# inferflow/inferflow

Hardware: AMD Instinct MI355X
Metric: decode tokens/sec, Llama-2-7B Q4 batch=1 greedy (whole job) (higher is better)
Workload: dtype i8 (Q8 activations x Q4_B32T1A weights, i32 dot, f32 scale, f16 I/O); 1 GPU; llama2_7b decode, Q4_B32T1A weights + F16 lm_head, F16 KV cache, batch 1 greedy, 16-token prompt, context 21..1851; parallelism=single, weights_bytes=4309647360

## Files before the change

### include/inferflow_amd.h

```cpp
#ifndef INFERFLOW_AMD_H_
#define INFERFLOW_AMD_H_

#include <stddef.h>
#include <stdint.h>

#ifdef __cplusplus
extern "C" {
#endif

typedef enum {
    IFA_F32 = 0, IFA_F16 = 1,
    IFA_Q8_B32T1 = 7, IFA_Q8_B32T2 = 8, IFA_Q6_B64T1 = 9, IFA_Q5_B64T1 = 10, IFA_Q5_B32T1 = 11,
    IFA_Q4_B16 = 12, IFA_Q4_B32T1A = 13, IFA_Q4_B32T1B = 14, IFA_Q4_B64T1 = 17, IFA_Q3H_B64T1 = 18,
    IFA_Q3_B32T1A = 19, IFA_Q3_B32T1B = 20, IFA_Q2_B32T1A = 21, IFA_Q2_B32T1B = 22
} ifa_dtype;

enum {
    IFA_OK = 0,
    IFA_ERR_ARG = -1,
    IFA_ERR_DTYPE = -2,
    IFA_ERR_HIP = -3,
    IFA_ERR_STATE = -4,
    IFA_ERR_NOMEM = -5
};
// ... 89 lines not shown
typedef struct {
    int strategy_id;
    float temperature, top_p;
    int max_k;
    float min_p;
    int pool_size;
} ifa_sample_params;
int ifa_sample_pool_rows(const int *counts_dev, const int *ids_dev, const void *vals_f16_dev, size_t rows, int k_stride,
                         const ifa_sample_params *params_dev, unsigned long long *rng_state_dev, int *tokens_out_dev, int *index_out_dev,
                         float *weights_out_dev, int *err_dev, ifa_stream stream);
int ifa_sample_pool_host(const int *ids, const unsigned short *vals_f16, int count, const ifa_sample_params *p,
                         unsigned long long *rng_state_inout, int *token_out, int *index_out, int *cut_len_out, float *weights_out,
                         int *order_ids_out);

int ifa_logit_adjust_rows(const void *logits_f16, size_t row_stride, const int *row_idx_dev, const int *state_slot_dev, size_t rows, size_t n,
                          const unsigned *state_dev, const float *bias_dev, const float *params_dev, void *out_f16_dev, ifa_stream stream);
int ifa_logit_state_reset(int slot, const int *prompt_tokens_dev, size_t n_prompt, float rep, float freq, float pres, const int *bias_ids_dev,
                          const float *bias_vals_dev, size_t n_bias, size_t n, unsigned *state_dev, float *bias_dev, float *params_dev, ifa_stream stream);
int ifa_logit_state_add(const int *slots_dev, const int *tokens_dev, size_t n_pairs, size_t n, size_t n_slots, unsigned *state_dev, ifa_stream stream);

typedef struct ifa_model ifa_model;

typedef struct {
    int dim, layers, heads, kv_heads, head_dim, ffn, vocab, max_ctx;
    int norm_kind;
    int act_kind;
    int is_glu;
    int rope_order;
    int use_alibi;
    int parallel_attn;
    int share_input;
    float rope_theta, partial_rotary, kq_scale, eps;
    int kv_dtype;
    int full_quant_gemv;
    int experts, moe_top_k, moe_norm_topk;
    int tp_rank, tp_size;
    int device;
    float attn_norm_base, ffn_norm_base, out_norm_base, attn_out_scale, ffn_out_scale, out_scale;
    float embd_scale;
} ifa_model_config;

enum {
    IFA_T_EMBD = 0, IFA_T_OUT_NORM = 1, IFA_T_OUT_NORM_B = 2, IFA_T_LM_HEAD = 3,
    IFA_T_ATTN_NORM = 10, IFA_T_ATTN_NORM_B = 11, IFA_T_WQ = 12, IFA_T_WK = 13, IFA_T_WV = 14, IFA_T_WO = 15,
    IFA_T_FFN_NORM = 16, IFA_T_FFN_NORM_B = 17, IFA_T_W1 = 18, IFA_T_W2 = 19, IFA_T_W3 = 20, IFA_T_MOE_GATE = 21,
    IFA_T_WQ_B = 22, IFA_T_WK_B = 23, IFA_T_WV_B = 24, IFA_T_WO_B = 25, IFA_T_W1_B = 26, IFA_T_W2_B = 27, IFA_T_W3_B = 28,
    IFA_T_ATTN_POST_NORM = 29, IFA_T_ATTN_POST_NORM_B = 30, IFA_T_FFN_POST_NORM = 31, IFA_T_FFN_POST_NORM_B = 32
};

int ifa_model_create(const ifa_model_config *cfg, ifa_model **out);
int ifa_model_destroy(ifa_model *m);
int ifa_model_set_tensor(ifa_model *m, int layer, int tensor_id, int expert, int dtype,
                         const void *dev_src, size_t rows, size_t cols);
int ifa_model_set_tensor_f16(ifa_model *m, int layer, int tensor_id, int expert, int target_dtype,
                             const void *dev_src_f16, size_t rows, size_t cols);
int ifa_model_finalize(ifa_model *m);
int ifa_model_reset(ifa_model *m);
int ifa_model_kv_slots(ifa_model *m, int n_slots);
int ifa_model_select_kv(ifa_model *m, int slot);
int ifa_model_kv_copy(ifa_model *m, int src_slot, int dst_slot, int n_rows);
int ifa_model_kv_shift(ifa_model *m, int slot, int keep, int discard, int n_rows);
int ifa_kv_shift_rows(int kv_dtype, void *kcache, void *vcache, size_t kv_heads, size_t head_dim, int rope_order, int rope_cols,
                      const float *table_dev, size_t keep, size_t discard, size_t n_rows, ifa_stream stream);
int ifa_model_set_option(ifa_model *m, const char *name, int value);
int ifa_model_set_excluded_tokens(ifa_model *m, const int *ids_host, int n);
int ifa_model_perf_stat(ifa_model *m, int *keys_out, float *ms_out, int cap, int *n_out, int clear);
int ifa_model_fused_supported(ifa_model *m, char *why, size_t why_len);
int ifa_model_forward(ifa_model *m, const int *tokens_host, int n_tokens, int prefix_len,
                      void *logits_out_dev, int *next_token_host);
int ifa_model_decode(ifa_model *m, int first_token, int start_pos, int n_steps,
                     int *out_tokens_host, float *elapsed_ms);
int ifa_model_decode_sampled(ifa_model *m, int first_token, int start_pos, int n_steps, const ifa_sample_params *p,
                             unsigned long long *rng_state_inout, int state_slot, int *out_tokens_host, float *elapsed_ms);
int ifa_model_decode_prepare(ifa_model *m, int start_pos, int n_steps);
int ifa_model_decode_batch(ifa_model *m, int n, const int *tokens_host, const int *positions_host, const int *kv_slots_host,
                           int *next_tokens_host, void *logits_out_dev);
int ifa_model_decode_draft(ifa_model *m, int n, const int *tokens_host, int pos0, int *next_tokens_host, void *logits_out_dev);
int ifa_model_set_pool_excluded(ifa_model *m, const int *ids_host, int n);
int ifa_model_decode_pool(ifa_model *m, int token, int pos, int k, int *next_token_host,
                          int *pool_ids_host, unsigned short *pool_vals_host, int *pool_count_host);
int ifa_model_decode_batch_pool(ifa_model *m, int n, const int *tokens_host, const int *positions_host, const int *kv_slots_host,
                                int *next_tokens_host, int k, const int *rows_sel_host, int n_sel,
                                int *pool_ids_host, unsigned short *pool_vals_host, int *pool_counts_host);
int ifa_model_forward_pool(ifa_model *m, const int *tokens_host, int n_tokens, int prefix_len, void *logits_out_dev, int k,
                           int *next_token_host, int *pool_ids_host, unsigned short *pool_vals_host, int *pool_count_host);
int ifa_model_pool_lse(ifa_model *m, float *lse_host, int cap, int *n_out);
#define IFA_LOGIT_BIAS_MAX 1024
int ifa_model_logit_state_reset(ifa_model *m, int kv_slot, const int *prompt_host, int n_prompt, float rep, float freq, float pres,
                                const int *bias_ids_host, const float *bias_vals_host, int n_bias);
int ifa_model_logit_state_add(ifa_model *m, int n, const int *kv_slots_host, const int *tokens_host);
int ifa_model_pool_adjust(ifa_model *m, int n_sel, const int *state_slots_host);
int ifa_model_forward_score(ifa_model *m, const int *tokens_host, int n_tokens, int prefix_len, const int *targets_host,
                            float *lse_host, float *target_logit_host, int *next_token_host);
int ifa_model_get_buffer(ifa_model *m, const char *name, int layer, void **dptr, size_t *bytes);
void *ifa_model_stream(ifa_model *m);
int ifa_debug_alloc_fail_at(long long nth);
int ifa_debug_live_allocs(long long *count, long long *bytes);
int ifa_model_set_stream(ifa_model *m, ifa_stream stream);

typedef struct ifa_comm ifa_comm;
#define IFA_COMM_ID_BYTES 128
int ifa_comm_unique_id(void *id_out_128);
int ifa_comm_init_rank(const void *id_128, int nranks, int rank, int device, ifa_comm **out);
int ifa_comm_init_all(const int *device_ids, int n, ifa_comm **comms_out);
int ifa_comm_capturable(const ifa_comm *c);
unsigned long long ifa_comm_serial(const ifa_comm *c);
int ifa_comm_oneshot(const ifa_comm *c);
#define IFA_ONESHOT_HANDLE_BYTES 128
int ifa_comm_oneshot_export(ifa_comm *c, void *handle_out_128);
int ifa_comm_oneshot_import(ifa_comm *c, const void *handles_all_ranks);
int ifa_comm_set_oneshot(ifa_comm *c, int on);
int ifa_comm_status(ifa_comm *c);
int ifa_comm_abort(ifa_comm *c);
int ifa_comm_destroy(ifa_comm *c);
int ifa_comm_rank(const ifa_comm *c);
int ifa_comm_size(const ifa_comm *c);
int ifa_comm_group_start(void);
int ifa_comm_group_end(void);
int ifa_allreduce_sum_f16(ifa_comm *c, const void *send_f16, void *recv_f16, size_t count, ifa_stream stream);
int ifa_allgather(ifa_comm *c, const void *send, void *recv, size_t bytes_per_rank, ifa_stream stream);
int ifa_broadcast(ifa_comm *c, void *buf, size_t bytes, int root, ifa_stream stream);
int ifa_send(ifa_comm *c, const void *buf, size_t bytes, int peer, ifa_stream stream);
int ifa_recv(ifa_comm *c, void *buf, size_t bytes, int peer, ifa_stream stream);

int ifa_model_tp_begin(ifa_model *m, int token, int pos);
int ifa_model_tp_begin_hidden(ifa_model *m, const void *x_f16, int pos);
int ifa_model_tp_hidden(ifa_model *m, void *x_out_f16);
int ifa_model_tp_attn(ifa_model *m, int layer, void *partial_out_f16);
int ifa_model_tp_post_attn(ifa_model *m, int layer, const void *reduced_f16);
int ifa_model_tp_ffn(ifa_model *m, int layer, void *partial_out_f16);
int ifa_model_tp_post_ffn(ifa_model *m, int layer, const void *reduced_f16);
int ifa_model_tp_logits(ifa_model *m, void *logits_shard_out_f16);
int ifa_model_tp_set_token(ifa_model *m, const int *token_dev);
typedef struct {
    ifa_comm *tp;
    ifa_comm *world;
    int stage, n_stages;
    int prev_rank, next_rank, token_src;
    int vocab_offset;
    int force_collectives;
} ifa_tp_topology;
int ifa_model_tp_decode(ifa_model *m, const ifa_tp_topology *topo, int first_token, int start_pos, int n_steps,
                        int *out_tokens_host, float *elapsed_ms);
int ifa_model_tp_prefill(ifa_model *m, const ifa_tp_topology *topo, const int *tokens_host, int n_tokens, int start_pos,
                         void *logits_shard_out_dev, int *next_token_host);
int ifa_model_tp_decode_batch(ifa_model *m, const ifa_tp_topology *topo, int n, const int *tokens_host, const int *positions_host,
                              const int *kv_slots_host, int *next_tokens_host, void *logits_shard_out_dev);
int ifa_model_get_tensor(ifa_model *m, int layer, int tensor_id, int *dtype, void **dptr, size_t *rows, size_t *cols);
int ifa_model_get_expert_tensor(ifa_model *m, int layer, int expert, int tensor_id, int *dtype, void **dptr, size_t *rows, size_t *cols);
int ifa_model_time_kernel(ifa_model *m, int which, int iters, float *avg_us);

int ifa_decode_route_plan(const int *facts, int n_facts, int *out, int n_out);
int ifa_model_decode_route(ifa_model *m, int *out, int n_out);

int ifa_prompt_route_plan(const int *facts, int n_facts, int *out, int n_out);
int ifa_batch_route_plan(const int *facts, int n_facts, int *out, int n_out);
int ifa_model_prompt_route(ifa_model *m, int *out, int n_out);

#ifdef __cplusplus
}
#endif
#endif
```

### inferflow_amd/_capi.py

```python
import ctypes as C
import os

_HERE = os.path.dirname(os.path.abspath(__file__))
_LIB_PATH = os.environ.get("IFA_LIB") or os.path.join(_HERE, "lib", "libinferflow_amd.so")
_lib = None


class IfaError(RuntimeError):
    def __init__(self, code, msg):
        super().__init__("inferflow_amd error %d: %s" % (code, msg))
        self.code = code


def library_path():
    return _LIB_PATH


def lib():
    global _lib
    if _lib is None:
        if not os.path.exists(_LIB_PATH):
            raise ImportError(
                "inferflow_amd: %s is missing -- run `python __graft_entry__.py build` "
                "(hipcc --offload-arch=gfx950); there is no CPU fallback" % _LIB_PATH)
        L = C.CDLL(_LIB_PATH, mode=C.RTLD_GLOBAL)
        _declare(L)
        _lib = L
    return _lib


def check(rc):
    if rc != 0:
        raise IfaError(rc, lib().ifa_last_error().decode(errors="replace"))
    return rc


_vp, _sz, _i, _f = C.c_void_p, C.c_size_t, C.c_int, C.c_float

SIGNATURES = {
    "ifa_version": (C.c_char_p, []),
    "ifa_last_error": (C.c_char_p, []),
    "ifa_device_count": (_i, []),
    "ifa_set_device": (_i, [_i]),
    "ifa_malloc": (_i, [C.POINTER(_vp), _sz]),
    "ifa_free": (_i, [_vp]),
    "ifa_memcpy_h2d": (_i, [_vp, _vp, _sz, _vp]),
    "ifa_memcpy_d2h": (_i, [_vp, _vp, _sz, _vp]),
    "ifa_memcpy_d2d": (_i, [_vp, _vp, _sz, _vp]),
    "ifa_memset": (_i, [_vp, _i, _sz, _vp]),
    "ifa_stream_create": (_i, [C.POINTER(_vp)]),
    "ifa_stream_destroy": (_i, [_vp]),
    "ifa_stream_sync": (_i, [_vp]),
    "ifa_block_capacity": (_i, [_i]),
    "ifa_block_bytes": (_i, [_i]),
    "ifa_row_bytes": (_sz, [_i, _sz]),
    "ifa_dtype_from_name": (_i, [C.c_char_p]),
    "ifa_quantize": (_i, [_i, _vp, _sz, _sz, _vp, _vp]),
    "ifa_quantize_f32": (_i, [_i, _vp, _sz, _sz, _vp, _vp]),
    "ifa_dequantize": (_i, [_i, _vp, _sz, _sz, _vp, _vp]),
    "ifa_quantize_act_q8": (_i, [_vp, _sz, _sz, _vp, _vp]),
    "ifa_gemv": (_i, [_i, _vp, _sz, _sz, _i, _vp, _vp, _vp, _vp]),
    "ifa_gemm": (_i, [_i, _vp, _sz, _sz, _vp, _sz, _vp, _vp, _vp]),
    "ifa_attention_two_pass_min": (_i, [_i]),
    "ifa_attention_two_pass_min_keys": (_i, [_i]),
    "ifa_gemm_big_tiles": (_i, [_i]),
    "ifa_wait_grid_decision": (_i, [_i, _i, C.c_longlong]),
    "ifa_visible_cus_from_mask": (_i, [C.c_char_p, _i, _i]),
    "ifa_inlaunch_waits_enabled": (_i, []),
    "ifa_gemm_release_stream": (_i, [_vp]),
    "ifa_tiled_row_bytes": (_sz, [_i, _sz]),
    "ifa_repack_weights": (_i, [_i, _vp, _sz, _sz, _vp, _vp]),
    "ifa_gemv_tiled": (_i, [_i, _vp, _sz, _sz, _vp, _vp, _vp, _vp]),
    "ifa_layernorm": (_i, [_i, _vp, _sz, _sz, _vp, _vp, _f, _f, _vp, _vp]),
    "ifa_exact_rmsnorm": (_i, [_vp, _sz, _sz, _vp, _vp, _f, _f, _vp, _vp]),
    "ifa_exact_gemv": (_i, [_i, _vp, _sz, _sz, _i, _vp, _vp, _vp, _vp]),
    "ifa_exact_attention": (_i, [_vp, _vp, _vp, _i, _i, _i, _i, _i, _f, _vp, _vp]),
    "ifa_exact_activation_mul": (_i, [_i, _vp, _vp, _sz, _vp, _vp]),
    "ifa_rope": (_i, [_vp, _i, _i, _i, _i, _f, _i, _f, _vp]),
    "ifa_alibi": (_i, [_vp, _i, _i, _i, _i, _i, _vp]),
    "ifa_softmax": (_i, [_vp, _i, _i, _i, _i, _f, _vp]),
    "ifa_activation": (_i, [_i, _i, _vp, _sz, _sz, _vp, _vp]),
    "ifa_mul": (_i, [_vp, _vp, _sz, _vp, _vp]),
    "ifa_add": (_i, [_vp, _vp, _sz, _sz, _vp, _vp]),
    "ifa_scale": (_i, [_vp, _f, _sz, _vp, _vp]),
    "ifa_attention": (_i, [_vp, _vp, _vp, _i, _i, _i, _i, _i, _i, _i, _f, _i, _i, _i, _vp, _vp]),
    "ifa_moe_route_topk": (_i, [_vp, _sz, _i, _i, _i, _vp, _vp, _vp]),
    "ifa_kv_store": (_i, [_i, _vp, _sz, _sz, _vp, _sz, _vp]),
    "ifa_argmax": (_i, [_vp, _sz, _vp, _vp]),
    "ifa_argmax_masked": (_i, [_vp, _sz, _vp, _vp, _vp]),
    "ifa_topk_pool": (_i, [_vp, _sz, _sz, _i, _vp, _vp, _vp, _vp, _vp]),
    "ifa_sample_pool_rows": (_i, [_vp, _vp, _vp, _sz, _i, _vp, _vp, _vp, _vp, _vp, _vp, _vp]),
    "ifa_sample_pool_host": (_i, [_vp, _vp, _i, _vp, _vp, _vp, _vp, _vp, _vp, _vp]),
    "ifa_logsumexp_workspace": (_sz, [_sz, _sz]),
    "ifa_logsumexp_rows": (_i, [_vp, _sz, _vp, _sz, _sz, _vp, _vp, _vp, _vp, _vp]),
    "ifa_logit_adjust_rows": (_i, [_vp, _sz, _vp, _vp, _sz, _sz, _vp, _vp, _vp, _vp, _vp]),
    "ifa_logit_state_reset": (_i, [_i, _vp, _sz, _f, _f, _f, _vp, _vp, _sz, _sz, _vp, _vp, _vp, _vp]),
    "ifa_logit_state_add": (_i, [_vp, _vp, _sz, _sz, _sz, _vp, _vp]),
    "ifa_model_create": (_i, [_vp, C.POINTER(_vp)]),
    "ifa_model_destroy": (_i, [_vp]),
    "ifa_debug_alloc_fail_at": (_i, [C.c_longlong]),
    "ifa_debug_live_allocs": (_i, [C.POINTER(C.c_longlong), C.POINTER(C.c_longlong)]),
    "ifa_model_set_tensor": (_i, [_vp, _i, _i, _i, _i, _vp, _sz, _sz]),
    "ifa_model_set_tensor_f16": (_i, [_vp, _i, _i, _i, _i, _vp, _sz, _sz]),
    "ifa_model_finalize": (_i, [_vp]),
    "ifa_model_reset": (_i, [_vp]),
    "ifa_model_set_option": (_i, [_vp, C.c_char_p, _i]),
    "ifa_model_set_excluded_tokens": (_i, [_vp, _vp, _i]),
    "ifa_model_perf_stat": (_i, [_vp, _vp, _vp, _i, _vp, _i]),
    "ifa_model_fused_supported": (_i, [_vp, C.c_char_p, _sz]),
    "ifa_model_forward": (_i, [_vp, _vp, _i, _i, _vp, _vp]),
    "ifa_model_decode": (_i, [_vp, _i, _i, _i, _vp, _vp]),
    "ifa_model_decode_sampled": (_i, [_vp, _i, _i, _i, _vp, _vp, _i, _vp, _vp]),
    "ifa_model_decode_prepare": (_i, [_vp, _i, _i]),
    "ifa_add_by_row_index": (_i, [_vp, _vp, _sz, _sz, _vp, _vp, _vp]),
    "ifa_model_kv_slots": (_i, [_vp, _i]),
    "ifa_model_select_kv": (_i, [_vp, _i]),
    "ifa_model_kv_copy": (_i, [_vp, _i, _i, _i]),
    "ifa_model_kv_shift": (_i, [_vp, _i, _i, _i, _i]),
    "ifa_kv_shift_rows": (_i, [_i, _vp, _vp, _sz, _sz, _i, _i, _vp, _sz, _sz, _sz, _vp]),
    "ifa_model_decode_batch": (_i, [_vp, _i, _vp, _vp, _vp, _vp, _vp]),
    "ifa_model_decode_draft": (_i, [_vp, _i, _vp, _i, _vp, _vp]),
    "ifa_model_set_pool_excluded": (_i, [_vp, _vp, _i]),
    "ifa_model_decode_pool": (_i, [_vp, _i, _i, _i, _vp, _vp, _vp, _vp]),
    "ifa_model_decode_batch_pool": (_i, [_vp, _i, _vp, _vp, _vp, _vp, _i, _vp, _i, _vp, _vp, _vp]),
    "ifa_model_forward_pool": (_i, [_vp, _vp, _i, _i, _vp, _i, _vp, _vp, _vp, _vp]),
    "ifa_model_pool_lse": (_i, [_vp, _vp, _i, _vp]),
    "ifa_model_logit_state_reset": (_i, [_vp, _i, _vp, _i, _f, _f, _f, _vp, _vp, _i]),
    "ifa_model_logit_state_add": (_i, [_vp, _i, _vp, _vp]),
    "ifa_model_pool_adjust": (_i, [_vp, _i, _vp]),
    "ifa_model_forward_score": (_i, [_vp, _vp, _i, _i, _vp, _vp, _vp, _vp]),
    "ifa_model_get_buffer": (_i, [_vp, C.c_char_p, _i, C.POINTER(_vp), C.POINTER(_sz)]),
    "ifa_model_stream": (_vp, [_vp]),
    "ifa_model_time_kernel": (_i, [_vp, _i, _i, _vp]),
    "ifa_decode_route_plan": (_i, [_vp, _i, _vp, _i]),
    "ifa_model_decode_route": (_i, [_vp, _vp, _i]),
    "ifa_prompt_route_plan": (_i, [_vp, _i, _vp, _i]),
    "ifa_batch_route_plan": (_i, [_vp, _i, _vp, _i]),
    "ifa_model_prompt_route": (_i, [_vp, _vp, _i]),
    "ifa_model_set_stream": (_i, [_vp, _vp]),
    "ifa_model_tp_begin": (_i, [_vp, _i, _i]),
    "ifa_model_tp_begin_hidden": (_i, [_vp, _vp, _i]),
    "ifa_model_tp_hidden": (_i, [_vp, _vp]),
    "ifa_model_tp_attn": (_i, [_vp, _i, _vp]),
    "ifa_model_tp_post_attn": (_i, [_vp, _i, _vp]),
    "ifa_model_tp_ffn": (_i, [_vp, _i, _vp]),
    "ifa_model_tp_post_ffn": (_i, [_vp, _i, _vp]),
    "ifa_model_tp_logits": (_i, [_vp, _vp]),
    "ifa_model_tp_set_token": (_i, [_vp, _vp]),
    "ifa_comm_unique_id": (_i, [_vp]),
    "ifa_comm_init_rank": (_i, [_vp, _i, _i, _i, C.POINTER(_vp)]),
    "ifa_comm_init_all": (_i, [_vp, _i, C.POINTER(_vp)]),
    "ifa_comm_destroy": (_i, [_vp]),
    "ifa_comm_capturable": (_i, [_vp]),
    "ifa_comm_serial": (C.c_ulonglong, [_vp]),
    "ifa_comm_abort": (_i, [_vp]),
    "ifa_comm_oneshot": (_i, [_vp]),
    "ifa_comm_oneshot_export": (_i, [_vp, _vp]),
    "ifa_comm_oneshot_import": (_i, [_vp, _vp]),
    "ifa_comm_set_oneshot": (_i, [_vp, _i]),
    "ifa_comm_status": (_i, [_vp]),
    "ifa_comm_rank": (_i, [_vp]),
    "ifa_comm_size": (_i, [_vp]),
    "ifa_comm_group_start": (_i, []),
    "ifa_comm_group_end": (_i, []),
    "ifa_allreduce_sum_f16": (_i, [_vp, _vp, _vp, _sz, _vp]),
    "ifa_allgather": (_i, [_vp, _vp, _vp, _sz, _vp]),
    "ifa_broadcast": (_i, [_vp, _vp, _sz, _i, _vp]),
    "ifa_send": (_i, [_vp, _vp, _sz, _i, _vp]),
    "ifa_recv": (_i, [_vp, _vp, _sz, _i, _vp]),
    "ifa_model_tp_decode": (_i, [_vp, _vp, _i, _i, _i, _vp, _vp]),
    "ifa_model_tp_prefill": (_i, [_vp, _vp, _vp, _i, _i, _vp, _vp]),
    "ifa_model_tp_decode_batch": (_i, [_vp, _vp, _i, _vp, _vp, _vp, _vp, _vp]),
    "ifa_model_get_tensor": (_i, [_vp, _i, _i, _vp, C.POINTER(_vp), C.POINTER(_sz), C.POINTER(_sz)]),
    "ifa_model_get_expert_tensor": (_i, [_vp, _i, _i, _i, _vp, C.POINTER(_vp), C.POINTER(_sz), C.POINTER(_sz)]),
}


_ip = C.POINTER(C.c_int)
ENGINE_SIGNATURES = {
    "ifa_engine_create": (_vp, [C.c_char_p, C.c_char_p, C.c_char_p]),
    "ifa_engine_destroy": (None, [_vp]),
    "ifa_engine_last_error": (C.c_char_p, []),
    "ifa_engine_add_query": (_i, [_vp, _ip, _i]),
    "ifa_engine_add_query_ex": (_i, [_vp, _ip, _i, _i, _i, _f]),
    "ifa_engine_add_query_lp": (_i, [_vp, _ip, _i, _i, _i, _f, _i]),
    "ifa_engine_add_query_opt": (_i, [_vp, _ip, _i, _vp]),
    "ifa_engine_last_logprobs": (_i, [_vp, _i, C.POINTER(_f), _ip, C.POINTER(_f), _i, _ip]),
    "ifa_engine_score": (_i, [_vp, _ip, _i, C.POINTER(_f)]),
    "ifa_engine_strategy_id": (_i, [_vp, C.c_char_p]),
    "ifa_sampling_choose": (_i, [_vp, _i, _i, _i, _f, _i, _f, C.c_longlong, _i, _ip, C.POINTER(_f), _ip, C.POINTER(_f), _i]),
    "ifa_sampling_choose_ex": (_i, [_vp, _i, _i, C.POINTER(_f), _f, C.c_longlong, _i, _ip, C.POINTER(_f), _ip, C.POINTER(_f), _i, C.POINTER(_f), _ip, _i]),
    "ifa_sampling_choose_from_pool": (_i, [_ip, _vp, _i, _i, C.POINTER(_f), _f, C.c_longlong, _i, _ip, C.POINTER(_f), _ip, C.POINTER(_f), _i, C.POINTER(_f), _ip, _i]),
    "ifa_sampling_random_doubles": (_i, [C.c_longlong, _i, C.POINTER(C.c_double)]),
    "ifa_engine_query_count": (_i, [_vp]),
    "ifa_engine_remove_query": (_i, [_vp, _i]),
    "ifa_engine_infer": (_i, [_vp, _ip, _ip, _i]),
    "ifa_engine_commit": (_i, [_vp, _ip, _ip, _ip, _i]),
    "ifa_engine_last_logits": (_i, [_vp, _i, _vp, _sz, _ip, _ip]),
    "ifa_engine_perf_stat": (_i, [_vp, _vp, _vp, _i]),
    "ifa_engine_generate": (_i, [_vp, _i, _i, _ip, C.POINTER(_f)]),
    "ifa_engine_generate_lookup": (_i, [_vp, _i, _i, _ip, _i, _ip, C.POINTER(_f)]),
    "ifa_lookup_draft": (_i, [_ip, _i, _ip, _i, _i, _i, _i, _ip]),
    "ifa_engine_perplexity": (_i, [_vp, _ip, _i, _i, _i, C.POINTER(C.c_double), C.POINTER(C.c_double), C.POINTER(C.c_longlong)]),
    "ifa_engine_perplexity_device": (_i, [_vp, _ip, _i, _i, _i, C.POINTER(C.c_double), C.POINTER(C.c_double), C.POINTER(C.c_longlong)]),
    "ifa_perplexity_token_nll": (C.c_double, [_vp, _i, _i]),
    "ifa_engine_model_info": (_i, [_vp, C.c_char_p]),
    "ifa_engine_query_cached_tokens": (_i, [_vp, _i]),
    "ifa_context_shift_plan": (_i, [_i, _i, _i, _i, _ip]),
    "ifa_engine_shift_query": (_i, [_vp, _i, _i, _i]),
    "ifa_engine_query_shifted_tokens": (_i, [_vp, _i]),
    "ifa_prefix_cache_plan": (_i, [_ip, _ip, _ip, C.POINTER(C.c_longlong), _i, _ip, _i, _i, _ip]),
    "ifa_step_plan_query": (_i, [_i, _i, _i, _i, _i, _ip]),
    "ifa_step_plan_batch": (_i, [_i, _ip, _i, _ip, _ip]),
    "ifa_engine_worker": (_vp, [_vp, _i]),
    "ifa_engine_worker_plan": (_i, [_vp, _i, _ip]),
    "ifa_service_parse_request": (_i, [C.c_char_p, _i, C.c_char_p, _sz]),
    "ifa_service_format_response": (_i, [_ip, _i, _i, _i, _i, _i, C.c_char_p, _sz]),
    "ifa_service_selftest_loop": (_i, [_i, _i, _i, _ip, _i, _i, _i, _i, _i, C.c_char_p, _sz]),
    "ifa_service_selftest_request": (_i, [C.c_char_p, _i, _i, C.c_char_p, _sz]),
    "ifa_partition_slice": (_i, [_i, _i, _i, _i, _i, _i, _i, _i, _sz, _sz, C.POINTER(_sz)]),
    "ifa_partition_split_layers": (_i, [_i, _i, _ip, _i]),
}


class QueryOptions(C.Structure):
    _fields_ = [("struct_size", C.c_size_t), ("strategy_id", C.c_int), ("random_seed", C.c_int), ("temperature", C.c_float),
                ("logprobs", C.c_int), ("repetition_penalty", C.c_float), ("presence_penalty", C.c_float),
                ("frequency_penalty", C.c_float), ("n_logit_bias", C.c_int), ("logit_bias_ids", C.POINTER(C.c_int)),
                ("logit_bias_values", C.POINTER(C.c_float))]


class QueryOptionsShift(C.Structure):
    _fields_ = QueryOptions._fields_ + [("context_shift", C.c_int), ("context_keep", C.c_int)]


class SampleParams(C.Structure):
    _fields_ = [("strategy_id", C.c_int), ("temperature", C.c_float), ("top_p", C.c_float), ("max_k", C.c_int), ("min_p", C.c_float), ("pool_size", C.c_int)]


class ModelConfig(C.Structure):
    _fields_ = [(n, C.c_int) for n in (
        "dim", "layers", "heads", "kv_heads", "head_dim", "ffn", "vocab", "max_ctx",
        "norm_kind", "act_kind", "is_glu", "rope_order", "use_alibi", "parallel_attn",
        "share_input")] + [(n, C.c_float) for n in (
            "rope_theta", "partial_rotary", "kq_scale", "eps")] + [(n, C.c_int) for n in (
                "kv_dtype", "full_quant_gemv", "experts", "moe_top_k", "moe_norm_topk",
                "tp_rank", "tp_size", "device")] + [(n, C.c_float) for n in (
                    "attn_norm_base", "ffn_norm_base", "out_norm_base", "attn_out_scale", "ffn_out_scale", "out_scale", "embd_scale")]


def _declare(L):
    missing = []
    for name, (res, args) in list(SIGNATURES.items()) + list(ENGINE_SIGNATURES.items()):
        try:
            fn = getattr(L, name)
        except AttributeError:
            missing.append(name)
            continue
        fn.restype = res
        fn.argtypes = args
    if missing and os.environ.get("IFA_LIB"):
        return
    if missing:
        raise ImportError("libinferflow_amd.so lacks symbols declared in include/*.h: %s" % missing)
```

### inferflow_amd/csrc/ifa_decode_route.h

```cpp
#pragma once
#include <algorithm>
#include <cstddef>
#include <cstring>

static constexpr size_t IFA_LDS_LIMIT = 160 * 1024;

namespace ifa {
constexpr int DEC_ATTN_MAX_SPLITS = 32;
constexpr int DEC_PV_STAGE = 4096;

constexpr size_t dec_attn_scores_smem(int head_dim, bool q8) { return q8 ? 16 : (size_t)256 * (head_dim * 2 + 16); }
constexpr size_t dec_attn_pv_smem(int head_dim, int max_ctx, int nsplits = 8)
{
    const size_t nsplit = 256 / (head_dim / 8);
    const size_t chunk = (((size_t)max_ctx + nsplits - 1) / nsplits + 63) / 64 * 64;
    return 8 * 4 + nsplit * head_dim * 4 + (size_t)(DEC_PV_STAGE + 8) * 2 + chunk * 2 + 16;
}
constexpr size_t dec_attn_smem(int head_dim, int max_ctx, int ktile_rows = 0)
{
    const size_t nsplit = 256 / (head_dim / 8);
    return (size_t)head_dim * 3 * 2 + 16 * 4 + nsplit * head_dim * 4 + (size_t)ktile_rows * head_dim * 2 + (((size_t)max_ctx * 2 + 15) & ~(size_t)15) + 16;
}

inline bool dec_qkv_attn_ul_shape(int rw, int gk) { return (rw == 6 && gk == 8) || (rw == 3 && gk == 32); }

struct DecRouteFacts {
    int head_dim = 0, heads = 0, kv_heads = 0, max_ctx = 0, kv_q8 = 0;
    int reach = 0;
    int attn_split_ctx = -1, attn_nsplits = 0, attn_kt = 1, attn_unload = 1, fuse_attn = 1, fuse_ffn = 0, attn_q8 = 1;
    int tail_layers_ok = 0, gk = 0, rw = 0;
    int chain_level = 0;
    int have_attq = 0;
    int waits = 1;
    int num_cus = 0, visible_cus = 0;
    int own_launches = 0;
};
enum DecRouteKind { DEC_ROUTE_ONE_WORKGROUP = 0, DEC_ROUTE_SPLIT = 1, DEC_ROUTE_FUSED_TAIL = 2 };

struct DecRoute {
    int kind = DEC_ROUTE_ONE_WORKGROUP;
    int nsplits = 0;
    int pb = 256, kt = 0, ul = 0;
    int gk = 0, rw = 0;
    int chain = 0;
    int split_threshold = 0, split = 0;
    int lds_attn = 0;
    int lds_scores = 0, lds_pv = 0;
    int error = 0;
    bool operator==(const DecRoute &o) const { return std::memcmp(this, &o, sizeof(o)) == 0; }
};
constexpr int DEC_ROUTE_N_FACTS = sizeof(DecRouteFacts) / sizeof(int), DEC_ROUTE_N_OUT = sizeof(DecRoute) / sizeof(int);

inline DecRoute plan_decode_route(const DecRouteFacts &f)
{
    DecRoute r;
    const bool tail_possible = f.fuse_attn && f.waits && dec_attn_smem(f.head_dim, f.max_ctx, 256) <= IFA_LDS_LIMIT && f.tail_layers_ok && (long long)f.kv_heads * f.gk <= (long long)f.visible_cus;
    r.split_threshold = f.attn_split_ctx >= 0 ? f.attn_split_ctx : (tail_possible && f.attn_unload) ? (f.heads > f.kv_heads ? 640 : 512) : 320;
    r.split = (r.split_threshold > 0 && f.reach > r.split_threshold) ? (f.reach > 8192 ? 16 : 8) : 0;
    const int bucket = f.reach <= 64 ? 64 : (f.reach <= 128 ? 128 : 256);
    const bool lds_split = dec_attn_smem(f.head_dim, f.max_ctx, 0) > IFA_LDS_LIMIT;
    r.kind = (r.split || lds_split) ? DEC_ROUTE_SPLIT : (tail_possible && !f.own_launches) ? DEC_ROUTE_FUSED_TAIL : DEC_ROUTE_ONE_WORKGROUP;
    const bool kt_fits = f.attn_kt && !f.kv_q8 && dec_attn_smem(f.head_dim, f.max_ctx, bucket) <= IFA_LDS_LIMIT;
    if (r.kind == DEC_ROUTE_SPLIT) {
        r.pb = 0; r.nsplits = r.split > 1 ? r.split : 8;
        while (r.nsplits < DEC_ATTN_MAX_SPLITS && dec_attn_pv_smem(f.head_dim, f.max_ctx, r.nsplits) > IFA_LDS_LIMIT) r.nsplits *= 2;
        if (f.attn_nsplits > 0) r.nsplits = std::min(f.attn_nsplits, DEC_ATTN_MAX_SPLITS);
        r.lds_scores = (int)dec_attn_scores_smem(f.head_dim, f.kv_q8 != 0); r.lds_pv = (int)dec_attn_pv_smem(f.head_dim, f.max_ctx, r.nsplits);
        r.error = (size_t)r.lds_pv > IFA_LDS_LIMIT;
    } else if (r.kind == DEC_ROUTE_ONE_WORKGROUP) {
        const bool pow2 = f.head_dim == 32 || f.head_dim == 64 || f.head_dim == 128;
        r.pb = pow2 ? bucket : 256; r.kt = kt_fits && pow2;
    } else {
        r.kt = kt_fits;
        const bool unload = (f.attn_unload >= 1 && bucket == 256) || (f.attn_unload >= 2 && bucket == 128 && (r.kt || f.kv_q8));
        r.ul = unload && dec_qkv_attn_ul_shape(f.rw, f.gk);
        r.pb = (r.ul && bucket == 64) || (!f.kv_q8 && !r.kt) ? 256 : bucket;
        r.gk = f.gk; r.rw = f.rw;
    }
    if (r.kind != DEC_ROUTE_SPLIT) r.lds_attn = (int)dec_attn_smem(f.head_dim, f.max_ctx, r.kt ? r.pb : 0);
    if (!f.own_launches) {
        r.chain = (f.fuse_ffn && f.waits && f.num_cus <= f.visible_cus) ? std::min(f.fuse_ffn, 2) : 0;
        if (r.chain == 2 && (!f.have_attq || !f.attn_q8 || f.head_dim % 32 != 0)) r.chain = 1;
        r.chain = std::min(r.chain, f.chain_level);
    }
    return r;
}

}
```

### inferflow_amd/csrc/ifa_engine.hip

```cpp
#include <mutex>
#include <unordered_map>
#include "ifa_engine_state.h"

namespace ifa {

namespace {
struct SpaceBook {
    std::mutex mu;
    std::unordered_map<void *, size_t> live;
    long long live_bytes = 0, fail_at = 0;
};
SpaceBook &book() { static SpaceBook *b = new SpaceBook(); return *b; }

template <class Alloc> int space_alloc(const char *call, void **p, size_t bytes, Alloc alloc)
{
    SpaceBook &b = book();
    *p = nullptr;
    {
        std::lock_guard<std::mutex> g(b.mu);
        if (b.fail_at > 0 && --b.fail_at == 0)
            return ifa_fail(IFA_ERR_HIP, "%s(%zu bytes) failed: out of memory (simulated: ifa_debug_alloc_fail_at)", call, bytes);
    }
    const hipError_t e = alloc(p, bytes);
    if (e != hipSuccess) {
        (void)hipGetLastError();
        *p = nullptr;
        return ifa_fail(IFA_ERR_HIP, "%s(%zu bytes) failed: %s", call, bytes, hipGetErrorString(e));
    }
    if (*p) { std::lock_guard<std::mutex> g(b.mu); b.live[*p] = bytes; b.live_bytes += (long long)bytes; }
    return IFA_OK;
}

void space_forget(void *p)
{
    SpaceBook &b = book();
    std::lock_guard<std::mutex> g(b.mu);
    auto it = b.live.find(p);
    if (it != b.live.end()) { b.live_bytes -= (long long)it->second; b.live.erase(it); }
}
}

int DevSpace::alloc(void **p, size_t bytes) { return space_alloc("hipMalloc", p, bytes, [](void **q, size_t n) { return hipMalloc(q, n); }); }
void DevSpace::free(void *p) { space_forget(p); (void)hipFree(p); }
int PinSpace::alloc(void **p, size_t bytes) { return space_alloc("hipHostMalloc", p, bytes, [](void **q, size_t n) { return hipHostMalloc(q, n, hipHostMallocDefault); }); }
void PinSpace::free(void *p) { space_forget(p); (void)hipHostFree(p); }

}

extern "C" int ifa_debug_alloc_fail_at(long long nth)
{
    IFA_REQUIRE(nth >= 0, "ifa_debug_alloc_fail_at: nth %lld", nth);
    std::lock_guard<std::mutex> g(book().mu);
    book().fail_at = nth;
    return IFA_OK;
}

extern "C" int ifa_debug_live_allocs(long long *count, long long *bytes)
{
    std::lock_guard<std::mutex> g(book().mu);
    if (count) *count = (long long)book().live.size();
    if (bytes) *bytes = book().live_bytes;
    return IFA_OK;
}

namespace ifae {

int perf_begin(ifa_model *m, int key)
{
    if (!m->opt_perf_stat) return -1;
    hipStreamCaptureStatus cs = hipStreamCaptureStatusNone;
    if (hipStreamIsCapturing(m->stream, &cs) != hipSuccess || cs != hipStreamCaptureStatusNone) { (void)hipGetLastError(); return -1; }
    auto take = [&]() -> hipEvent_t {
        if (!m->perf_pool.empty()) { hipEvent_t e = m->perf_pool.back(); m->perf_pool.pop_back(); return e; }
        hipEvent_t e = nullptr;
        if (hipEventCreate(&e) != hipSuccess) { (void)hipGetLastError(); return nullptr; }
        return e;
    };
    ifa_model::PerfSpanRec r; r.key = key; r.e0 = take(); r.e1 = take();
    if (!r.e0 || !r.e1) { if (r.e0) m->perf_pool.push_back(r.e0); if (r.e1) m->perf_pool.push_back(r.e1); return -1; }
    if (hipEventRecord(r.e0, m->stream) != hipSuccess) { (void)hipGetLastError(); m->perf_pool.push_back(r.e0); m->perf_pool.push_back(r.e1); return -1; }
    m->perf_spans.push_back(r);
    return (int)m->perf_spans.size() - 1;
}

void perf_end(ifa_model *m, int idx)
{
    if (idx < 0 || idx >= (int)m->perf_spans.size()) return;
    if (hipEventRecord(m->perf_spans[(size_t)idx].e1, m->stream) != hipSuccess) (void)hipGetLastError();
}

int perf_collect(ifa_model *m)
{
    if (m->perf_spans.empty()) return IFA_OK;
    IFA_HIP_CHECK(hipStreamSynchronize(m->stream));
    for (auto &r : m->perf_spans) {
        float ms = 0.0f;
        if (hipEventElapsedTime(&ms, r.e0, r.e1) == hipSuccess) m->perf_map[r.key] += ms;
        else (void)hipGetLastError();
        m->perf_pool.push_back(r.e0); m->perf_pool.push_back(r.e1);
    }
    m->perf_spans.clear();
    return IFA_OK;
}

void drop_graphs(ifa_model *m)
{
    if (m->tp_graph_exec) { (void)hipGraphExecDestroy(m->tp_graph_exec); m->tp_graph_exec = nullptr; }
    if (m->tp_graph) { (void)hipGraphDestroy(m->tp_graph); m->tp_graph = nullptr; }
    if (m->graph_exec) { (void)hipGraphExecDestroy(m->graph_exec); m->graph_exec = nullptr; }
    if (m->graph) { (void)hipGraphDestroy(m->graph); m->graph = nullptr; }
    if (m->graph_exec_n) { (void)hipGraphExecDestroy(m->graph_exec_n); m->graph_exec_n = nullptr; }
    if (m->graph_n) { (void)hipGraphDestroy(m->graph_n); m->graph_n = nullptr; }
    for (auto &sl : m->slots) {
        if (sl.exec) { (void)hipGraphExecDestroy(sl.exec); sl.exec = nullptr; }
        if (sl.graph) { (void)hipGraphDestroy(sl.graph); sl.graph = nullptr; }
    }
    for (auto &kv : m->batch_graphs) if (kv.second) (void)hipGraphExecDestroy(kv.second);
    m->batch_graphs.clear();
    for (auto &kv : m->draft_graphs) if (kv.second) (void)hipGraphExecDestroy(kv.second);
    m->draft_graphs.clear();
    sampled_drop_graphs(m);
}

int ensure_scratch(ifa_model *m, int T)
{
    if (T <= m->scratch_tokens) return IFA_OK;
    const ifa_model_config &c = m->cfg;
    const size_t D = c.dim, QD = (size_t)c.heads * c.head_dim, KVD = (size_t)c.kv_heads * c.head_dim, F = c.ffn;
    size_t maxcols = std::max(std::max(D, QD), F);
    Scratch n;
    int rc;
    if ((rc = n.x.alloc(T * D)) || (rc = n.x2.alloc(T * D)) || (rc = n.xn.alloc(T * D)) || (rc = n.hn.alloc(T * D)) || (rc = n.pn.alloc(T * D))
        || (rc = n.q.alloc(T * QD)) || (rc = n.k.alloc(T * KVD)) || (rc = n.v.alloc(T * KVD)) || (rc = n.att.alloc(T * QD))
        || (rc = n.a.alloc(T * D)) || (rc = n.f.alloc(T * D)) || (rc = n.t1.alloc(std::max<size_t>(T, 3) * F)) || (rc = n.t2.alloc(T * F))
        || (rc = n.logits.alloc((size_t)T * c.vocab)))
        return rc;
    if (!m->dqkv && (rc = n.dqkv.alloc(QD + 2 * KVD))) return rc;
    if (T <= 32 && !m->bqkv && ((rc = n.bqkv.alloc(32 * (QD + 2 * KVD))) || (rc = n.brope.alloc(32 * (size_t)c.head_dim)))) return rc;
    if (c.experts > 0) {
        const size_t cap = (size_t)T * (size_t)std::max(1, c.moe_top_k);
        if ((rc = n.moe_gate.alloc((size_t)T * c.experts)) || (rc = n.moe_out.alloc((size_t)T * D)) || (rc = n.moe_in.alloc((size_t)T * D))
            || (rc = n.moe_wdev.alloc(cap)) || (rc = n.moe_idx.alloc(cap)) || (rc = n.moe_pin.alloc(cap * (sizeof(int) + 2) + 16)))
            return rc;
        if (!m->moe_route) {
            if ((rc = n.moe_route.alloc(64 / sizeof(int)))) return rc;
            IFA_HIP_CHECK(hipMemsetAsync(n.moe_route, 0, 64, m->stream));
        }
        if ((rc = n.moe_sel.alloc(cap)) || (rc = n.moe_epos.alloc(cap)) || (rc = n.moe_counts.alloc(16))
            || (rc = n.moe_xq_in.alloc(cap * (D / 32 + 1) * 34)) || (rc = n.moe_xq_mid.alloc(cap * (F / 32 + 1) * 34))
            || (rc = n.moe_tiles.alloc((cap / 64 + (size_t)c.experts + 1) * sizeof(MoeTile)))
            || (rc = n.moe_singles.alloc(((size_t)c.experts + 1) * sizeof(MoeSingle))) || (rc = n.moe_smalls.alloc(((size_t)c.experts + 1) * sizeof(MoeTile)))
            || (rc = n.moe_selw.alloc(cap)) || (rc = n.moe_g1.alloc(cap * F)) || (rc = n.moe_g3.alloc(cap * F)) || (rc = n.moe_gin.alloc(cap * D))
            || (rc = n.moe_gout.alloc(cap * D)))
            return rc;
    }
    if ((rc = n.xq.alloc((maxcols / 32 + 1) * 34))) return rc;
    if (!m->attq && (rc = n.attq.alloc(xq_image_bytes(c.heads * c.head_dim)))) return rc;
    if ((rc = n.tokens_dev.alloc((size_t)T))) return rc;
    if (!n.dqkv) n.dqkv = std::move(m->dqkv);
    if (!n.bqkv) { n.bqkv = std::move(m->bqkv); n.brope = std::move(m->brope); }
    if (!n.moe_route) n.moe_route = std::move(m->moe_route);
    if (!n.attq) n.attq = std::move(m->attq);
    static_cast<Scratch &>(*m) = std::move(n);
    m->scratch_tokens = T;
    drop_graphs(m);
    return IFA_OK;
}

void *kv_ptr(ifa_model *m, size_t layer, int slot, bool is_v)
{
    if (slot == m->cur_slot || m->slots.empty()) return is_v ? m->layers[layer].vcache : m->layers[layer].kcache;
    const ifa_model::KvSlot &sl = m->slots[(size_t)slot];
    return is_v ? sl.v[layer] : sl.k[layer];
}

int ensure_mo(ifa_model *m)
{
    if (!m->opt_rows_mo) return IFA_OK;
    const int rc = ensure_mo_build(m);
    if (rc == IFA_OK) return IFA_OK;
    (void)hipGetLastError();
    for (Layer &L : m->layers) {
        for (Tensor &t : L.t) t.mo.reset();
        for (Tensor &t : L.experts) t.mo.reset();
        L.moe_table_mo.reset();
    }
    m->opt_rows_mo = 0;
    drop_graphs(m);
    fprintf(stderr, "inferflow_amd: the rows GEMM's operand-order weight copies could not be built (%s); batched steps use the tiled kernels\n", ifa_last_error());
    return IFA_OK;
}

int ensure_mo_build(ifa_model *m)
{
    const ifa_model_config &c = m->cfg;
    bool built = false;
    for (Layer &L : m->layers) {
        const bool moe = c.experts > 0 && L.t[T_MOE_GATE].present();
        const int ids[] = {T_WQ, T_WK, T_WV, T_WO, T_W1, T_W3, T_W2};
        for (int id : ids) {
            Tensor &t = L.t[id];
            if (moe && (id == T_W1 || id == T_W3 || id == T_W2)) continue;
            if (t.mo || !t.present() || !t.tiled || !rows_mo_fmt(t.dtype) || t.cols % 128 != 0) continue;
            if (m->opt_debug_mo_alloc_fail && built) return ifa_fail(IFA_ERR_HIP, "hipMalloc: out of memory (simulated: debug_mo_alloc_fail)");
            int rc = t.mo.alloc(gemm_rows_mo_bytes(t.rows, t.cols));
            if (rc) return rc;
            rc = gemm_rows_mo_build(t.dtype, t.tiled, t.rows, t.cols, t.mo, m->stream);
            if (rc) return rc;
            built = true;
        }
    }
    for (Layer &L : m->layers) {
        if (!(c.experts > 0 && L.t[T_MOE_GATE].present()) || L.moe_table_mo || (int)L.experts.size() != c.experts * 3) continue;
        bool ok = true;
        for (Tensor &t : L.experts) ok = ok && t.present() && t.tiled && is_q4(t.dtype) && t.cols % 128 == 0;
        if (!ok) continue;
        std::vector<void *> tab((size_t)c.experts * 4, nullptr);
        for (int e = 0; e < c.experts; e++) {
            const int order[3] = {0, 2, 1};
            for (int k = 0; k < 3; k++) {
                Tensor &t = L.experts[(size_t)e * 3 + order[k]];
                if (!t.mo) {
                    int rc = t.mo.alloc(gemm_rows_mo_bytes(t.rows, t.cols));
                    if (rc) return rc;
                    rc = gemm_rows_mo_build(t.dtype, t.tiled, t.rows, t.cols, t.mo, m->stream);
                    if (rc) return rc;
                    built = true;
                }
                tab[(size_t)e * 4 + k] = t.mo;
            }
        }
        { int rc = L.moe_table_mo.alloc(tab.size()); if (rc) return rc; }
        IFA_HIP_CHECK(hipMemcpy(L.moe_table_mo, tab.data(), tab.size() * sizeof(void *), hipMemcpyHostToDevice));
    }
    if (built) IFA_HIP_CHECK(hipStreamSynchronize(m->stream));
    return IFA_OK;
}

int ensure_x32(ifa_model *m)
{
    bool built = false;
    for (Layer &L : m->layers) {
        const int ids[] = {T_WQ, T_WK, T_WV, T_WO, T_W1, T_W3, T_W2};
        for (int id : ids) {
            Tensor &t = L.t[id];
            if (t.x32 || !t.present() || !t.tiled || (t.dtype != Q4_B64T1 && t.dtype != Q3H_B64T1) || t.cols % 64 != 0) continue;
            int rc = t.x32.alloc(t.rows * (t.cols / 32) * 20);
            if (rc) return rc;
            rc = expand_b64_to_q4b32(t.dtype, t.tiled, t.rows, t.cols, t.x32, m->stream);
            if (rc) return rc;
            built = true;
        }
    }
    if (built) IFA_HIP_CHECK(hipStreamSynchronize(m->stream));
    return IFA_OK;
}

int ensure_q3hn(ifa_model *m)
{
    bool built = false;
    for (Layer &L : m->layers) {
        const int ids[] = {T_WO, T_W1, T_W3, T_W2};
        for (int id : ids) {
            Tensor &t = L.t[id];
            if (t.q3hn || !t.present() || t.dtype != Q3H_B64T1 || t.cols % 64 != 0) continue;
            int rc = t.q3hn.alloc(t.rows * (t.cols / 64) * 32);
            if (rc) return rc;
            rc = q3h_native_rows(t.data, t.rows, t.cols, t.q3hn, m->stream);
            if (rc) return rc;
// ... 83 lines not shown
        if (vec) IFA_REQUIRE(rows * cols == ec, "ifa_model_set_tensor: tensor %d holds %zu x %zu values, the model needs %zu", tensor_id, rows, cols, ec);
        else {
            IFA_REQUIRE(ec == 0 || cols == ec, "ifa_model_set_tensor: tensor %d has %zu columns, the model needs %zu", tensor_id, cols, ec);
            IFA_REQUIRE(er == 0 || rows == er, "ifa_model_set_tensor: tensor %d has %zu rows, the model needs %zu", tensor_id, rows, er);
        }
        if (tensor_id == T_LM_HEAD && layer < 0) IFA_REQUIRE(rows <= (size_t)c.vocab, "ifa_model_set_tensor: lm_head has %zu rows, vocab is %d", rows, c.vocab);
        if (tensor_id == T_EMBD) IFA_REQUIRE(rows <= (size_t)c.vocab, "ifa_model_set_tensor: %zu embedding rows, vocab is %d", rows, c.vocab);
    }
    IFA_HIP_CHECK(hipSetDevice(m->cfg.device));
    Tensor *t;
    if (tensor_id < 10) t = &m->g[tensor_id];
    else {
        IFA_REQUIRE(layer >= 0 && layer < m->cfg.layers, "ifa_model_set_tensor: layer %d", layer);
        Layer &L = m->layers[(size_t)layer];
        if (expert >= 0) {
            if (L.experts.empty()) L.experts.resize((size_t)m->cfg.experts * 3);
            t = &L.experts[(size_t)expert * 3 + (tensor_id == T_W1 ? 0 : (tensor_id == T_W2 ? 1 : 2))];
        } else t = &L.t[tensor_id];
    }
    *t = Tensor();
    if (expert >= 0) m->layers[(size_t)layer].moe_table_mo.reset();
    IFA_HIP_CHECK(hipDeviceSynchronize());
    const size_t bytes = rows * ifa_row_bytes(dtype, cols);
    int rc = t->data.alloc(bytes);
    if (rc) return rc;
    IFA_HIP_CHECK(hipMemcpyAsync(t->data, dev_src, bytes, hipMemcpyDeviceToDevice, m->stream));
    t->dtype = dtype; t->rows = rows; t->cols = cols;
    const bool is_matrix = (layer < 0 && tensor_id == T_LM_HEAD) || tensor_id == T_WQ || tensor_id == T_WK || tensor_id == T_WV || tensor_id == T_WO
        || tensor_id == T_W1 || tensor_id == T_W2 || tensor_id == T_W3;
    if (is_matrix && ax8_eligible(dtype)) {
        if ((rc = t->tiled.alloc(rows * ifa_tiled_row_bytes(dtype, cols)))) return rc;
        rc = ifa_repack_weights(dtype, t->data, rows, cols, t->tiled, m->stream);
        if (rc) return rc;
    }
    IFA_HIP_CHECK(hipStreamSynchronize(m->stream));
    drop_graphs(m);
    return IFA_OK;
}

int ifa_model_set_tensor_f16(ifa_model *m, int layer, int tensor_id, int expert, int target_dtype,
                             const void *dev_src_f16, size_t rows, size_t cols)
{
    IFA_REQUIRE(m && dev_src_f16, "ifa_model_set_tensor_f16: null pointer");
    if (target_dtype == F16) return ifa_model_set_tensor(m, layer, tensor_id, expert, F16, dev_src_f16, rows, cols);
    IFA_HIP_CHECK(hipSetDevice(m->cfg.device));
    DevBuf<void> tmp;
    const size_t bytes = rows * ifa_row_bytes(target_dtype, cols);
    IFA_REQUIRE(bytes > 0, "ifa_model_set_tensor_f16: dtype %d", target_dtype);
    int rc = tmp.alloc(bytes);
    if (rc) return rc;
    IFA_HIP_CHECK(hipDeviceSynchronize());
    rc = ifa_quantize(target_dtype, dev_src_f16, rows, cols, tmp, m->stream);
    if (rc == IFA_OK) rc = ifa_model_set_tensor(m, layer, tensor_id, expert, target_dtype, tmp, rows, cols);
    (void)hipStreamSynchronize(m->stream);
    return rc;
}

int ifa_model_finalize(ifa_model *m)
{
    IFA_REQUIRE(m, "ifa_model_finalize: null model");
    IFA_HIP_CHECK(hipSetDevice(m->cfg.device));
    (void)wait_err_word();
    const ifa_model_config &c = m->cfg;
    const size_t KVD = (size_t)c.kv_heads * c.head_dim;
    IFA_REQUIRE(c.kv_dtype != Q8_B32T2 || KVD % 32 == 0, "Q8 KV cache needs kv_dim %% 32 == 0");
    m->kv_row_bytes = ifa_row_bytes(c.kv_dtype, KVD);
    int rc;
    for (Layer &L : m->layers) {
        if (!L.kcache) {
            const size_t kv_alloc = m->kv_row_bytes * (size_t)std::max(c.max_ctx, DEC_ATTN_MIN_ROWS);
            if ((rc = L.kcache.alloc(kv_alloc)) || (rc = L.vcache.alloc(kv_alloc))) return rc;
            IFA_HIP_CHECK(hipMemsetAsync(L.kcache, 0, kv_alloc, m->stream));
            IFA_HIP_CHECK(hipMemsetAsync(L.vcache, 0, kv_alloc, m->stream));
        }
        if (c.experts > 0 && (int)L.experts.size() == c.experts * 3) {
            std::vector<void *> tab((size_t)c.experts * 4, nullptr);
            for (int e = 0; e < c.experts; e++) {
                tab[(size_t)e * 4 + 0] = L.experts[(size_t)e * 3 + 0].tiled;
                tab[(size_t)e * 4 + 1] = L.experts[(size_t)e * 3 + 2].tiled;
                tab[(size_t)e * 4 + 2] = L.experts[(size_t)e * 3 + 1].tiled;
            }
            if (!L.moe_table && (rc = L.moe_table.alloc(tab.size()))) return rc;
            IFA_HIP_CHECK(hipMemcpy(L.moe_table, tab.data(), tab.size() * sizeof(void *), hipMemcpyHostToDevice));
            std::vector<void *> aos((size_t)c.experts * 3, nullptr);
            for (int e = 0; e < c.experts; e++) for (int k3 = 0; k3 < 3; k3++) aos[(size_t)e * 3 + k3] = L.experts[(size_t)e * 3 + k3].data;
            if (!L.moe_table_aos && (rc = L.moe_table_aos.alloc(aos.size()))) return rc;
            IFA_HIP_CHECK(hipMemcpy(L.moe_table_aos, aos.data(), aos.size() * sizeof(void *), hipMemcpyHostToDevice));
        }
    }
    if (!m->attn_ws.S) {
        if ((rc = m->attn_ws_S.alloc((size_t)c.heads * c.max_ctx + 32))
            || (rc = m->attn_ws_lmax.alloc((size_t)c.heads * DEC_ATTN_MAX_SPLITS))
            || (rc = m->attn_ws_opart.alloc((size_t)c.heads * DEC_ATTN_MAX_SPLITS * c.head_dim))) return rc;
        m->attn_ws.S = m->attn_ws_S; m->attn_ws.lmax = m->attn_ws_lmax; m->attn_ws.opart = m->attn_ws_opart;
    }
    if (!m->state) {
        if ((rc = m->state.alloc(8 + ifa_model::RING))) return rc;
        IFA_HIP_CHECK(hipMemsetAsync(m->state, 0, sizeof(int) * (8 + ifa_model::RING), m->stream));
        if ((rc = m->rope_tab.alloc((size_t)c.head_dim)) || (rc = m->host_pinned.alloc(16 + ifa_model::RING))) return rc;
    }
    if ((rc = ensure_scratch(m, 1))) return rc;
    IFA_HIP_CHECK(hipStreamSynchronize(m->stream));
    m->finalized = true;
    return IFA_OK;
}

int ifa_model_reset(ifa_model *m)
{
    IFA_REQUIRE(m && m->finalized, "ifa_model_reset: model not finalized");
    IFA_HIP_CHECK(hipSetDevice(m->cfg.device));
    for (Layer &L : m->layers) {
        IFA_HIP_CHECK(hipMemsetAsync(L.kcache, 0, m->kv_row_bytes * (size_t)m->cfg.max_ctx, m->stream));
        IFA_HIP_CHECK(hipMemsetAsync(L.vcache, 0, m->kv_row_bytes * (size_t)m->cfg.max_ctx, m->stream));
    }
    IFA_HIP_CHECK(hipStreamSynchronize(m->stream));
    return IFA_OK;
}

int ifa_model_kv_slots(ifa_model *m, int n_slots)
{
    IFA_REQUIRE(m && m->finalized, "ifa_model_kv_slots: model not finalized");
    IFA_REQUIRE(n_slots >= 1 && n_slots <= 4096, "ifa_model_kv_slots: n_slots %d", n_slots);
    IFA_HIP_CHECK(hipSetDevice(m->cfg.device));
    if (m->slots.empty()) m->slots.resize(1);
    IFA_REQUIRE((int)m->slots.size() <= n_slots, "ifa_model_kv_slots: cannot shrink below %zu slots", m->slots.size());
    const size_t bytes = m->kv_row_bytes * (size_t)std::max(m->cfg.max_ctx, DEC_ATTN_MIN_ROWS);
    while ((int)m->slots.size() < n_slots) {
        ifa_model::KvSlot sl;
        for (size_t l = 0; l < m->layers.size(); l++) {
            DevBuf<void> k, v;
            int rc;
            if ((rc = k.alloc(bytes)) || (rc = v.alloc(bytes))) return rc;
            IFA_HIP_CHECK(hipMemsetAsync(k, 0, bytes, m->stream));
            IFA_HIP_CHECK(hipMemsetAsync(v, 0, bytes, m->stream));
            sl.k.push_back(std::move(k)); sl.v.push_back(std::move(v));
        }
        m->slots.push_back(std::move(sl));
    }
    IFA_HIP_CHECK(hipStreamSynchronize(m->stream));
    return IFA_OK;
}

int ifa_model_select_kv(ifa_model *m, int slot)
{
    IFA_REQUIRE(m && m->finalized, "ifa_model_select_kv: model not finalized");
    if (m->slots.empty()) m->slots.resize(1);
    IFA_REQUIRE(slot >= 0 && slot < (int)m->slots.size(), "ifa_model_select_kv: slot %d of %zu", slot, m->slots.size());
    if (slot == m->cur_slot) return IFA_OK;
    if (m->tp_graph_exec) { (void)hipGraphExecDestroy(m->tp_graph_exec); m->tp_graph_exec = nullptr; }
    if (m->tp_graph) { (void)hipGraphDestroy(m->tp_graph); m->tp_graph = nullptr; }
    ifa_model::KvSlot &out = m->slots[(size_t)m->cur_slot], &in = m->slots[(size_t)slot];
    out.k.clear(); out.v.clear();
    for (Layer &L : m->layers) { out.k.push_back(std::move(L.kcache)); out.v.push_back(std::move(L.vcache)); }
    out.graph = m->graph; out.exec = m->graph_exec;
    if (m->graph_exec_n) { (void)hipGraphExecDestroy(m->graph_exec_n); m->graph_exec_n = nullptr; }
    if (m->graph_n) { (void)hipGraphDestroy(m->graph_n); m->graph_n = nullptr; }
    for (size_t l = 0; l < m->layers.size(); l++) { m->layers[l].kcache = std::move(in.k[l]); m->layers[l].vcache = std::move(in.v[l]); }
    m->graph = in.graph; m->graph_exec = in.exec;
    in.k.clear(); in.v.clear(); in.graph = nullptr; in.exec = nullptr;
    m->cur_slot = slot;
    return IFA_OK;
}

int ifa_model_set_option(ifa_model *m, const char *name, int value)
{
    IFA_REQUIRE(m && name, "ifa_model_set_option: null pointer");
    if (strcmp(name, "pool_lse") == 0) { m->opt_pool_lse = value != 0; return IFA_OK; }
    struct { const char *n; int *p; } opts[] = {
        {"fused", &m->opt_fused}, {"graph", &m->opt_graph}, {"rpw_qkv", &m->opt_rpw_qkv}, {"rpw_wo", &m->opt_rpw_wo},
        {"rpw_ffn", &m->opt_rpw_ffn}, {"rpw_w2", &m->opt_rpw_w2}, {"rpw_lm", &m->opt_rpw_lm}, {"trace", &m->opt_trace},
        {"bench_mode", &m->opt_bench_mode}, {"touch_stride", &m->opt_touch_stride}, {"attn_split_ctx", &m->opt_attn_split_ctx}, {"batch_graph", &m->opt_batch_graph}, {"gemm_rows", &m->opt_gemm_rows}, {"batch_fused", &m->opt_batch_fused}, {"rows_mo", &m->opt_rows_mo}, {"debug_mo_alloc_fail", &m->opt_debug_mo_alloc_fail}, {"rows_kparts", &m->opt_rows_kparts}, {"prefill_chunk", &m->opt_prefill_chunk}, {"prefill_big_min", &m->opt_prefill_big_min}, {"prefill_mid", &m->opt_prefill_mid}, {"prefill_mid_max", &m->opt_prefill_mid_max}, {"prefill_res_mid", &m->opt_prefill_res_mid}, {"gemm_splitk", &m->opt_gemm_splitk}, {"moe_singles", &m->opt_moe_singles}, {"moe_overlap", &m->opt_moe_overlap}, {"prefill_big", &m->opt_prefill_big}, {"moe_router_fused", &m->opt_moe_router_fused}, {"tp_fuse_add", &m->opt_tp_fuse_add}, {"attn_q8", &m->opt_attn_q8}, {"attn_kt", &m->opt_attn_kt}, {"fuse_attn", &m->opt_fuse_attn}, {"fuse_ffn", &m->opt_fuse_ffn}, {"attn_post_as_residual", &m->opt_attn_post_as_residual}, {"chain_late_w2", &m->opt_chain_late_w2}, {"exact_order", &m->opt_exact_order}, {"perf_stat", &m->opt_perf_stat}, {"attn_nsplits", &m->opt_attn_nsplits}, {"attn_unload", &m->opt_attn_unload}, {"q3h_native", &m->opt_q3h_native}, {"fuse_attn_timeout_us", &m->opt_fuse_attn_timeout_us}, {"step_tail", &m->opt_step_tail}, {"graph_steps", &m->opt_graph_steps}, {"moe_device", &m->opt_moe_device}, 
        
        {"debug_layers", &m->opt_debug_layers}, {"debug_layer0", &m->opt_debug_layer0}, {"debug_hidden_in", &m->opt_debug_hidden_in}};
    for (auto &o : opts)
        if (strcmp(o.n, name) == 0) {
            *o.p = value;
            drop_graphs(m);
            return IFA_OK;
        }
    return ifa_fail(IFA_ERR_ARG, "ifa_model_set_option: unknown option '%s'", name);
}

int ifa_model_perf_stat(ifa_model *m, int *keys_out, float *ms_out, int cap, int *n_out, int clear)
{
    IFA_REQUIRE(m && n_out && cap >= 0 && (cap == 0 || (keys_out && ms_out)), "ifa_model_perf_stat: null pointer");
    IFA_HIP_CHECK(hipSetDevice(m->cfg.device));
    int rc = perf_collect(m);
    if (rc) return rc;
    int n = 0;
    for (auto &kv : m->perf_map) {
        if (n < cap) { keys_out[n] = kv.first; ms_out[n] = kv.second; }
        n++;
    }
    *n_out = n;
    if (clear) m->perf_map.clear();
    return IFA_OK;
}

int ifa_model_set_excluded_tokens(ifa_model *m, const int *ids_host, int n)
{
    IFA_REQUIRE(m && m->finalized, "ifa_model_set_excluded_tokens: model not finalized");
    IFA_REQUIRE(n >= 0 && n <= 3 && (n == 0 || ids_host), "ifa_model_set_excluded_tokens: n %d (0..3)", n);
    int v[4] = {n, -1, -1, -1};
    for (int i = 0; i < n; i++) v[1 + i] = ids_host[i];
    IFA_HIP_CHECK(hipStreamSynchronize(m->stream));
    IFA_HIP_CHECK(hipMemcpy(m->state + 3, v, sizeof(v), hipMemcpyHostToDevice));
    return IFA_OK;
}

int ifa_model_fused_supported(ifa_model *m, char *why, size_t why_len)
{
    IFA_REQUIRE(m, "ifa_model_fused_supported: null model");
    std::string w;
    bool ok = fused_supported(m, &w);
    if (why && why_len) { strncpy(why, w.c_str(), why_len - 1); why[why_len - 1] = 0; }
    return ok ? 1 : 0;
}

int ifa_decode_route_plan(const int *facts, int n_facts, int *out, int n_out)
{
    IFA_REQUIRE(facts && out && n_facts == DEC_ROUTE_N_FACTS && n_out >= DEC_ROUTE_N_OUT, "ifa_decode_route_plan: %d facts, %d outputs expected", DEC_ROUTE_N_FACTS, DEC_ROUTE_N_OUT);
    DecRouteFacts f;
    memcpy(&f, facts, sizeof(f));
    IFA_REQUIRE(f.head_dim >= 8 && f.max_ctx >= 1, "ifa_decode_route_plan: head_dim %d, max_ctx %d", f.head_dim, f.max_ctx);
    const DecRoute r = plan_decode_route(f);
    memcpy(out, &r, sizeof(r));
    return IFA_OK;
}

int ifa_model_decode_route(ifa_model *m, int *out, int n_out)
{
    IFA_REQUIRE(m && out && n_out >= DEC_ROUTE_N_OUT + 3, "ifa_model_decode_route: %d outputs expected", DEC_ROUTE_N_OUT + 3);
    memcpy(out, &m->route, sizeof(m->route));
    out[DEC_ROUTE_N_OUT] = num_cus(); out[DEC_ROUTE_N_OUT + 1] = visible_cus(); out[DEC_ROUTE_N_OUT + 2] = waits_enabled() ? 1 : 0;
    return IFA_OK;
}

int ifa_prompt_route_plan(const int *facts, int n_facts, int *out, int n_out)
{
    IFA_REQUIRE(facts && out && n_facts == PROMPT_ROUTE_N_FACTS && n_out >= PROMPT_ROUTE_N_OUT, "ifa_prompt_route_plan: %d facts, %d outputs expected", PROMPT_ROUTE_N_FACTS, PROMPT_ROUTE_N_OUT);
    PromptRouteFacts f;
    memcpy(&f, facts, sizeof(f));
    const PromptRoute r = plan_prompt_route(f);
    memcpy(out, &r, sizeof(r));
    return IFA_OK;
}

int ifa_batch_route_plan(const int *facts, int n_facts, int *out, int n_out)
{
    IFA_REQUIRE(facts && out && n_facts == BATCH_ROUTE_N_FACTS && n_out >= BATCH_ROUTE_N_OUT, "ifa_batch_route_plan: %d facts, %d outputs expected", BATCH_ROUTE_N_FACTS, BATCH_ROUTE_N_OUT);
    BatchRouteFacts f;
    memcpy(&f, facts, sizeof(f));
    const BatchRoute r = plan_batch_route(f);
    memcpy(out, &r, sizeof(r));
    return IFA_OK;
}

int ifa_model_prompt_route(ifa_model *m, int *out, int n_out)
{
    IFA_REQUIRE(m && out && n_out >= PROMPT_ROUTE_N_OUT, "ifa_model_prompt_route: %d outputs expected", PROMPT_ROUTE_N_OUT);
    memcpy(out, &m->prompt_route, sizeof(m->prompt_route));
    return IFA_OK;
}

int ifa_model_get_buffer(ifa_model *m, const char *name, int layer, void **dptr, size_t *bytes)
{
    IFA_REQUIRE(m && name && dptr, "ifa_model_get_buffer: null pointer");
    const ifa_model_config &c = m->cfg;
    size_t b = 0; void *p = nullptr;
    if (!strcmp(name, "logits")) { p = m->logits; b = (size_t)c.vocab * 2; }
    else if (!strcmp(name, "logits_adj")) { p = m->la_adj; b = m->la_adj ? m->la_adj.cap() / m->g[T_LM_HEAD].rows * (size_t)c.vocab * 2 : 0; }
    else if (!strcmp(name, "logit_state")) { p = m->la_state; b = m->la_slots * m->g[T_LM_HEAD].rows * sizeof(unsigned); }
    else if (!strcmp(name, "tp_logits")) { p = m->tp_logits; b = m->tp_logits ? m->g[T_LM_HEAD].rows * 2 : 0; }
    else if (!strcmp(name, "trace")) { p = m->trace; b = m->trace ? sizeof(long long) * 2048 * 8 : 0; }
    else if (!strcmp(name, "hidden")) { p = m->xn; b = (size_t)c.dim * 2; }
    else if (!strcmp(name, "x")) { p = m->x; b = (size_t)c.dim * 2; }
    else if (!strcmp(name, "x2")) { p = m->x2; b = (size_t)c.dim * 2; }
    else if (!strcmp(name, "dqkv")) { p = m->dqkv; b = ((size_t)c.heads + 2 * (size_t)c.kv_heads) * c.head_dim * 2; }
    else if (!strcmp(name, "att")) { p = m->att; b = (size_t)c.heads * c.head_dim * 2; }
    else if (!strcmp(name, "attq")) { p = m->attq; b = m->attq ? xq_image_bytes(c.heads * c.head_dim) : 0; }
    else if (!strcmp(name, "a")) { p = m->a; b = (size_t)c.dim * 2; }
    else if (!strcmp(name, "t1")) { p = m->t1; b = (size_t)c.ffn * 2; }
    else if (!strcmp(name, "kcache") || !strcmp(name, "vcache")) {
        IFA_REQUIRE(layer >= 0 && layer < c.layers && m->finalized, "ifa_model_get_buffer: layer %d", layer);
        p = name[0] == 'k' ? m->layers[(size_t)layer].kcache : m->layers[(size_t)layer].vcache;
        b = m->kv_row_bytes * (size_t)c.max_ctx;
    } else return ifa_fail(IFA_ERR_ARG, "ifa_model_get_buffer: unknown buffer '%s'", name);
    *dptr = p;
    if (bytes) *bytes = b;
    return IFA_OK;
}

void *ifa_model_stream(ifa_model *m) { return m ? (void *)m->stream : nullptr; }

int ifa_model_set_stream(ifa_model *m, ifa_stream stream)
{
    IFA_REQUIRE(m, "ifa_model_set_stream: null model");
    IFA_HIP_CHECK(hipSetDevice(m->cfg.device));
    if (m->stream) IFA_HIP_CHECK(hipStreamSynchronize(m->stream));
    if (m->stream) (void)ifa_gemm_release_stream((ifa_stream)m->stream);
    if (m->stream && m->own_stream) IFA_HIP_CHECK(hipStreamDestroy(m->stream));
    m->stream = ifa_s(stream);
    m->own_stream = false;
    drop_graphs(m);
    return IFA_OK;
}

int ifa_model_get_tensor(ifa_model *m, int layer, int tensor_id, int *dtype, void **dptr, size_t *rows, size_t *cols)
{
    IFA_REQUIRE(m && tensor_id >= 0 && tensor_id < T_MAX, "ifa_model_get_tensor: bad arguments");
    const Tensor *t;
    if (tensor_id < 10) t = &m->g[tensor_id];
    else {
        IFA_REQUIRE(layer >= 0 && layer < m->cfg.layers, "ifa_model_get_tensor: layer %d", layer);
        t = &m->layers[(size_t)layer].t[tensor_id];
    }
    if (dtype) *dtype = t->dtype;
    if (dptr) *dptr = t->data;
    if (rows) *rows = t->rows;
    if (cols) *cols = t->cols;
    return t->present() ? IFA_OK : 1;
}

int ifa_model_get_expert_tensor(ifa_model *m, int layer, int expert, int tensor_id, int *dtype, void **dptr, size_t *rows, size_t *cols)
{
    IFA_REQUIRE(m && layer >= 0 && layer < m->cfg.layers, "ifa_model_get_expert_tensor: layer %d", layer);
    IFA_REQUIRE(tensor_id == T_W1 || tensor_id == T_W2 || tensor_id == T_W3, "ifa_model_get_expert_tensor: tensor id %d (w1 / w2 / w3 only)", tensor_id);
    const Layer &L = m->layers[(size_t)layer];
    IFA_REQUIRE(expert >= 0 && (size_t)expert * 3 + 2 < L.experts.size(), "ifa_model_get_expert_tensor: expert %d of layer %d", expert, layer);
    const Tensor &t = L.experts[(size_t)expert * 3 + (tensor_id == T_W1 ? 0 : (tensor_id == T_W2 ? 1 : 2))];
    if (dtype) *dtype = t.dtype;
    if (dptr) *dptr = t.data;
    if (rows) *rows = t.rows;
    if (cols) *cols = t.cols;
    return t.present() ? IFA_OK : 1;
}

}
```

### inferflow_amd/csrc/ifa_engine_decode.hip

```cpp
#include "ifa_engine_state.h"

namespace ifae {


__global__ void __launch_bounds__(256) k_touch(const uint8_t *__restrict__ p, size_t bytes, size_t stride, int *sink)
{
    size_t i = ((size_t)blockIdx.x * blockDim.x + threadIdx.x) * stride;
    int acc = 0;
    for (; i < bytes; i += (size_t)gridDim.x * blockDim.x * stride) acc += *reinterpret_cast<const int *>(p + i);
    if (acc == 0x7FFFFFFF) *sink = acc;
}

static long long *g_trace_ptr = nullptr;

bool fused_ok(const Tensor &t, bool long_rows)
{
    if (!t.present()) return false;
    if (fused_int8(t.dtype)) return t.tiled && (long_rows ? dec_gemv_supported_long(t.dtype, t.cols) : dec_gemv_supported(t.dtype, t.cols));
    return dec_gemv_h_supported(t.dtype, t.cols) && (long_rows || t.cols <= 8192);
}

template <int EPI, int NORM>
static int launch_dec_gemv(int w_dtype, const DecGemvParams &P, int wgs_per_cu_opt, hipStream_t s)
{
    if (!fused_int8(w_dtype) && w_dtype != Q3H_NATIVE) {
        if constexpr (NORM == 2 || epi_is_moe(EPI)) return ifa_fail(IFA_ERR_STATE, "fused GEMV: dtype %d has no kernel for this launch", w_dtype);
        else return dec_gemv_h_launch(w_dtype, EPI, NORM, P, s);
    }
    return dec_gemv_launch(w_dtype, EPI, NORM, P, wgs_per_cu_opt, s, g_trace_ptr);
}

int lmhead_grid(const DecLmHeadParams &P, int wgs_per_cu_opt)
{
    const int nj = (P.cols / 8 + 63) / 64;
    const int R = nj <= 4 ? 2 : 1;
    const int nbatch = (P.rows + R - 1) / R;
    const int per_cu = wgs_per_cu_opt > 0 ? wgs_per_cu_opt : 2;
    return std::max(1, std::min(num_cus() * per_cu, (nbatch + DEC_WAVES - 1) / DEC_WAVES));
}

template <int NJ>
static void lmhead_go(int nj, int norm, dim3 grid, size_t smem, hipStream_t s, const DecLmHeadParams &P, const DecStepTail *Z)
{
    if constexpr (NJ <= 16) {
        constexpr int R = NJ <= 4 ? 2 : 1;
        if (nj != NJ) return lmhead_go<NJ + 1>(nj, norm, grid, smem, s, P, Z);
        if (Z) { if (norm) k_dec_lmhead_tail<NJ, R, 1><<<grid, dim3(DEC_THREADS), smem, s>>>(P, *Z); else k_dec_lmhead_tail<NJ, R, 0><<<grid, dim3(DEC_THREADS), smem, s>>>(P, *Z); }
        else if (norm) k_dec_lmhead_f16<NJ, R, 1><<<grid, dim3(DEC_THREADS), smem, s>>>(P);
        else k_dec_lmhead_f16<NJ, R, 0><<<grid, dim3(DEC_THREADS), smem, s>>>(P);
    }
}

int launch_lmhead(const DecLmHeadParams &P, int norm, int wgs_per_cu_opt, hipStream_t s, const DecStepTail *Z)
{
    const int nj = (P.cols / 8 + 63) / 64;
    if (P.cols % 8 != 0 || nj < 1 || nj > 16) return ifa_fail(IFA_ERR_ARG, "fused lm_head supports cols %% 8 == 0 and <= 8192 (got %d)", P.cols);
    dim3 grid((unsigned)lmhead_grid(P, wgs_per_cu_opt));
    const size_t smem = (((size_t)P.cols * 2 + 15) & ~(size_t)15) + 132 * 4 + 16;
    lmhead_go<1>(nj, norm, grid, smem, s, P, Z);
    IFA_LAUNCH_CHECK();
    return IFA_OK;
}

bool has_post_norms(const ifa_model *m)
{
    for (const Layer &L : m->layers) if (L.t[T_ATTN_POST_NORM].present() || L.t[T_FFN_POST_NORM].present()) return true;
    return false;
}

bool fused_supported(const ifa_model *m, std::string *why)
{
    const ifa_model_config &c = m->cfg;
    auto fail = [&](const char *s) { if (why) *why = s; return false; };
    if (has_post_norms(m)) return fail("post norms (self_attn.post_norm / feed_forward.post_norm) use the op-by-op path");
    if (c.experts > 64 || (c.experts > 0 && (c.moe_top_k < 1 || c.moe_top_k > 8))) return fail("MoE: experts / top_k out of range");
    if ((scale_on(c.attn_out_scale) || scale_on(c.ffn_out_scale) || scale_on(c.out_scale)) && c.tp_size > 1)
        return fail("output scales (attn_out_scale / ffn_out_scale / out_scale) on a partitioned model use the op-by-op path");
    if (c.experts > 0 && (c.norm_kind != 0 || c.parallel_attn || c.share_input)) return fail("MoE layers need the sequential RMS-norm wiring");
    if (!c.full_quant_gemv) return fail("full_quant_gemv disabled");
    if (c.head_dim != 32 && c.head_dim != 48 && c.head_dim != 64 && c.head_dim != 80 && c.head_dim != 96 && c.head_dim != 128)
        return fail("fused attention supports head_dim 32/48/64/80/96/128");
    if (c.kv_dtype == Q8_B32T2 && c.head_dim % 32 != 0) return fail("Q8 KV needs head_dim % 32 == 0");
    if (dec_attn_pv_smem(c.head_dim, c.max_ctx, DEC_ATTN_MAX_SPLITS) > IFA_LDS_LIMIT) return fail("max_context_len too large for the fused attention kernels' LDS (decode falls back to the op-by-op path)");
    if (c.dim % 32 != 0 || c.ffn % 32 != 0) return fail("dim/ffn must be multiples of 32");
    if (c.dim > 8192) return fail("fused norm prologue supports dim <= 8192");
    for (const Layer &L : m->layers) {
        const bool moe = c.experts > 0 && L.t[T_MOE_GATE].present();
        if (moe) {
            if ((int)L.experts.size() != c.experts * 3 || !L.moe_table) return fail("MoE: expert tensors missing");
            for (int e = 0; e < c.experts; e++)
                for (int k = 0; k < 3; k++) {
                    const Tensor &t = L.experts[(size_t)e * 3 + k];
                    if (!t.present() || !t.tiled || !(k == 1 ? dec_gemv_supported_long(t.dtype, t.cols) : dec_gemv_supported(t.dtype, t.cols)))
                        return fail("MoE: expert weights must be in an int8-GEMV format");
                    if (!same_fmt(t.dtype, L.experts[(size_t)(k == 1 ? 1 : 0)].dtype) || t.rows != L.experts[(size_t)k].rows) return fail("MoE: experts differ in dtype / shape");
                }
        }
        const int ids_dense[] = {T_WQ, T_WK, T_WV, T_WO, T_W1, T_W2};
        const int ids_moe[] = {T_WQ, T_WK, T_WV, T_WO};
        const int *ids = moe ? ids_moe : ids_dense;
        const int n_ids = moe ? 4 : 6;
        for (int ii = 0; ii < n_ids; ii++) {
            const int id = ids[ii];
            const Tensor &t = L.t[id];
            if (!t.present()) return fail("fused path: a layer's weight matrix is missing");
            const bool plain_input = id == T_WO || id == T_W2;
            if (!fused_ok(t, plain_input)) return fail("fused GEMV: columns out of range for this weight format (or cols % 8 != 0 for fp16 activations)");
        }
        if (L.t[T_W3].present() && (!fused_ok(L.t[T_W3], false) || !same_fmt(L.t[T_W3].dtype, L.t[T_W1].dtype))) return fail("w1/w3 dtype mismatch");
        if (!L.t[T_ATTN_NORM].present()) return fail("pre-norm weights required");
        if (!L.t[T_FFN_NORM].present() && !c.parallel_attn) return fail("ffn pre-norm weights required");
    }
    const Tensor &lm = m->g[T_LM_HEAD];
    if (!lm.present()) {  }
    else if (lm.dtype == F16) {
        if (lm.cols > 8192 || lm.cols % 8 != 0) return fail("fused F16 lm_head needs cols <= 8192");
    } else if (!fused_ok(lm, false) || !m->g[T_OUT_NORM].present()) {
        return fail("fused lm_head: columns out of range for its weight format (or no output norm)");
    }
    if (m->g[T_EMBD].present() && m->g[T_EMBD].dtype != F16) return fail("F16 embeddings required");
    return true;
}

int sep_norm(ifa_model *m, const half_t *x, const Tensor &w, const Tensor &b, half_t *dst)
{
    return ifa_layernorm(m->cfg.norm_kind, x, 1, (size_t)m->cfg.dim, w.data, b.data, 0.0f, m->cfg.eps, dst, (ifa_stream)m->stream);
}

static bool qkv_attn_layer_ok(const ifa_model *m, int l, int *gk_out, int *rw_out)
{
    const ifa_model_config &c = m->cfg;
    const Layer &L = m->layers[(size_t)l];
    if (c.norm_kind != 0 || c.tp_size > 1) return false;
    const Tensor &wq = L.t[T_WQ], &wk = L.t[T_WK], &wv = L.t[T_WV];
    if (!wq.present() || !wk.present() || !wv.present() || !wq.tiled || !wk.tiled || !wv.tiled) return false;
    if (!fused_int8(wq.dtype) || !same_fmt(wq.dtype, wk.dtype) || !same_fmt(wq.dtype, wv.dtype)) return false;
    if ((int)wq.rows != c.heads * c.head_dim || (int)wk.rows != c.kv_heads * c.head_dim || (int)wv.rows != c.kv_heads * c.head_dim) return false;
    return dec_qkv_attn_supported(wq.dtype, (int)wq.cols, c.heads, c.kv_heads, c.head_dim, num_cus(), gk_out, rw_out);
}

static int chain_level(const ifa_model *m)
{
    const ifa_model_config &c = m->cfg;
    if (c.norm_kind != 0 || c.tp_size > 1 || c.experts != 0 || c.parallel_attn || c.share_input) return 0;
    int level = 2;
    for (int l = 0; level && l < c.layers; l++) {
        const Layer &L = m->layers[(size_t)l];
        const Tensor &wo = L.t[T_WO], &w1 = L.t[T_W1], &w3 = L.t[T_W3], &w2 = L.t[T_W2];
        if (!w1.present() || !w1.tiled || !w3.present() || !w3.tiled || !w2.present() || !w2.tiled || !L.t[T_FFN_NORM].present()
            || (int)w1.cols != c.dim || (int)w2.rows != c.dim || w2.cols != w1.rows || w3.rows != w1.rows || !same_fmt(w1.dtype, w3.dtype)
            || !dec_chain_supported(w1.dtype, w2.dtype, w1.dtype, c.dim, (int)w1.rows, false, c.dim, num_cus()))
            level = 0;
        else if (level == 2 && (!wo.present() || !wo.tiled || (int)wo.rows != c.dim
                                || !dec_chain_supported(w1.dtype, w2.dtype, wo.dtype, c.dim, (int)w1.rows, true, (int)wo.cols, num_cus())))
            level = 1;
    }
    return level;
}

static DecRouteFacts route_facts(const ifa_model *m, int reach, bool own_launches)
{
    const ifa_model_config &c = m->cfg;
    DecRouteFacts f;
    f.head_dim = c.head_dim; f.heads = c.heads; f.kv_heads = c.kv_heads; f.max_ctx = c.max_ctx; f.kv_q8 = c.kv_dtype == Q8_B32T2;
    f.reach = reach;
    f.attn_split_ctx = m->opt_attn_split_ctx; f.attn_nsplits = m->opt_attn_nsplits; f.attn_kt = m->opt_attn_kt; f.attn_unload = m->opt_attn_unload;
    f.fuse_attn = m->opt_fuse_attn; f.fuse_ffn = m->opt_fuse_ffn; f.attn_q8 = m->opt_attn_q8;
    f.waits = waits_enabled(); f.num_cus = num_cus(); f.visible_cus = visible_cus();
    f.have_attq = m->attq ? 1 : 0; f.own_launches = own_launches;
    f.tail_layers_ok = f.fuse_attn && f.waits;
    for (int l = 0; f.tail_layers_ok && l < c.layers; l++) if (!qkv_attn_layer_ok(m, l, &f.gk, &f.rw)) f.tail_layers_ok = 0;
    f.chain_level = (f.fuse_ffn && f.waits && !own_launches) ? chain_level(m) : 0;
    return f;
}

int decode_route_ready(ifa_model *m, int reach, bool own_launches)
{
    const ifa_model_config &c = m->cfg;
    const DecRoute route = plan_decode_route(route_facts(m, reach, own_launches));
    m->route_reach = reach;
    if (!(route == m->route)) { m->route = route; drop_graphs(m); }
    if (route.kind == DEC_ROUTE_FUSED_TAIL && !m->qa_gran) {
        const size_t n = (size_t)c.layers * (size_t)(c.heads + 2 * c.kv_heads) * c.head_dim;
        DevBuf<unsigned long long> gran; DevBuf<unsigned> call, err;
        int rc;
        if ((rc = gran.alloc(n)) || (rc = call.alloc(4)) || (rc = err.alloc(4))) return rc;
        IFA_HIP_CHECK(hipMemsetAsync(gran, 0, n * 8, m->stream));
        IFA_HIP_CHECK(hipMemsetAsync(call, 0, 16, m->stream));
        IFA_HIP_CHECK(hipMemsetAsync(err, 0, 16, m->stream));
        m->qa_gran = std::move(gran); m->qa_call = std::move(call); m->qa_err = std::move(err);
        IFA_HIP_CHECK(hipStreamSynchronize(m->stream));
    }
    if (route.chain && !m->ch_gran) {
        const size_t n = (size_t)c.layers * (size_t)(c.dim + (int)m->layers[0].t[T_W1].rows);
        DevBuf<uint32_t> gran, flags; DevBuf<unsigned> call, err;
        int rc;
        if ((rc = gran.alloc(n)) || (rc = flags.alloc((size_t)c.layers * 2 * 1024))) return rc;
        IFA_HIP_CHECK(hipMemsetAsync(gran, 0, n * 4, m->stream));
        IFA_HIP_CHECK(hipMemsetAsync(flags, 0, (size_t)c.layers * 2 * 1024 * 4, m->stream));
        if (!m->qa_call) { if ((rc = call.alloc(4))) return rc; IFA_HIP_CHECK(hipMemsetAsync(call, 0, 16, m->stream)); }
        if (!m->qa_err) { if ((rc = err.alloc(4))) return rc; IFA_HIP_CHECK(hipMemsetAsync(err, 0, 16, m->stream)); }
        m->ch_gran = std::move(gran); m->ch_flags = std::move(flags);
        if (call) m->qa_call = std::move(call);
        if (err) m->qa_err = std::move(err);
        IFA_HIP_CHECK(hipStreamSynchronize(m->stream));
    }
    return IFA_OK;
}

void qkv_params(ifa_model *m, int l, const half_t *x, DecGemvParams &P)
{
    const ifa_model_config &c = m->cfg;
    Layer &L = m->layers[(size_t)l];
    memset(&P, 0, sizeof(P));
    P.x = x; P.norm_w = (const half_t *)L.t[T_ATTN_NORM].data; P.norm_b = (const half_t *)L.t[T_ATTN_NORM_B].data;
    P.multi_base = c.attn_norm_base; P.eps = c.eps; P.cols = c.dim; P.nblk = c.dim / 32;
    if (c.parallel_attn) P.xn_out = m->xn;
    const int ids[3] = {T_WQ, T_WK, T_WV}; const int bids[3] = {T_WQ_B, T_WK_B, T_WV_B};
    const size_t QDd = (size_t)c.heads * c.head_dim, KVDd = (size_t)c.kv_heads * c.head_dim;
    half_t *outs[3] = {m->dqkv, m->dqkv + QDd, m->dqkv + QDd + KVDd};
    for (int i = 0; i < 3; i++) {
        P.W0[i] = wbytes(L.t[ids[i]]); P.b0[i] = (const half_t *)L.t[bids[i]].data;
        P.y[i] = outs[i]; P.rows[i] = (int)L.t[ids[i]].rows;
    }
    P.nsets = 3;
}

int launch_qkv_attn(ifa_model *m, int l, const half_t *x, unsigned tag_add)
{
    const ifa_model_config &c = m->cfg;
    Layer &L = m->layers[(size_t)l];
    DecGemvParams P; qkv_params(m, l, x, P);
    DecAttnParams A; attn_params(m, l, A);
    DecQkvAttnExtra E; memset(&E, 0, sizeof(E));
    E.gran = m->qa_gran + (size_t)l * (size_t)(c.heads + 2 * c.kv_heads) * c.head_dim;
    const DecRoute &R = m->route;
    E.epoch = m->qa_call; E.epoch_add = tag_add; E.err = m->qa_err; E.timeout_us = m->opt_fuse_attn_timeout_us; E.gk = R.gk; E.unload = R.ul;
    return dec_qkv_attn_launch(L.t[T_WQ].dtype, 1, A.kv_q8 != 0, R.pb, R.kt != 0, R.ul != 0, P, A, E, c.max_ctx, m->stream);
}

int launch_qkv(ifa_model *m, int l, const half_t *x)
{
    const ifa_model_config &c = m->cfg;
    Layer &L = m->layers[(size_t)l];
    DecGemvParams P; qkv_params(m, l, x, P);
    const bool std_norm = c.norm_kind != 0;
    if (std_norm) {
        int rc = sep_norm(m, x, L.t[T_ATTN_NORM], L.t[T_ATTN_NORM_B], m->xn);
        if (rc) return rc;
        P.x = m->xn; P.norm_w = nullptr; P.norm_b = nullptr; P.xn_out = nullptr;
    }
    if (m->pend.on && !std_norm) {
        P.x = m->pend.x; P.x_add = m->pend.add; P.x_add_bias = m->pend.bias; P.xsum_out = m->pend.out;
        m->pend.on = false;
    }
    auto go = [&](int dtype, const DecGemvParams &Q) {
        if (std_norm) return launch_dec_gemv<EPI_PLAIN, 0>(dtype, Q, m->opt_rpw_qkv, m->stream);
        return launch_dec_gemv<EPI_PLAIN, 1>(dtype, Q, m->opt_rpw_qkv, m->stream);
    };
    if (same_fmt(L.t[T_WQ].dtype, L.t[T_WK].dtype) && same_fmt(L.t[T_WQ].dtype, L.t[T_WV].dtype)) return go(L.t[T_WQ].dtype, P);
    const int ids[3] = {T_WQ, T_WK, T_WV};
    for (int i = 0; i < 3; i++) {
        DecGemvParams Q = P;
        Q.nsets = 1; Q.W0[0] = P.W0[i]; Q.b0[0] = P.b0[i]; Q.y[0] = P.y[i]; Q.rows[0] = P.rows[i];
        if (i > 0) {
            Q.xn_out = nullptr;
            if (P.x_add) { Q.x = P.xsum_out; Q.x_add = nullptr; Q.x_add_bias = nullptr; Q.xsum_out = nullptr; }
        }
        int rc = go(L.t[ids[i]].dtype, Q);
        if (rc) return rc;
    }
    return IFA_OK;
}

void attn_params(ifa_model *m, int l, DecAttnParams &A)
{
    const ifa_model_config &c = m->cfg;
    Layer &L = m->layers[(size_t)l];
    const int rope_dims = (int)(c.head_dim * c.partial_rotary + 0.5f);
    memset(&A, 0, sizeof(A));
    A.q = m->dqkv; A.k_new = m->dqkv + (size_t)c.heads * c.head_dim; A.v_new = A.k_new + (size_t)c.kv_heads * c.head_dim; A.kcache = (uint8_t *)L.kcache; A.vcache = (uint8_t *)L.vcache;
    A.state = m->state; A.rope_tab = m->rope_tab; A.heads = c.heads; A.kv_heads = c.kv_heads;
    A.kv_q8 = c.kv_dtype == Q8_B32T2; A.kq_scale = c.use_alibi ? 1.0f : c.kq_scale;
    A.rope_order = c.rope_order; A.rope_cols = rope_dims;
    A.alibi = c.use_alibi; A.alibi_base = c.tp_rank * c.heads; A.alibi_total = c.heads * std::max(1, c.tp_size);
    A.out = m->att; A.max_ctx = c.max_ctx; A.xq = (c.head_dim % 32 == 0) ? m->attq : nullptr; A.trace = g_trace_ptr;
}

int launch_attn(ifa_model *m, int l)
{
    const ifa_model_config &c = m->cfg;
    const bool unplanned = m->route.kind == DEC_ROUTE_FUSED_TAIL || (m->route.lds_attn | m->route.lds_pv) == 0;
    const DecRoute R = unplanned ? plan_decode_route(route_facts(m, m->route_reach, true)) : m->route;
    hipStream_t s = m->stream;
    DecAttnParams A; attn_params(m, l, A);
    if (R.kind == DEC_ROUTE_SPLIT) {
        if (R.error) return ifa_fail(IFA_ERR_ARG, "fused attention: max_context_len %d needs %d bytes of LDS per workgroup", c.max_ctx, R.lds_pv);
        DecAttnSplitWs ws = m->attn_ws; ws.nsplits = R.nsplits;
        const dim3 g2((unsigned)c.heads, (unsigned)R.nsplits);
        return attn_dispatch(c.head_dim, A.kv_q8 != 0, [&](auto hd, auto q8) {
            constexpr int HD = decltype(hd)::value; constexpr bool Q8 = decltype(q8)::value;
            int rc;
            if ((rc = launch_lds(k_dec_attn_scores<HD, Q8>, g2, dim3(256), (size_t)R.lds_scores, s, A, ws))) return rc;
            if ((rc = launch_lds(k_dec_attn_pv<HD, Q8>, g2, dim3(256), (size_t)R.lds_pv, s, A, ws))) return rc;
            return launch_lds(k_dec_attn_combine<HD>, dim3((unsigned)c.heads), dim3(HD), 0, s, ws, m->att.get(), A.xq, c.heads);
        });
    }
    return attn_dispatch(c.head_dim, A.kv_q8 != 0, [&](auto hd, auto q8) {
        constexpr int HD = decltype(hd)::value; constexpr bool Q8 = decltype(q8)::value;
        constexpr bool pow2 = HD == 32 || HD == 64 || HD == 128;
        auto go = [&](auto pb, auto kt) -> int {
            constexpr int PB = decltype(pb)::value; constexpr bool KT = decltype(kt)::value;
            if constexpr ((PB != 256 && !pow2) || (KT && (Q8 || !pow2)))
                return ifa_fail(IFA_ERR_ARG, "fused attention: no instance for head_dim %d, Q8 cache %d, %d-row bucket, K tile %d", HD, (int)Q8, PB, (int)KT);
            else
                return launch_lds(k_dec_attn<HD, Q8, false, PB, KT>, dim3((unsigned)c.heads), dim3(256), (size_t)R.lds_attn, s, A.q, A.kcache, A.vcache, A.heads, A.kv_heads, A);
        };
        auto by_kt = [&](auto pb) { return R.kt ? go(pb, std::true_type{}) : go(pb, std::false_type{}); };
        using std::integral_constant;
        return R.pb == 64 ? by_kt(integral_constant<int, 64>{}) : R.pb == 128 ? by_kt(integral_constant<int, 128>{}) : by_kt(integral_constant<int, 256>{});
    });
}

static int native_fmt(const ifa_model *m, const Tensor &t, const uint8_t *&w)
{
    if (m->opt_q3h_native && t.q3hn && t.dtype == Q3H_B64T1) { w = (const uint8_t *)t.q3hn; return Q3H_NATIVE; }
    return t.dtype;
}

void wo_params(ifa_model *m, int l, const half_t *x, half_t *partial, DecGemvParams &P)
{
    Layer &L = m->layers[(size_t)l];
    memset(&P, 0, sizeof(P));
    P.x = m->att; P.cols = (int)L.t[T_WO].cols; P.nblk = P.cols / 32; P.eps = m->cfg.eps;
    P.W0[0] = wbytes(L.t[T_WO]); P.rows[0] = (int)L.t[T_WO].rows; P.nsets = 1;
    if (partial) { P.y[0] = partial; return; }
    P.b0[0] = (const half_t *)L.t[T_WO_B].data;
    P.y[0] = m->a; P.residual = x;
    if (scale_on(m->cfg.attn_out_scale)) P.pre_scale = m->cfg.attn_out_scale;
}

int launch_wo(ifa_model *m, int l, const half_t *x, half_t *partial)
{
    Layer &L = m->layers[(size_t)l];
    DecGemvParams P; wo_params(m, l, x, partial, P);
    const bool preq = m->attq && m->opt_attn_q8 && m->cfg.head_dim % 32 == 0 && P.cols == m->cfg.heads * m->cfg.head_dim && fused_int8(L.t[T_WO].dtype)
        && dec_gemv_supported(L.t[T_WO].dtype, (size_t)P.cols);
    if (preq) P.x = reinterpret_cast<const half_t *>(m->attq.get());
    const int dto = native_fmt(m, L.t[T_WO], P.W0[0]);
    const bool plain = partial || m->cfg.parallel_attn || m->cfg.share_input;
    if (preq) return plain ? launch_dec_gemv<EPI_PLAIN, 2>(dto, P, m->opt_rpw_wo, m->stream) : launch_dec_gemv<EPI_RESIDUAL, 2>(dto, P, m->opt_rpw_wo, m->stream);
    return plain ? launch_dec_gemv<EPI_PLAIN, 0>(dto, P, m->opt_rpw_wo, m->stream) : launch_dec_gemv<EPI_RESIDUAL, 0>(dto, P, m->opt_rpw_wo, m->stream);
}

void moe_params(ifa_model *m, Layer &L, DecGemvParams &P, int slot, int tab_off)
{
    P.w_table = (const uint8_t *const *)L.moe_table;
    P.moe_sel = m->moe_route;
    P.moe_w = reinterpret_cast<const half_t *>(reinterpret_cast<const char *>(m->moe_route.get()) + 32);
    P.moe_acc = m->f;
// ... 134 lines not shown
int step_tail_ready(ifa_model *m)
{
    const int want = step_tail_ok(m) ? 1 : 0;
    if (want != m->st_on) { m->st_on = want; drop_graphs(m); }
    if (!want) return IFA_OK;
    const int grid = lmhead_grid(lm_params(m, m->x, nullptr), m->opt_rpw_lm);
    int rc;
    if ((size_t)grid > m->st_keys.cap()) {
        IFA_HIP_CHECK(hipStreamSynchronize(m->stream));
        if ((rc = m->st_keys.alloc((size_t)grid))) return rc;
    }
    if (!m->st_counter) {
        if ((rc = m->st_counter.alloc(4))) return rc;
        IFA_HIP_CHECK(hipMemsetAsync(m->st_counter, 0, 16, m->stream));
    }
    return IFA_OK;
}

int launch_lm_tail(ifa_model *m, const half_t *x)
{
    const ifa_model_config &c = m->cfg;
    const DecLmHeadParams H = lm_params(m, x, nullptr);
    DecStepTail Z; memset(&Z, 0, sizeof(Z));
    Z.state = m->state; Z.ring = ifa_model::RING; Z.keys = m->st_keys; Z.counter = m->st_counter;
    Z.embd = (const half_t *)m->g[T_EMBD].data; Z.vocab = (int)m->g[T_EMBD].rows; Z.x_out = m->x;
    Z.rope_tab = c.rope_order ? m->rope_tab : nullptr; Z.head_dim = c.head_dim; Z.theta = c.rope_theta;
    Z.rope_dims = (int)(c.head_dim * c.partial_rotary + 0.5f); Z.embd_scale = c.embd_scale;
    return launch_lmhead(H, m->g[T_OUT_NORM].present() ? 1 : 0, m->opt_rpw_lm, m->stream, &Z);
}

int launch_gather(ifa_model *m)
{
    const ifa_model_config &c = m->cfg;
    k_dec_gather<<<dim3(2), dim3(256), 0, m->stream>>>(m->opt_debug_hidden_in ? nullptr : (const half_t *)m->g[T_EMBD].data, m->state, c.dim, (int)m->g[T_EMBD].rows, m->x,
                                                       c.rope_order ? m->rope_tab : nullptr, c.head_dim, c.rope_theta,
                                                       (int)(c.head_dim * c.partial_rotary + 0.5f), c.embd_scale);
    IFA_LAUNCH_CHECK();
    return IFA_OK;
}

int launch_lm(ifa_model *m, const half_t *x, half_t *logits_out)
{
    const ifa_model_config &c = m->cfg;
    const Tensor &lmt = m->g[T_LM_HEAD];
    if (lmt.dtype != F16) {
        DecGemvParams P; memset(&P, 0, sizeof(P));
        P.x = x; P.norm_w = (const half_t *)m->g[T_OUT_NORM].data; P.norm_b = (const half_t *)m->g[T_OUT_NORM_B].data;
        P.eps = c.eps; P.cols = c.dim; P.xn_out = m->xn; P.multi_base = c.out_norm_base;
        P.W0[0] = wbytes(lmt); P.rows[0] = (int)lmt.rows; P.nsets = 1;
        P.y[0] = logits_out ? logits_out : m->logits;
        return launch_dec_gemv<EPI_PLAIN, 1>(lmt.dtype, P, m->opt_rpw_lm, m->stream);
    }
    if (c.norm_kind != 0 && m->g[T_OUT_NORM].present()) {
        int rc = sep_norm(m, x, m->g[T_OUT_NORM], m->g[T_OUT_NORM_B], m->xn);
        if (rc) return rc;
        DecLmHeadParams H2; memset(&H2, 0, sizeof(H2));
        H2.x = m->xn; H2.eps = c.eps; H2.cols = c.dim; H2.W = (const half_t *)lmt.data; H2.logits = logits_out ? logits_out : m->logits;
        H2.rows = (int)lmt.rows;
        return launch_lmhead(H2, 0, m->opt_rpw_lm, m->stream);
    }
    return launch_lmhead(lm_params(m, x, logits_out), m->g[T_OUT_NORM].present() ? 1 : 0, m->opt_rpw_lm, m->stream);
}

int enqueue_fused_step(ifa_model *m, int tail)
{
    const ifa_model_config &c = m->cfg;
    hipStream_t s = m->stream;
    int rc;
    if ((!m->st_on || tail == STEP_TAIL_SAMPLED) && (rc = launch_gather(m))) return rc;
    half_t *x = m->x, *xnext = m->x2;
    const int l_first = std::min(std::max(m->opt_debug_layer0, 0), c.layers - 1);
    const int n_layers = (m->opt_debug_layers > 0 && l_first + m->opt_debug_layers < c.layers) ? l_first + m->opt_debug_layers : c.layers;
    for (int l = l_first; l < n_layers; l++) {
        if (m->route.kind == DEC_ROUTE_FUSED_TAIL) {
            if ((rc = launch_qkv_attn(m, l, x))) return rc;
        } else {
            if ((rc = launch_qkv(m, l, x))) return rc;
            if ((rc = launch_attn(m, l))) return rc;
        }
        if (m->route.chain) {
            if (m->route.chain == 1 && (rc = launch_wo(m, l, x))) return rc;
            if ((rc = launch_chain(m, l, x, xnext))) return rc;
            std::swap(x, xnext);
            continue;
        }
        if ((rc = launch_wo(m, l, x))) return rc;
        Layer &L = m->layers[(size_t)l];
        if (c.experts > 0 && L.t[T_MOE_GATE].present()) {
            if ((rc = launch_moe_router(m, l))) return rc;
            for (int k0 = 0; k0 < c.moe_top_k; k0 += 3) {
                const int ns = std::min(3, c.moe_top_k - k0);
                if ((rc = launch_ffn13(m, l, k0, nullptr, ns))) return rc;
                for (int k = k0; k < k0 + ns; k++)
                    if ((rc = launch_w2(m, l, xnext, nullptr, k, k + 1 == c.moe_top_k, nullptr, k - k0))) return rc;
            }
        } else {
            const bool extra = c.parallel_attn || c.share_input;
            if ((rc = launch_ffn13(m, l, -1, x))) return rc;
            if ((rc = launch_w2(m, l, xnext, nullptr, -1, false, extra ? x : nullptr))) return rc;
        }
        std::swap(x, xnext);
    }
    if (tail == STEP_TAIL_SAMPLED) return sampled_tail_enqueue(m, x);
    if (m->st_on) return launch_lm_tail(m, x);
    if ((rc = launch_lm(m, x))) return rc;
    k_dec_argmax_advance<<<dim3(1), dim3(1024), 0, s>>>(m->logits, (int)m->g[T_LM_HEAD].rows, m->state, ifa_model::RING);
    IFA_LAUNCH_CHECK();
    return IFA_OK;
}

}

extern "C" {

int ifa_model_decode(ifa_model *m, int first_token, int start_pos, int n_steps, int *out_tokens_host, float *elapsed_ms)
{
    return decode_impl(m, first_token, start_pos, n_steps, out_tokens_host, elapsed_ms, false);
}

int ifa_model_decode_prepare(ifa_model *m, int start_pos, int n_steps)
{
    return decode_impl(m, 0, start_pos, n_steps, nullptr, nullptr, true);
}

}

namespace ifae {

static int qa_err_check(ifa_model *m, int qerr)
{
    if (qerr == 0) return IFA_OK;
    (void)hipMemsetAsync(m->qa_err, 0, 16, m->stream);
    (void)hipStreamSynchronize(m->stream);
    m->opt_fuse_attn = 0; m->opt_fuse_ffn = 0;
    drop_graphs(m);
    waits_disable("the fused QKV + attention launch timed out waiting for sibling workgroups");
    return ifa_fail(IFA_ERR_STATE, "fused decode launch: a wait for another workgroup's rows timed out (code 0x%x: 0x5_ q | k | v / attention output, 0x6_ Wo output, 0x9_ chained FFN launch); "
                    "the results of this call are not valid -- repeat it: options fuse_attn / fuse_ffn are off now (five-launch step)", (unsigned)qerr);
}

static int capture_steps(ifa_model *m, int n, hipGraph_t *graph, hipGraphExec_t *exec)
{
    int rc = IFA_OK;
    IFA_HIP_CHECK(hipStreamSynchronize(m->stream));
    IFA_HIP_CHECK(hipStreamBeginCapture(m->stream, hipStreamCaptureModeThreadLocal));
    for (int i = 0; i < n && !rc; i++) rc = enqueue_fused_step(m);
    hipGraph_t gph = nullptr;
    hipError_t e = hipStreamEndCapture(m->stream, &gph);
    if (rc) { if (gph) (void)hipGraphDestroy(gph); return rc; }
    if (e != hipSuccess) return ifa_fail(IFA_ERR_HIP, "hipStreamEndCapture: %s", hipGetErrorString(e));
    if (*graph) (void)hipGraphDestroy(*graph);
    *graph = gph;
    IFA_HIP_CHECK(hipGraphInstantiate(exec, gph, nullptr, nullptr, 0));
    return IFA_OK;
}

int decode_impl(ifa_model *m, int first_token, int start_pos, int n_steps, int *out_tokens_host, float *elapsed_ms, bool prepare_only,
                const SampledCall *sc)
{
    IFA_REQUIRE(m && m->finalized, "ifa_model_decode: model not finalized");
    IFA_REQUIRE(n_steps > 0 && n_steps <= ifa_model::RING, "ifa_model_decode: n_steps %d (max %d per call)", n_steps, ifa_model::RING);
    IFA_REQUIRE(start_pos >= 0 && start_pos + n_steps <= m->cfg.max_ctx, "ifa_model_decode: positions [%d,%d) exceed max_ctx %d",
                start_pos, start_pos + n_steps, m->cfg.max_ctx);
    IFA_REQUIRE(m->g[T_EMBD].present() && m->g[T_LM_HEAD].present(), "ifa_model_decode: embeddings / lm_head missing (pipeline stage worker)");
    IFA_HIP_CHECK(hipSetDevice(m->cfg.device));
    std::string why;
    const bool exact = m->opt_exact_order != 0;
    if (exact || !m->opt_fused || m->opt_perf_stat || !fused_supported(m, &why)) {
        if (prepare_only) return IFA_OK;
        int tok = first_token;
        for (int i = 0; i < n_steps; i++) {
            int nt = 0;
            int rc = exact ? forward_exact(m, tok, start_pos + i, nullptr, &nt) : forward_ops(m, &tok, 1, start_pos + i, nullptr, &nt);
            if (rc) return rc;
            if (out_tokens_host) out_tokens_host[i] = nt;
            tok = nt;
        }
        if (elapsed_ms) *elapsed_ms = -1.0f;
        return IFA_OK;
    }
    static const bool trace_host = getenv("IFA_TRACE_DECODE") != nullptr;
    const auto th0 = std::chrono::steady_clock::now();
    auto th = [&](const char *what) {
        if (trace_host) fprintf(stderr, "decode-host %-28s %8.1f us\n", what, std::chrono::duration<double, std::micro>(std::chrono::steady_clock::now() - th0).count());
    };
    int rc = ensure_scratch(m, 1);
    if (rc) return rc;
    if (m->opt_q3h_native && (rc = ensure_q3hn(m))) return rc;
    hipStream_t s = m->stream;
    if ((rc = decode_route_ready(m, start_pos + n_steps))) return rc;
    const bool waits_on = m->route.kind == DEC_ROUTE_FUSED_TAIL || m->route.chain;
    if ((rc = step_tail_ready(m))) return rc;
    m->host_pinned[0] = first_token; m->host_pinned[1] = start_pos; m->host_pinned[2] = 0;
    IFA_HIP_CHECK(hipMemcpyAsync(m->state, m->host_pinned, 3 * sizeof(int), hipMemcpyHostToDevice, s));
    if (waits_on) {
        m->qa_calls = (m->qa_calls % 4000u) + 1u;
        m->host_pinned[6] = (int)m->qa_calls;
        IFA_HIP_CHECK(hipMemcpyAsync(m->qa_call, m->host_pinned + 6, sizeof(int), hipMemcpyHostToDevice, s));
    }
    hipGraphExec_t samp_exec = nullptr;
    if (sc) {
        if ((rc = sampled_prepare(m, *sc))) return rc;
        if (m->opt_graph && (rc = sampled_graph(m, &samp_exec))) return rc;
        if ((rc = sampled_begin(m, *sc))) return rc;
    }
    if (!sc && m->opt_graph && !m->graph_exec && (rc = capture_steps(m, 1, &m->graph, &m->graph_exec))) return rc;
    const int S = m->opt_graph_steps;
    if (!sc && m->opt_graph && S > 1 && n_steps >= S && (!m->graph_exec_n || m->graph_n_steps != S)) {
        if (m->graph_exec_n) { (void)hipGraphExecDestroy(m->graph_exec_n); m->graph_exec_n = nullptr; }
        if (m->graph_n) { (void)hipGraphDestroy(m->graph_n); m->graph_n = nullptr; }
        if ((rc = capture_steps(m, S, &m->graph_n, &m->graph_exec_n))) return rc;
        m->graph_n_steps = S;
    }
    if (prepare_only) return IFA_OK;
    th("state copies enqueued");
    hipEvent_t e0 = nullptr, e1 = nullptr;
    if (elapsed_ms) { IFA_HIP_CHECK(hipEventCreate(&e0)); IFA_HIP_CHECK(hipEventCreate(&e1)); IFA_HIP_CHECK(hipEventRecord(e0, s)); }
    th("events created, first recorded");
    if (!sc && m->st_on && (rc = launch_gather(m))) return rc;
    for (int i = 0; i < n_steps;) {
        if (sc) {
            if (samp_exec) IFA_HIP_CHECK(hipGraphLaunch(samp_exec, s));
            else if ((rc = enqueue_fused_step(m, STEP_TAIL_SAMPLED))) return rc;
            i++;
            continue;
        }
        if (m->opt_graph && m->graph_exec_n && m->graph_n_steps == S && S > 1 && n_steps - i >= S) { IFA_HIP_CHECK(hipGraphLaunch(m->graph_exec_n, s)); i += S; continue; }
        if (m->opt_graph) IFA_HIP_CHECK(hipGraphLaunch(m->graph_exec, s));
        else if ((rc = enqueue_fused_step(m))) return rc;
        i++;
    }
    th("steps enqueued");
    if (elapsed_ms) IFA_HIP_CHECK(hipEventRecord(e1, s));
    if (!sc && (rc = pool_enqueue(m, m->logits, 1))) return rc;
    if (sc && (rc = sampled_copy_back(m))) return rc;
    IFA_HIP_CHECK(hipMemcpyAsync(m->host_pinned + 8, m->state + 8, sizeof(int) * (size_t)n_steps, hipMemcpyDeviceToHost, s));
    int *qerr = m->host_pinned + 8 + ifa_model::RING;
    qerr[0] = 0;
    if (waits_on) IFA_HIP_CHECK(hipMemcpyAsync(qerr, m->qa_err, 4, hipMemcpyDeviceToHost, s));
    th("copies back enqueued");
    IFA_HIP_CHECK(hipStreamSynchronize(s));
    th("stream synchronised");
    if ((rc = qa_err_check(m, qerr[0])) || (sc && (rc = sampled_finish(m, *sc)))) {
        if (elapsed_ms) { (void)hipEventDestroy(e0); (void)hipEventDestroy(e1); }
        return rc;
    }
    if (elapsed_ms) { IFA_HIP_CHECK(hipEventElapsedTime(elapsed_ms, e0, e1)); (void)hipEventDestroy(e0); (void)hipEventDestroy(e1); }
    if (out_tokens_host) memcpy(out_tokens_host, m->host_pinned + 8, sizeof(int) * (size_t)n_steps);
    th("done");
    return IFA_OK;
}

}

extern "C" {

int ifa_model_time_kernel(ifa_model *m, int which, int iters, float *avg_us)
{
    IFA_REQUIRE(m && m->finalized && avg_us, "ifa_model_time_kernel: bad arguments");
    IFA_REQUIRE(iters > 0 && which >= 0 && which <= 9, "ifa_model_time_kernel: which %d iters %d", which, iters);
    IFA_HIP_CHECK(hipSetDevice(m->cfg.device));
    std::string why;
    if (!fused_supported(m, &why)) return ifa_fail(IFA_ERR_STATE, "fused path unavailable: %s", why.c_str());
    int rc = ensure_scratch(m, 1);
    if (rc) return rc;
    if (m->opt_q3h_native && (rc = ensure_q3hn(m))) return rc;
    hipStream_t s = m->stream;
    m->host_pinned[0] = 1; m->host_pinned[1] = std::min(m->cfg.max_ctx - 1, 64); m->host_pinned[2] = 0;
    IFA_HIP_CHECK(hipMemcpyAsync(m->state, m->host_pinned, 3 * sizeof(int), hipMemcpyHostToDevice, s));
    auto touch_layer = [&](int l) {
        const int ids[] = {T_WQ, T_WK, T_WV, T_WO, T_W1, T_W3, T_W2};
        for (int id : ids) {
            const Tensor &t = m->layers[(size_t)l].t[id];
            if (!t.tiled) continue;
            const size_t bytes = t.rows * ifa_tiled_row_bytes(t.dtype, t.cols);
            k_touch<<<dim3(8), dim3(256), 0, s>>>((const uint8_t *)t.tiled, bytes, (size_t)m->opt_touch_stride, m->state + 7);
        }
    };
    if ((rc = decode_route_ready(m, m->route_reach))) return rc;
    if (which == 9 && !m->route.chain) return ifa_fail(IFA_ERR_STATE, "chained FFN launch unavailable for this model / option set");
    if (which == 7 && m->route.kind != DEC_ROUTE_FUSED_TAIL) return ifa_fail(IFA_ERR_STATE, "fused QKV + attention launch unavailable for this model / option set");
    auto one = [&](int i) -> int {
        if (which == 7) return launch_qkv_attn(m, i % m->cfg.layers, m->x, (unsigned)(i + 1));
        if (which == 9) return launch_chain(m, i % m->cfg.layers, m->x, m->x2, (unsigned)(i + 1));
        const int l = m->opt_bench_mode == 1 ? 0 : i % m->cfg.layers;
        if (m->opt_bench_mode == 2) touch_layer(l);
        switch (which) {
        case 0: return launch_qkv(m, l, m->x);
        case 1: return launch_attn(m, l);
        case 2: return launch_wo(m, l, m->x);
        case 3: return launch_ffn13(m, l, -1, m->x);
        case 4: return launch_w2(m, l, m->x2);
        default: return launch_lm(m, m->x);
        }
    };
    if ((rc = launch_gather(m))) return rc;
    for (int i = 0; i < 3; i++) if ((rc = one(i))) return rc;
    if (m->opt_trace) {
        if (!m->trace && (rc = m->trace.alloc(2048 * 8))) return rc;
        IFA_HIP_CHECK(hipMemsetAsync(m->trace, 0, sizeof(long long) * 2048 * 8, s));
        g_trace_ptr = m->trace;
    }
    hipEvent_t e0, e1;
    IFA_HIP_CHECK(hipEventCreate(&e0)); IFA_HIP_CHECK(hipEventCreate(&e1));
    IFA_HIP_CHECK(hipEventRecord(e0, s));
    for (int i = 0; i < iters; i++) if ((rc = one(i))) return rc;
    IFA_HIP_CHECK(hipEventRecord(e1, s));
    IFA_HIP_CHECK(hipStreamSynchronize(s));
    g_trace_ptr = nullptr;
    float ms = 0;
    IFA_HIP_CHECK(hipEventElapsedTime(&ms, e0, e1));
    (void)hipEventDestroy(e0); (void)hipEventDestroy(e1);
    *avg_us = ms * 1000.0f / (float)iters;
    return IFA_OK;
}

}
```

### inferflow_amd/csrc/ifa_engine_sampled.hip

```cpp
#include <algorithm>
#include "ifa_engine_state.h"
#include "ifa_sample_rule.h"

namespace ifa {
int topk_pool_rows(const void *logits, size_t row_stride, const int *row_idx_dev, size_t rows, size_t n, int k, const unsigned *excl,
                   int *ids_out, void *vals_out, int *count_out, hipStream_t s);
int logit_adjust_rows(const void *logits, size_t row_stride, const int *row_idx_dev, const int *state_slot_dev, size_t rows, size_t n,
                      const unsigned *state_dev, const float *bias_dev, const float *params_dev, void *out, hipStream_t s);
int sample_pool_launch(const int *counts, const int *ids, const void *vals, size_t rows, int k_stride, const ifa_sample_params *params,
                       unsigned long long *rng, int *tokens_out, int *index_out, float *weights_out, int *err, int *state, int ring, hipStream_t s);
}

namespace ifae {

enum { SB_PARAMS = 0, SB_RNG = 6, SB_SLOT = 8, SB_ERR = 9, SB_TOKEN = 10, SB_INDEX = 11, SB_WORDS = 16 };
static_assert(sizeof(ifa_sample_params) <= SB_RNG * sizeof(int), "ifa_sample_params outgrew its words of the block");

int sampled_prepare(ifa_model *m, const SampledCall &sc)
{
    const size_t V = m->g[T_LM_HEAD].rows;
    int rc;
    if (!m->samp_blk.cap()) {
        IFA_HIP_CHECK(hipStreamSynchronize(m->stream));
        if ((rc = m->samp_blk.reserve(SB_WORDS))) return rc;
    }
    if ((rc = pool_reserve(m, 1, sc.p->pool_size))) return rc;
    if (sc.state_slot >= 0 && V > m->la_adj.cap()) {
        IFA_HIP_CHECK(hipStreamSynchronize(m->stream));
        if (m->la_adj.alloc(8 * V)) return ifa_fail(IFA_ERR_NOMEM, "ifa_model_decode_sampled: no memory for the adjusted logits row");
    }
    m->samp_k = sc.p->pool_size; m->samp_armed = sc.state_slot >= 0;
    return IFA_OK;
}

int sampled_tail_enqueue(ifa_model *m, const half_t *x)
{
    const size_t V = m->g[T_LM_HEAD].rows;
    const int k = m->samp_k;
    hipStream_t s = m->stream;
    int *blk = m->samp_blk.dev;
    int rc;
    if ((rc = launch_lm(m, x))) return rc;
    const half_t *src = m->logits;
    if (m->samp_armed) {
        if ((rc = ifa::logit_adjust_rows(m->logits, V, nullptr, blk + SB_SLOT, 1, V, m->la_state, m->la_bias, m->la_params, m->la_adj, s))) return rc;
        src = m->la_adj;
    }
    int *counts = (int *)m->pool_blk.dev.get(), *ids = counts + 1;
    uint16_t *vals = (uint16_t *)(ids + k);
    if ((rc = ifa::topk_pool_rows(src, V, nullptr, 1, V, k, m->pool_excl, ids, vals, counts, s))) return rc;
    if ((rc = ifa::sample_pool_launch(counts, ids, vals, 1, k, (const ifa_sample_params *)(blk + SB_PARAMS), (unsigned long long *)(blk + SB_RNG),
                                      blk + SB_TOKEN, blk + SB_INDEX, nullptr, blk + SB_ERR, m->state, ifa_model::RING, s))) return rc;
    if (m->samp_armed && (rc = ifa_logit_state_add(blk + SB_SLOT, m->state, 1, V, m->la_slots, m->la_state, (ifa_stream)s))) return rc;
    return IFA_OK;
}

int sampled_graph(ifa_model *m, hipGraphExec_t *exec_out)
{
    const int key = (m->cur_slot << 10) | (m->samp_k << 1) | (m->samp_armed ? 1 : 0);
    ifa_model::SampGraph &G = m->samp_graphs[key];
    const void *now[8] = {m->samp_blk.dev.get(), m->pool_blk.dev.get(), m->pool_excl.get(), m->la_state.get(), m->la_bias.get(), m->la_params.get(),
                          m->la_adj.get(), m->logits};
    if (G.exec && !std::equal(now, now + 8, G.ptrs)) { (void)hipGraphExecDestroy(G.exec); G.exec = nullptr; }
    if (!G.exec) {
        hipStream_t s = m->stream;
        IFA_HIP_CHECK(hipStreamSynchronize(s));
        IFA_HIP_CHECK(hipStreamBeginCapture(s, hipStreamCaptureModeThreadLocal));
        const int rc = enqueue_fused_step(m, STEP_TAIL_SAMPLED);
        hipGraph_t gph = nullptr;
        const hipError_t e = hipStreamEndCapture(s, &gph);
        if (rc) { if (gph) (void)hipGraphDestroy(gph); return rc; }
        if (e != hipSuccess) return ifa_fail(IFA_ERR_HIP, "hipStreamEndCapture: %s", hipGetErrorString(e));
        const hipError_t ei = hipGraphInstantiate(&G.exec, gph, nullptr, nullptr, 0);
        (void)hipGraphDestroy(gph);
        if (ei != hipSuccess) { G.exec = nullptr; return ifa_fail(IFA_ERR_HIP, "hipGraphInstantiate: %s", hipGetErrorString(ei)); }
        std::copy(now, now + 8, G.ptrs);
    }
    *exec_out = G.exec;
    return IFA_OK;
}

void sampled_drop_graphs(ifa_model *m)
{
    for (auto &kv : m->samp_graphs) if (kv.second.exec) (void)hipGraphExecDestroy(kv.second.exec);
    m->samp_graphs.clear();
}

int sampled_begin(ifa_model *m, const SampledCall &sc)
{
    int *pin = m->samp_blk.pin;
    memset(pin, 0, sizeof(int) * SB_WORDS);
    memcpy(pin + SB_PARAMS, sc.p, sizeof(ifa_sample_params));
    memcpy(pin + SB_RNG, sc.rng, sizeof(unsigned long long));
    pin[SB_SLOT] = std::max(sc.state_slot, 0);
    IFA_HIP_CHECK(hipMemcpyAsync(m->samp_blk.dev, pin, sizeof(int) * SB_WORDS, hipMemcpyHostToDevice, m->stream));
    return IFA_OK;
}

int sampled_copy_back(ifa_model *m)
{
    IFA_HIP_CHECK(hipMemcpyAsync(m->samp_blk.pin + SB_RNG, m->samp_blk.dev + SB_RNG, sizeof(int) * (SB_WORDS - SB_RNG), hipMemcpyDeviceToHost, m->stream));
    return IFA_OK;
}

int sampled_finish(ifa_model *m, const SampledCall &sc)
{
    const int *pin = m->samp_blk.pin;
    if (pin[SB_ERR] != 0)
        return ifa_fail(IFA_ERR_STATE, "ifa_model_decode_sampled: step %d had no token to draw (an empty candidate pool); the results of this call are not valid", pin[SB_ERR] - 1);
    memcpy(sc.rng, pin + SB_RNG, sizeof(unsigned long long));
    return IFA_OK;
}

}

extern "C" {

int ifa_model_decode_sampled(ifa_model *m, int first_token, int start_pos, int n_steps, const ifa_sample_params *p,
                             unsigned long long *rng_state_inout, int state_slot, int *out_tokens_host, float *elapsed_ms)
{
    using namespace ifae;
    const char *who = "ifa_model_decode_sampled";
    IFA_REQUIRE(m && m->finalized, "%s: model not finalized", who);
    IFA_REQUIRE(p && rng_state_inout, "%s: null pointer", who);
    IFA_REQUIRE(ifa_sr::sr_strategy_ok(p->strategy_id), "%s: strategy %d is not one of 1 sample.std, 2 greedy, 3 top_k, 4 sample.top_p, 7 min_p", who, p->strategy_id);
    IFA_REQUIRE(p->pool_size >= 1 && p->pool_size <= IFA_POOL_MAX, "%s: pool_size %d outside 1..%d", who, p->pool_size, IFA_POOL_MAX);
    if (m->cfg.tp_size > 1 || m->topo) return ifa_fail(IFA_ERR_STATE, "%s: the vocabulary of a partitioned worker is sharded; the draw runs on a single-device worker", who);
    if (!m->g[T_LM_HEAD].present() || !m->g[T_EMBD].present()) return ifa_fail(IFA_ERR_STATE, "%s: embeddings / lm_head missing (pipeline stage worker)", who);
    if (m->opt_exact_order) return ifa_fail(IFA_ERR_STATE, "%s: option exact_order steps on the host; the sampled step is the fused, captured one", who);
    if (m->opt_perf_stat) return ifa_fail(IFA_ERR_STATE, "%s: option perf_stat times the op-by-op step; the sampled step is the fused, captured one", who);
    std::string why;
    if (!m->opt_fused || !fused_supported(m, &why)) return ifa_fail(IFA_ERR_STATE, "%s: the fused decode step does not cover this model (%s)", who, m->opt_fused ? why.c_str() : "option fused = 0");
    IFA_REQUIRE(state_slot >= -1 && (state_slot < 0 || (size_t)state_slot < m->la_slots), "%s: state slot %d has no logit state (ifa_model_logit_state_reset first)", who, state_slot);
    SampledCall sc;
    sc.p = p; sc.rng = rng_state_inout; sc.state_slot = state_slot;
    return decode_impl(m, first_token, start_pos, n_steps, out_tokens_host, elapsed_ms, false, &sc);
}

}
```

### inferflow_amd/csrc/ifa_engine_state.h

```cpp
#pragma once
#include <chrono>
#include <cstdlib>
#include <cstring>
#include <map>
#include <string>
#include <type_traits>
#include <vector>
#include "ifa_host.h"
#include "ifa_buf_hip.h"
#include "ifa_decode_kernels.h"
#include "ifa_decode_attn.h"
#include "ifa_decode_gemv.h"
#include "ifa_moe.h"
#include "ifa_gemm_rows_mfma.h"
#include "ifa_gemm_big.h"
#include "ifa_decode_lmhead_tail.h"
#include "ifa_decode_singles.h"
#include "ifa_decode_qkv_attn.h"
#include "ifa_decode_chain.h"
#include "ifa_prompt_route.h"

using namespace ifa;

namespace ifae {


enum { T_EMBD = 0, T_OUT_NORM = 1, T_OUT_NORM_B = 2, T_LM_HEAD = 3,
       T_ATTN_NORM = 10, T_ATTN_NORM_B = 11, T_WQ = 12, T_WK = 13, T_WV = 14, T_WO = 15,
       T_FFN_NORM = 16, T_FFN_NORM_B = 17, T_W1 = 18, T_W2 = 19, T_W3 = 20, T_MOE_GATE = 21,
       T_WQ_B = 22, T_WK_B = 23, T_WV_B = 24, T_WO_B = 25, T_W1_B = 26, T_W2_B = 27, T_W3_B = 28,
       T_ATTN_POST_NORM = 29, T_ATTN_POST_NORM_B = 30, T_FFN_POST_NORM = 31, T_FFN_POST_NORM_B = 32,
       T_MAX = 36 };

struct Tensor {
    int dtype = -1;
    DevBuf<void> data;
    DevBuf<void> tiled;
    DevBuf<void> mo;
    DevBuf<void> q3hn;
    DevBuf<void> x32;
    size_t rows = 0, cols = 0;
    bool present() const { return data != nullptr; }
};

struct Layer {
    Tensor t[T_MAX];
    std::vector<Tensor> experts;
    DevBuf<void *> moe_table;
    DevBuf<void *> moe_table_aos;
    DevBuf<void *> moe_table_mo;
    DevBuf<void> kcache, vcache;
};

struct Scratch {
    DevBuf<half_t> x, x2, xn, hn, q, k, v;
    DevBuf<half_t> dqkv;
    DevBuf<half_t> bqkv;
    DevBuf<float> brope;
    DevBuf<half_t> att, a, f, t1, t2, logits;
    DevBuf<uint8_t> xq;
    DevBuf<int8_t> attq;
    DevBuf<half_t> moe_gate, moe_out;
    DevBuf<half_t> moe_in, moe_wdev;
    DevBuf<int> moe_route;
    DevBuf<int> moe_idx; PinBuf<void> moe_pin;
    DevBuf<int> moe_sel, moe_epos, moe_counts;
    DevBuf<half_t> moe_selw, moe_g1, moe_g3, moe_gin, moe_gout;
    DevBuf<uint8_t> moe_xq_in, moe_xq_mid;
    DevBuf<void> moe_tiles, moe_singles, moe_smalls;
    DevBuf<int> tokens_dev;
    DevBuf<half_t> pn;
};


}
using namespace ifae;

struct ifa_model : Scratch {
    ifa_model_config cfg;
    std::vector<Layer> layers;
    Tensor g[10];
    hipStream_t stream = nullptr;
    hipStream_t side_stream = nullptr; Event ev_fork, ev_join; int opt_moe_overlap = 1;
    bool own_stream = true;
    bool finalized = false;
    int opt_moe_device = 1;
    DevBuf<int> state;
    DevBuf<float> rope_tab;
    DevBuf<long long> trace;
    int opt_trace = 0, opt_bench_mode = 0, opt_touch_stride = 65536;
    PinBuf<int> host_pinned;
    int scratch_tokens = 0;
    size_t kv_row_bytes = 0;
    hipGraph_t graph = nullptr;
    hipGraphExec_t graph_exec = nullptr;
    hipGraph_t graph_n = nullptr; hipGraphExec_t graph_exec_n = nullptr; int graph_n_steps = 0, opt_graph_steps = 1;
    struct PendingAdd { const half_t *x = nullptr, *add = nullptr, *bias = nullptr; half_t *out = nullptr; bool on = false; } pend;
    int opt_tp_fuse_add = 1;
    DevPin<void> batch_tab;
    std::map<int, hipGraphExec_t> batch_graphs;
    std::map<int, hipGraphExec_t> draft_graphs;
    DecAttnSplitWs attn_ws = {nullptr, nullptr, nullptr, 8};
    DevBuf<half_t> attn_ws_S; DevBuf<float> attn_ws_lmax, attn_ws_opart;
    int opt_attn_unload = 1;
    int opt_attn_nsplits = 0;
    DecRoute route; int route_reach = 256;
    PromptRoute prompt_route;
    int opt_fuse_attn = 1, opt_fuse_attn_timeout_us = 20000;
    DevBuf<unsigned long long> qa_gran;
    DevBuf<unsigned> qa_call, qa_err; unsigned qa_calls = 0;
    int opt_fuse_ffn = 0, opt_chain_late_w2 = 0;
    int opt_q3h_native = 0;
    int opt_perf_stat = 0;
    struct PerfSpanRec { int key; hipEvent_t e0, e1; };
    std::vector<PerfSpanRec> perf_spans;
    std::vector<hipEvent_t> perf_pool;
    std::map<int, float> perf_map;
    int opt_exact_order = 0;
    DevBuf<float> exact_rope_tab;
    DevBuf<uint32_t> ch_gran, ch_flags;
    int opt_step_tail = 1, st_on = 0;
    DevBuf<unsigned long long> st_keys; DevBuf<unsigned> st_counter;
    int opt_attn_kt = 1;
    int opt_attn_split_ctx = -1, opt_batch_graph = 0, opt_gemm_rows = 1, opt_batch_fused = 1, opt_moe_router_fused = 1, opt_prefill_big = 1, opt_rows_mo = 1, opt_moe_singles = 1;
    struct KvSlot { std::vector<DevBuf<void>> k, v; hipGraph_t graph = nullptr; hipGraphExec_t exec = nullptr; };
    std::vector<KvSlot> slots;
    int cur_slot = 0;
    int opt_attn_q8 = 1;
    DevBuf<half_t> tp_a, tp_f, tp_hid, tp_logits;
    DevBuf<float> tp_best, tp_gather;
    DevBuf<int> tp_tok;
    hipGraph_t tp_graph = nullptr;
    hipGraphExec_t tp_graph_exec = nullptr;
    struct TpKey {
        unsigned long long tp = 0, world = 0; int tp_size = 0, stage = 0, n_stages = 0, prev = 0, next = 0, src = 0, voff = 0, force = 0, fuse = 0, slot = 0, oneshot = 0;
        bool operator==(const TpKey &o) const { return tp == o.tp && world == o.world && tp_size == o.tp_size && stage == o.stage && n_stages == o.n_stages
                && prev == o.prev && next == o.next && src == o.src && voff == o.voff && force == o.force && fuse == o.fuse && slot == o.slot
                && oneshot == o.oneshot; }
    } tp_key;
    const ifa_tp_topology *topo = nullptr;
    int opt_attn_post_as_residual = 1;
    int opt_fused = 1, opt_graph = 1, opt_rpw_qkv = 0, opt_rpw_wo = 0, opt_rpw_ffn = 0, opt_rpw_w2 = 0, opt_rpw_lm = 0;
    int opt_debug_layers = 0;
    int opt_debug_layer0 = 0, opt_debug_hidden_in = 0;
    int opt_prefill_big_min = 47;
    int opt_prefill_chunk = 1;
    int opt_prefill_mid = 1, opt_prefill_mid_max = 768;
    int opt_prefill_res_mid = 2048;
    int opt_rows_kparts = 1, opt_gemm_splitk = 1;
    int opt_debug_mo_alloc_fail = 0;
    struct PoolReq {
        int k = 0;
        int n_sel = 0;
        const int *rows_sel = nullptr;
        int chunk0 = 0; bool last_chunk = true;
        int done = 0;
        bool lse = false;
        std::vector<int> adj;
    } pool;
    DevBuf<unsigned> pool_excl;
    DevPin<void> pool_blk;
    DevPin<int> pool_idx;
    static constexpr int LA_RING = 8;
    DevBuf<unsigned> la_state; DevBuf<float> la_bias, la_params; size_t la_slots = 0;
    DevBuf<half_t> la_adj;
    std::vector<int> pool_adj_next;
    DevPin<int> la_ring; Event la_ev[LA_RING]; bool la_ev_used[LA_RING] = {}; unsigned la_calls = 0;
    DevPin<int> la_reset;
    int opt_pool_lse = 0;
    std::vector<float> pool_lse_last;
    DevBuf<float> lse_part;
    struct ScoreReq {
        int n = 0;
        int done = 0;
    } score;
    DevPin<int> score_tgt;
    DevPin<float> score_out;
    DevPin<void *> kvc_tab;
    std::vector<void *> kvc_tab_host;
    std::vector<DevPin<void *>> kvc_retired;
    DevBuf<float> kvs_rot;
    struct SampGraph { hipGraphExec_t exec = nullptr; const void *ptrs[8] = {}; };
    std::map<int, SampGraph> samp_graphs;
    DevPin<int> samp_blk;
    int samp_k = 0; bool samp_armed = false;
    static constexpr int RING = 1024;
};


static inline bool is_q4(int dt) { return dt == Q4_B32T1A || dt == Q4_B32T1B; }

static inline bool rows_mo_fmt(int dt) { return is_q4(dt) || dt == Q4_B64T1 || dt == Q3H_B64T1; }

static inline bool scale_on(float s) { return s < 0.9999f || s > 1.0001f; }

static inline bool same_fmt(int a, int b) { return a == b || (is_q4(a) && is_q4(b)); }


static inline int num_cus() { return dec_num_cus(); }


static inline bool fused_int8(int w_dtype) { return ax8_eligible(w_dtype); }

static inline const uint8_t *wbytes(const Tensor &t) { return (const uint8_t *)(fused_int8(t.dtype) ? t.tiled.get() : t.data.get()); }


extern "C" int ifa_add_layernorm(int kind, const void *a, const void *addend, size_t rows, size_t cols, const void *w, const void *b,
                                 float multi_base, float eps, void *sum_out, void *y, ifa_stream stream);

extern "C" int ifa_rope_qk_store(void *q, void *k, const void *v, int head_dim, int heads, int kv_heads, int tokens, int pos0, float theta,
                                 int order, float partial_rotary_factor, void *kcache_rows, void *vcache_rows, size_t cache_row_elems,
                                 ifa_stream stream);

extern "C" int ifa_activation_mul(int kind, const void *a, const void *b, size_t n, void *c, ifa_stream stream);

extern "C" int ifa_argmax_rows(const void *logits, size_t n, size_t row_stride, size_t rows, int *out_dev, const int *excluded_dev, ifa_stream stream);

extern "C" int ifa_gemm_rows_q4(const void *Wt_tiled, size_t rows, size_t cols, const void *x_f16, size_t tokens,
                                const void *bias_f16, void *y_f16, ifa_stream stream);

namespace ifa {
int moe_build_lists(const int *sel, const void *wsel, int T, int top_k, int E, int tile_rows, int small_max, int *idx, void *wdev, int *epos,
                    MoeTile *tiles, MoeSingle *singles, MoeTile *smalls, int *counts, hipStream_t s);
int gemm_rows_q4_grouped_cap(size_t cols);
bool gemm_rows_use_mfma();
bool gemm_rows_mfma_ok(size_t rows, size_t cols, size_t tokens);
int gemm_rows_mfma_grouped(const MoeSmallGroup &grp, size_t rows, size_t cols, const void *X, void *Y, int max_groups, int max_rows, hipStream_t s);
int gemm_rows_mo_grouped(const MoeSmallGroup &grp, size_t rows, size_t cols, const void *X, void *Y, int max_groups, int glu, int act_kind, hipStream_t s);
int gemm_rows_q4_grouped(const MoeSmallGroup &grp, size_t rows, size_t cols, const void *X, void *Y, int max_groups, hipStream_t s);
int moe_gather(const void *src, const int *idx, const int *counts, int max_entries, int dim, void *dst, hipStream_t s);
int moe_combine(const void *y, const int *epos, const void *wsel, int T, int top_k, int dim, void *out, hipStream_t s, const void *residual = nullptr);
int gemm_q_grouped(int w_dtype, const MoeGroup &grp, size_t N, size_t K, const void *X, void *Y, int max_tiles, int tile_rows, hipStream_t s);
int gemv_ax8_grouped(int w_dtype, const MoeGroup &grp, size_t rows, size_t cols, const void *xq8_rows, void *y_rows, int max_singles,
                     hipStream_t s);
}


struct AttnRowH { const void *kc, *vc; int n_ctx, pad; };

extern "C" int ifa_attention_rows(const void *q, const void *rows_dev, int kv_dtype, int n_rows, int max_ctx, int heads, int kv_heads,
                                  int head_dim, float kq_scale, int alibi, int alibi_base_head, int alibi_total_heads, void *out,
                                  ifa_stream stream);

extern "C" int ifa_rope_rows(void *x, int head_dim, int heads, int tokens, const int *positions_dev, float theta, int order,
                             float partial_rotary_factor, ifa_stream stream);

namespace ifae {

template <class K, class... Args>
static int launch_lds(K kern, dim3 grid, dim3 block, size_t smem, hipStream_t s, Args... args)
{
    if (smem > 48 * 1024) IFA_HIP_CHECK(hipFuncSetAttribute((const void *)kern, hipFuncAttributeMaxDynamicSharedMemorySize, (int)smem));
    kern<<<grid, block, smem, s>>>(args...);
    IFA_LAUNCH_CHECK();
    return IFA_OK;
}

template <class F>
static int attn_dispatch(int head_dim, bool q8, F &&f)
{
    using std::integral_constant;
    switch (head_dim) {
    case 32: return q8 ? f(integral_constant<int, 32>{}, std::true_type{}) : f(integral_constant<int, 32>{}, std::false_type{});
    case 64: return q8 ? f(integral_constant<int, 64>{}, std::true_type{}) : f(integral_constant<int, 64>{}, std::false_type{});
    case 96: return q8 ? f(integral_constant<int, 96>{}, std::true_type{}) : f(integral_constant<int, 96>{}, std::false_type{});
    case 128: return q8 ? f(integral_constant<int, 128>{}, std::true_type{}) : f(integral_constant<int, 128>{}, std::false_type{});
    case 48: if (!q8) return f(integral_constant<int, 48>{}, std::false_type{}); break;
    case 80: if (!q8) return f(integral_constant<int, 80>{}, std::false_type{}); break;
    }
    return ifa_fail(IFA_ERR_ARG, "fused attention: head_dim %d with %s cache", head_dim, q8 ? "a Q8" : "an F16");
}

void drop_graphs(ifa_model *m);
int perf_begin(ifa_model *m, int key);
void perf_end(ifa_model *m, int idx);
int perf_collect(ifa_model *m);
struct PerfSpan {
    ifa_model *m; int idx;
    PerfSpan(ifa_model *mm, int key, bool on = true) : m(mm), idx(on ? perf_begin(mm, key) : -1) {}
    ~PerfSpan() { done(); }
    void done() { if (idx >= 0) { perf_end(m, idx); idx = -1; } }
};
void *kv_ptr(ifa_model *m, size_t layer, int slot, bool is_v);
int kv_copy_table(ifa_model *m, int a, int b);
int ensure_mo(ifa_model *m);
int ensure_mo_build(ifa_model *m);
int ensure_x32(ifa_model *m);
int ensure_q3hn(ifa_model *m);
int ensure_scratch(ifa_model *m, int T);
bool fused_ok(const Tensor &t, bool long_rows);
int lmhead_grid(const DecLmHeadParams &P, int wgs_per_cu_opt);
int launch_lmhead(const DecLmHeadParams &P, int norm, int wgs_per_cu_opt, hipStream_t s, const DecStepTail *Z = nullptr);
bool has_post_norms(const ifa_model *m);
bool fused_supported(const ifa_model *m, std::string *why);
int sep_norm(ifa_model *m, const half_t *x, const Tensor &w, const Tensor &b, half_t *dst);
void attn_params(ifa_model *m, int l, DecAttnParams &A);
int decode_route_ready(ifa_model *m, int reach, bool own_launches = false);
void qkv_params(ifa_model *m, int l, const half_t *x, DecGemvParams &P);
int launch_qkv_attn(ifa_model *m, int l, const half_t *x, unsigned tag_add = 0);
int launch_qkv(ifa_model *m, int l, const half_t *x);
int launch_attn(ifa_model *m, int l);
int launch_wo(ifa_model *m, int l, const half_t *x, half_t *partial = nullptr);
void moe_params(ifa_model *m, Layer &L, DecGemvParams &P, int slot, int tab_off);
int launch_ffn13(ifa_model *m, int l, int moe_slot = -1, const half_t *x_layer = nullptr, int moe_nslots = 1);
int launch_w2(ifa_model *m, int l, half_t *xnext, half_t *partial = nullptr, int moe_slot = -1, bool moe_last = false,
                     const half_t *residual2 = nullptr, int moe_t1_slot = 0);
int launch_chain(ifa_model *m, int l, const half_t *x, half_t *xnext, unsigned tag_add = 0);
bool step_tail_ok(const ifa_model *m);
DecLmHeadParams lm_params(ifa_model *m, const half_t *x, half_t *logits_out);
int step_tail_ready(ifa_model *m);
int launch_lm_tail(ifa_model *m, const half_t *x);
int launch_gather(ifa_model *m);
int launch_lm(ifa_model *m, const half_t *x, half_t *logits_out = nullptr);
enum { STEP_TAIL_GREEDY = 0, STEP_TAIL_SAMPLED = 1 };
struct SampledCall { const ifa_sample_params *p = nullptr; unsigned long long *rng = nullptr; int state_slot = -1; };
int enqueue_fused_step(ifa_model *m, int tail = STEP_TAIL_GREEDY);
int decode_impl(ifa_model *m, int first_token, int start_pos, int n_steps, int *out_tokens_host, float *elapsed_ms, bool prepare_only,
                const SampledCall *sc = nullptr);
int sampled_prepare(ifa_model *m, const SampledCall &sc);
int sampled_tail_enqueue(ifa_model *m, const half_t *x);
int sampled_graph(ifa_model *m, hipGraphExec_t *exec_out);
void sampled_drop_graphs(ifa_model *m);
int sampled_begin(ifa_model *m, const SampledCall &sc);
int sampled_copy_back(ifa_model *m);
int sampled_finish(ifa_model *m, const SampledCall &sc);
int gather_rows(ifa_model *m, const half_t *src, const int *idx_dev, int T, int dim, int n_src, half_t *dst, float scale);
int matmul(ifa_model *m, const half_t *A, int T, const Tensor &W, const Tensor &bias, half_t *C);
int norm_rows(ifa_model *m, const half_t *x, int T, const Tensor &w, const Tensor &b, half_t *y, float base = 0.0f);
int ffn_dense(ifa_model *m, const half_t *x, int T, const Tensor &w1, const Tensor &b1, const Tensor &w3, const Tensor &b3,
                     const Tensor &w2, const Tensor &b2, half_t *out, int perf_base = 0);
int layer_tail_ops(ifa_model *m, int l, int T, half_t *&x, const half_t *attn_in, bool &xn_ready);
int prompt_route_ready(ifa_model *m, int T, int prefix_len, bool entry, PromptRoute &R);
int forward_ops(ifa_model *m, const int *tokens_host, int T, int prefix_len, void *logits_out, int *next_token, bool no_head = false,
                const PromptRoute *planned = nullptr);
int draft_kv_store_launch(ifa_model *m, int n, const half_t *k, const half_t *v, int stride, const void *rows_l);
int forward_batch(ifa_model *m, int n, const int *tokens_host, const int *pos_host, const int *slot_host, int *next_tokens,
                         void *logits_out, bool draft = false);
int pool_enqueue(ifa_model *m, const half_t *logits, int n_rows);
int pool_reserve(ifa_model *m, int n_sel, int k);
static constexpr size_t LSE_PART_FLOATS = 256;
int lse_part_reserve(ifa_model *m);
int score_enqueue(ifa_model *m, const half_t *logits, int n_rows);
int launch_moe_router(ifa_model *m, int l);
bool moe_device_ok(const ifa_model *m, const Layer &L);
int moe_ffn_device(ifa_model *m, Layer &L, const half_t *ff_n, int T, const half_t *pre_norm = nullptr, const half_t *residual = nullptr, half_t *out = nullptr);
int moe_ffn(ifa_model *m, Layer &L, const half_t *ff_n, int T);
int max_smalls_possible(bool rows_kernel, int E, int cap);
int ensure_side_stream(ifa_model *m);
bool moe_router_rows_ok(const ifa_model *m, const Layer &L, int T);
bool exact_supported(const ifa_model *m, std::string *why);
int forward_exact(ifa_model *m, int token, int pos, void *logits_out, int *next_token);
int tp_argmax_scratch(ifa_model *m, size_t n_rows);
int tp_pick_rows(ifa_model *m, const ifa_tp_topology &t, const half_t *shard, size_t row_stride, int shard_rows, int n_rows);
bool tp_merging(const ifa_model *m);
int tp_merge_rows(ifa_model *m, half_t *buf, int T, const Tensor &bias);
int tp_ready(ifa_model *m);
int tp_flush_pending(ifa_model *m);
int tp_buffers(ifa_model *m);
int tp_step(ifa_model *m, const ifa_tp_topology &t, int token, int pos, bool want_token = true, void *logits_copy = nullptr);
int tp_check(ifa_model *m, const ifa_tp_topology *topo, const char *who);
int tp_oneshot_status(ifa_model *m, const ifa_tp_topology &t, const char *who);

}
```

### inferflow_amd/worker.py

```python
import ctypes as C

import numpy as np

from . import _capi, dtypes as dt
from ._capi import ModelConfig, check, lib

T_EMBD, T_OUT_NORM, T_OUT_NORM_B, T_LM_HEAD = 0, 1, 2, 3
T_ATTN_NORM, T_ATTN_NORM_B, T_WQ, T_WK, T_WV, T_WO = 10, 11, 12, 13, 14, 15
T_FFN_NORM, T_FFN_NORM_B, T_W1, T_W2, T_W3, T_MOE_GATE = 16, 17, 18, 19, 20, 21
T_WQ_B, T_WK_B, T_WV_B, T_WO_B, T_W1_B, T_W2_B, T_W3_B = 22, 23, 24, 25, 26, 27, 28
T_ATTN_POST_NORM, T_ATTN_POST_NORM_B, T_FFN_POST_NORM, T_FFN_POST_NORM_B = 29, 30, 31, 32

_DEFAULTS = dict(norm_kind=0, act_kind=0, is_glu=1, rope_order=2, use_alibi=0, parallel_attn=0, share_input=0,
                 rope_theta=10000.0, partial_rotary=1.0, kq_scale=1.0, eps=1e-5, kv_dtype=dt.F16,
                 full_quant_gemv=1, experts=0, moe_top_k=0, moe_norm_topk=1, tp_rank=0, tp_size=1, device=0,
                 attn_norm_base=0.0, ffn_norm_base=0.0, out_norm_base=0.0, attn_out_scale=1.0, ffn_out_scale=1.0, out_scale=1.0,
                 embd_scale=0.0)


class DecodeWorker:
    def __init__(self, **kw):
        cfg = ModelConfig()
        vals = dict(_DEFAULTS)
        vals.update(kw)
# ... 55 lines not shown
    def kv_shift(self, slot, keep, discard, n_rows):
        check(lib().ifa_model_kv_shift(self._h, int(slot), int(keep), int(discard), int(n_rows)))

    def kv_shift_rows(self, kcache_ptr, vcache_ptr, table_ptr, keep, discard, n_rows):
        c = self.cfg
        kv_shift_rows(c.kv_dtype, kcache_ptr, vcache_ptr, c.kv_heads, c.head_dim, c.rope_order, int(c.head_dim * c.partial_rotary + 0.5), table_ptr,
                      keep, discard, n_rows, lib().ifa_model_stream(self._h))

    def sync(self):
        check(lib().ifa_stream_sync(C.c_void_p(lib().ifa_model_stream(self._h))))

    def decode_batch(self, tokens, positions, slots, logits_out=None):
        toks = np.ascontiguousarray(tokens, np.int32)
        pos = np.ascontiguousarray(positions, np.int32)
        sl = np.ascontiguousarray(slots, np.int32)
        out = np.zeros(toks.size, np.int32)
        check(lib().ifa_model_decode_batch(self._h, toks.size, toks.ctypes.data_as(C.c_void_p), pos.ctypes.data_as(C.c_void_p),
                                           sl.ctypes.data_as(C.c_void_p), out.ctypes.data_as(C.c_void_p),
                                           C.c_void_p(logits_out.data_ptr()) if logits_out is not None else None))
        return out

    def decode_draft(self, tokens, pos0, logits_out=None):
        toks = np.ascontiguousarray(tokens, np.int32)
        out = np.zeros(toks.size, np.int32)
        check(lib().ifa_model_decode_draft(self._h, toks.size, toks.ctypes.data_as(C.c_void_p), int(pos0), out.ctypes.data_as(C.c_void_p),
                                           C.c_void_p(logits_out.data_ptr()) if logits_out is not None else None))
        return out

    def decode(self, first_token, start_pos, n_steps, timed=True):
        out = np.zeros(n_steps, np.int32)
        ms = C.c_float(-1.0)
        check(lib().ifa_model_decode(self._h, int(first_token), int(start_pos), int(n_steps),
                                     out.ctypes.data_as(C.c_void_p), C.byref(ms) if timed else None))
        return out, ms.value

    def decode_sampled(self, first_token, start_pos, n_steps, params, rng_state, state_slot=-1, timed=True):
        out = np.zeros(n_steps, np.int32)
        ms = C.c_float(-1.0)
        st = C.c_ulonglong(int(rng_state))
        check(lib().ifa_model_decode_sampled(self._h, int(first_token), int(start_pos), int(n_steps), C.byref(params), C.byref(st), int(state_slot),
                                             out.ctypes.data_as(C.c_void_p), C.byref(ms) if timed else None))
        return out, st.value, ms.value

    def set_pool_excluded(self, ids):
        a = np.ascontiguousarray(ids, np.int32).reshape(-1)
        check(lib().ifa_model_set_pool_excluded(self._h, a.ctypes.data_as(C.c_void_p) if a.size else None, a.size))

    def decode_pool(self, token, pos, k):
        ids, vals = np.zeros(k, np.int32), np.zeros(k, np.uint16)
        nxt, cnt = C.c_int(-1), C.c_int(0)
        check(lib().ifa_model_decode_pool(self._h, int(token), int(pos), int(k), C.byref(nxt), ids.ctypes.data_as(C.c_void_p),
                                          vals.ctypes.data_as(C.c_void_p), C.byref(cnt)))
        return nxt.value, ids[:cnt.value].copy(), vals[:cnt.value].copy()

    def forward_pool(self, tokens, prefix_len, k, logits_out=None):
        toks = np.ascontiguousarray(tokens, np.int32)
        ids, vals = np.zeros(k, np.int32), np.zeros(k, np.uint16)
        nxt, cnt = C.c_int(-1), C.c_int(0)
        check(lib().ifa_model_forward_pool(self._h, toks.ctypes.data_as(C.c_void_p), toks.size, int(prefix_len),
                                           C.c_void_p(logits_out.data_ptr()) if logits_out is not None else None, int(k), C.byref(nxt),
                                           ids.ctypes.data_as(C.c_void_p), vals.ctypes.data_as(C.c_void_p), C.byref(cnt)))
        return nxt.value, ids[:cnt.value].copy(), vals[:cnt.value].copy()

    def decode_batch_pool(self, tokens, positions, slots, k, rows_sel):
        toks = np.ascontiguousarray(tokens, np.int32)
        pos = np.ascontiguousarray(positions, np.int32)
        sl = np.ascontiguousarray(slots, np.int32)
        sel = np.ascontiguousarray(rows_sel, np.int32).reshape(-1)
        out = np.zeros(toks.size, np.int32)
        ids, vals = np.zeros((max(sel.size, 1), k), np.int32), np.zeros((max(sel.size, 1), k), np.uint16)
        cnt = np.zeros(max(sel.size, 1), np.int32)
        check(lib().ifa_model_decode_batch_pool(self._h, toks.size, toks.ctypes.data_as(C.c_void_p), pos.ctypes.data_as(C.c_void_p),
                                                sl.ctypes.data_as(C.c_void_p), out.ctypes.data_as(C.c_void_p), int(k),
                                                sel.ctypes.data_as(C.c_void_p), sel.size, ids.ctypes.data_as(C.c_void_p),
                                                vals.ctypes.data_as(C.c_void_p), cnt.ctypes.data_as(C.c_void_p)))
        return out, [(ids[j, :cnt[j]].copy(), vals[j, :cnt[j]].copy()) for j in range(sel.size)]

    def pool_lse(self, cap=256):
        out, n = np.zeros(cap, np.float32), C.c_int(0)
        check(lib().ifa_model_pool_lse(self._h, out.ctypes.data_as(C.c_void_p), cap, C.byref(n)))
        return out[:n.value].copy()

    def decode_pool_lse(self, token, pos, k):
        self.set_option("pool_lse", 1)
        try:
            nxt, ids, vals = self.decode_pool(token, pos, k)
            return nxt, ids, vals, float(self.pool_lse()[0])
        finally:
            self.set_option("pool_lse", 0)

    def forward_pool_lse(self, tokens, prefix_len, k, logits_out=None):
        self.set_option("pool_lse", 1)
        try:
            nxt, ids, vals = self.forward_pool(tokens, prefix_len, k, logits_out)
            return nxt, ids, vals, float(self.pool_lse()[0])
        finally:
            self.set_option("pool_lse", 0)

    def decode_batch_pool_lse(self, tokens, positions, slots, k, rows_sel):
        self.set_option("pool_lse", 1)
        try:
            out, pools = self.decode_batch_pool(tokens, positions, slots, k, rows_sel)
            return out, pools, self.pool_lse(max(len(pools), 1))
        finally:
            self.set_option("pool_lse", 0)

    def logit_state_reset(self, kv_slot, prompt, rep=1.0, freq=0.0, pres=0.0, bias=None):
        pr = np.ascontiguousarray(prompt, np.int32).reshape(-1)
        items = sorted((bias or {}).items())
        ids = np.ascontiguousarray([k for k, _ in items], np.int32)
        vals = np.ascontiguousarray([v for _, v in items], np.float32)
        check(lib().ifa_model_logit_state_reset(self._h, int(kv_slot), pr.ctypes.data_as(C.c_void_p) if pr.size else None, pr.size, float(rep), float(freq),
                                                float(pres), ids.ctypes.data_as(C.c_void_p) if ids.size else None,
                                                vals.ctypes.data_as(C.c_void_p) if vals.size else None, ids.size))

    def logit_state_add(self, kv_slots, tokens):
        sl = np.ascontiguousarray(kv_slots, np.int32).reshape(-1)
        tk = np.ascontiguousarray(tokens, np.int32).reshape(-1)
        assert sl.size == tk.size
        check(lib().ifa_model_logit_state_add(self._h, sl.size, sl.ctypes.data_as(C.c_void_p), tk.ctypes.data_as(C.c_void_p)))

    def pool_adjust(self, state_slots):
        sl = np.ascontiguousarray(state_slots, np.int32).reshape(-1)
        check(lib().ifa_model_pool_adjust(self._h, sl.size, sl.ctypes.data_as(C.c_void_p) if sl.size else None))

    def forward_score(self, tokens, prefix_len, targets):
        toks = np.ascontiguousarray(tokens, np.int32)
        tg = np.ascontiguousarray(targets, np.int32).reshape(-1)
        assert tg.size == toks.size, (tg.size, toks.size)
        lse, tl = np.zeros(toks.size, np.float32), np.zeros(toks.size, np.float32)
        nxt = C.c_int(-1)
        check(lib().ifa_model_forward_score(self._h, toks.ctypes.data_as(C.c_void_p), toks.size, int(prefix_len), tg.ctypes.data_as(C.c_void_p),
                                            lse.ctypes.data_as(C.c_void_p), tl.ctypes.data_as(C.c_void_p), C.byref(nxt)))
        return nxt.value, lse, tl

    def decode_prepare(self, start_pos, n_steps):
        check(lib().ifa_model_decode_prepare(self._h, int(start_pos), int(n_steps)))

    def time_kernel(self, which, iters=200):
        us = C.c_float(0)
        check(lib().ifa_model_time_kernel(self._h, which, iters, C.byref(us)))
        return us.value

    ROUTE_FIELDS = ("kind", "nsplits", "pb", "kt", "ul", "gk", "rw", "chain", "split_threshold", "split", "lds_attn", "lds_scores", "lds_pv",
                    "error", "num_cus", "visible_cus", "waits")
    ROUTE_KINDS = ("one_workgroup", "split", "fused_tail")

    def decode_route(self):
        out = (C.c_int * len(self.ROUTE_FIELDS))()
        check(lib().ifa_model_decode_route(self._h, out, len(out)))
        d = dict(zip(self.ROUTE_FIELDS, out))
        d["kind"] = self.ROUTE_KINDS[d["kind"]]
        return d

    PROMPT_ROUTE_FIELDS = ("kind", "first_pass", "norm_fused", "res_mid") + tuple(
        p + "_" + k for p in ("qkv", "wo", "w13", "w2") for k in ("kernel", "src", "mo", "no_waits")) + ("need_mo", "need_x32")
    PROMPT_ROUTE_KINDS = ("exact", "op_by_op", "rows", "mid", "big")

    def prompt_route(self):
        out = (C.c_int * len(self.PROMPT_ROUTE_FIELDS))()
        check(lib().ifa_model_prompt_route(self._h, out, len(out)))
        d = dict(zip(self.PROMPT_ROUTE_FIELDS, out))
        d["kind"] = self.PROMPT_ROUTE_KINDS[d["kind"]]
        return d

    def get_tensor_host(self, layer, tid):
        d, p, r, c = C.c_int(), C.c_void_p(), C.c_size_t(), C.c_size_t()
        rc = lib().ifa_model_get_tensor(self._h, layer, tid, C.byref(d), C.byref(p), C.byref(r), C.byref(c))
        if rc == 1:
            return None
        check(rc)
        nbytes = r.value * dt.row_bytes(d.value, c.value)
        out = np.empty(nbytes, np.uint8)
        check(lib().ifa_memcpy_d2h(out.ctypes.data_as(C.c_void_p), p, nbytes, None))
        check(lib().ifa_stream_sync(None))
        if d.value == dt.F16:
            out = out.view(np.uint16)
        return d.value, out, r.value, c.value

    def get_expert_tensor_host(self, layer, expert, tid):
        d, p, r, c = C.c_int(), C.c_void_p(), C.c_size_t(), C.c_size_t()
        rc = lib().ifa_model_get_expert_tensor(self._h, layer, expert, tid, C.byref(d), C.byref(p), C.byref(r), C.byref(c))
        if rc == 1:
            return None
        check(rc)
        nbytes = r.value * dt.row_bytes(d.value, c.value)
        out = np.empty(nbytes, np.uint8)
        check(lib().ifa_memcpy_d2h(out.ctypes.data_as(C.c_void_p), p, nbytes, None))
        check(lib().ifa_stream_sync(None))
        return d.value, out, r.value, c.value

    def set_stream(self, stream_ptr):
        check(lib().ifa_model_set_stream(self._h, C.c_void_p(stream_ptr)))

    def tp_begin(self, token, pos):
        check(lib().ifa_model_tp_begin(self._h, int(token), int(pos)))

    def tp_begin_hidden(self, x_dev_f16, pos):
        check(lib().ifa_model_tp_begin_hidden(self._h, C.c_void_p(x_dev_f16.data_ptr()), int(pos)))

    def tp_hidden(self, x_out_dev_f16):
        check(lib().ifa_model_tp_hidden(self._h, C.c_void_p(x_out_dev_f16.data_ptr())))

    def tp_attn(self, layer, partial):
        check(lib().ifa_model_tp_attn(self._h, layer, C.c_void_p(partial.data_ptr())))

    def tp_post_attn(self, layer, reduced):
        check(lib().ifa_model_tp_post_attn(self._h, layer, C.c_void_p(reduced.data_ptr())))

    def tp_ffn(self, layer, partial):
        check(lib().ifa_model_tp_ffn(self._h, layer, C.c_void_p(partial.data_ptr())))

    def tp_post_ffn(self, layer, reduced):
        check(lib().ifa_model_tp_post_ffn(self._h, layer, C.c_void_p(reduced.data_ptr())))

    def tp_logits(self, shard_out):
        check(lib().ifa_model_tp_logits(self._h, C.c_void_p(shard_out.data_ptr())))

    def tp_set_token(self, token_dev_int32):
        check(lib().ifa_model_tp_set_token(self._h, C.c_void_p(token_dev_int32.data_ptr())))

    def buffer(self, name, layer=0):
        p, n = C.c_void_p(), C.c_size_t()
        check(lib().ifa_model_get_buffer(self._h, name.encode(), layer, C.byref(p), C.byref(n)))
        return p.value, n.value

    def read_buffer(self, name, layer=0, nbytes=None):
        p, n = self.buffer(name, layer)
        n = n if nbytes is None else nbytes
        out = np.empty(n, np.uint8)
        check(lib().ifa_memcpy_d2h(out.ctypes.data_as(C.c_void_p), C.c_void_p(p), n, None))
        check(lib().ifa_stream_sync(None))
        return out

    def write_buffer(self, name, data, layer=0, offset=0):
        a = np.ascontiguousarray(data).view(np.uint8).reshape(-1)
        p, n = self.buffer(name, layer)
        assert offset + a.size <= n, (name, offset, a.size, n)
        check(lib().ifa_memcpy_h2d(C.c_void_p(p + offset), a.ctypes.data_as(C.c_void_p), a.size, None))
        check(lib().ifa_stream_sync(None))

    def close(self):
        if self._h:
            lib().ifa_model_destroy(self._h)
            self._h = C.c_void_p()

    def __del__(self):
        try:
            self.close()
        except Exception:
            pass


def topk_pool(logits, k, excluded_bits=None, stream=None):
    import torch
    rows, n = (1, logits.numel()) if logits.dim() == 1 else logits.shape
    ids = torch.empty((rows, max(k, 1)), dtype=torch.int32, device=logits.device)
    vals = torch.empty((rows, max(k, 1)), dtype=torch.int16, device=logits.device)
    cnt = torch.empty(rows, dtype=torch.int32, device=logits.device)
    check(lib().ifa_topk_pool(C.c_void_p(logits.data_ptr()), rows, n, int(k),
                              C.c_void_p(excluded_bits.data_ptr()) if excluded_bits is not None else None,
                              C.c_void_p(ids.data_ptr()), C.c_void_p(vals.data_ptr()), C.c_void_p(cnt.data_ptr()), C.c_void_p(stream)))
    return ids, vals, cnt


def rng_state_of_seed(seed):
    return (int(seed) ^ 0x5DEECE66D) & ((1 << 48) - 1)


def sample_params_array(rows):
    rec = np.dtype([("strategy_id", np.int32), ("temperature", np.float32), ("top_p", np.float32), ("max_k", np.int32), ("min_p", np.float32),
                   ("pool_size", np.int32)])
    a = np.zeros(len(rows), rec)
    for i, r in enumerate(rows):
        a[i] = tuple(r) + (0,)
    return a


def sample_pool_host(ids, vals_f16_bits, params, rng_state):
    ids = np.ascontiguousarray(ids, np.int32).reshape(-1)
    vals = np.ascontiguousarray(vals_f16_bits).view(np.uint16).reshape(-1)
    assert ids.size == vals.size
    if isinstance(params, np.void):
        params = np.array([params], params.dtype)
    pp = C.c_void_p(params.ctypes.data) if isinstance(params, np.ndarray) else C.cast(C.pointer(params), C.c_void_p)
    st = C.c_ulonglong(int(rng_state))
    tok, idx, cut = C.c_int(-1), C.c_int(-1), C.c_int(0)
    w, order = np.zeros(max(ids.size, 1), np.float32), np.full(max(ids.size, 1), -1, np.int32)
    check(lib().ifa_sample_pool_host(ids.ctypes.data_as(C.c_void_p), vals.ctypes.data_as(C.c_void_p), ids.size, pp, C.cast(C.pointer(st), C.c_void_p),
                                     C.cast(C.pointer(tok), C.c_void_p), C.cast(C.pointer(idx), C.c_void_p), C.cast(C.pointer(cut), C.c_void_p),
                                     w.ctypes.data_as(C.c_void_p), order.ctypes.data_as(C.c_void_p)))
    return tok.value, idx.value, cut.value, w[:ids.size], order[:ids.size], st.value


def sample_pool_rows(counts, ids, vals, params, rng_states, err, weights=None, stream=None):
    import torch
    rows, k = ids.shape
    tokens = torch.empty(rows, dtype=torch.int32, device=ids.device)
    index = torch.empty(rows, dtype=torch.int32, device=ids.device)
    check(lib().ifa_sample_pool_rows(_ptr(counts), _ptr(ids), _ptr(vals), rows, int(k), _ptr(params), _ptr(rng_states), _ptr(tokens), _ptr(index),
                                     _ptr(weights), _ptr(err), C.c_void_p(stream)))
    return tokens, index


def logsumexp_rows(logits, n=None, row_idx=None, targets=None, split=True, stream=None):
    import torch
# ... 165 lines not shown
```

Before: 622.4 tokens/s.

## Split decode into context-length route segments with per-route cached step graphs

Decode planning now divides the step range into up to three segments, ending at contexts 64, 128 and the full reach, and plans a separate attention route for each. Early steps can therefore use routes sized for short contexts instead of the one chosen for the longest context. Step graphs are cached per route, and graphs are uploaded during prepare, so switching routes avoids re-capturing and drop_graphs churn. The cost is more graph captures and memory, plus extra bookkeeping in the sampled-graph keys and in KV slot swaps.

```diff
diff --git a/include/inferflow_amd.h b/include/inferflow_amd.h
--- a/include/inferflow_amd.h
+++ b/include/inferflow_amd.h
@@ -265,6 +265,9 @@
 
 int ifa_decode_route_plan(const int *facts, int n_facts, int *out, int n_out);
 int ifa_model_decode_route(ifa_model *m, int *out, int n_out);
+int ifa_decode_segments_plan(const int *facts, int n_facts, int start_pos, int *out, int n_out);
+int ifa_model_decode_segments(ifa_model *m, int *out, int n_out);
+int ifa_model_graph_captures(ifa_model *m, unsigned long long *n_out);
 
 int ifa_prompt_route_plan(const int *facts, int n_facts, int *out, int n_out);
 int ifa_batch_route_plan(const int *facts, int n_facts, int *out, int n_out);
diff --git a/inferflow_amd/_capi.py b/inferflow_amd/_capi.py
--- a/inferflow_amd/_capi.py
+++ b/inferflow_amd/_capi.py
@@ -133,6 +133,9 @@
     "ifa_model_stream": (_vp, [_vp]),
     "ifa_model_time_kernel": (_i, [_vp, _i, _i, _vp]),
     "ifa_decode_route_plan": (_i, [_vp, _i, _vp, _i]),
+    "ifa_decode_segments_plan": (_i, [_vp, _i, _i, _vp, _i]),
+    "ifa_model_decode_segments": (_i, [_vp, _vp, _i]),
+    "ifa_model_graph_captures": (_i, [_vp, C.POINTER(C.c_ulonglong)]),
     "ifa_model_decode_route": (_i, [_vp, _vp, _i]),
     "ifa_prompt_route_plan": (_i, [_vp, _i, _vp, _i]),
     "ifa_batch_route_plan": (_i, [_vp, _i, _vp, _i]),
diff --git a/inferflow_amd/csrc/ifa_decode_route.h b/inferflow_amd/csrc/ifa_decode_route.h
--- a/inferflow_amd/csrc/ifa_decode_route.h
+++ b/inferflow_amd/csrc/ifa_decode_route.h
@@ -86,4 +86,25 @@
     return r;
 }
 
+struct DecSegment { int end = 0; DecRoute route; };
+struct DecSegments { int n = 0; DecSegment seg[3]; };
+constexpr int DEC_ROUTE_N_SEG_OUT = 1 + 3 * (1 + DEC_ROUTE_N_OUT);
+
+inline DecSegments plan_decode_segments(const DecRouteFacts &f, int start_pos)
+{
+    DecSegments S;
+    const DecRoute whole = plan_decode_route(f);
+    if (whole.kind == DEC_ROUTE_SPLIT || whole.error) { S.seg[0].end = f.reach; S.seg[0].route = whole; S.n = 1; return S; }
+    const int ends[3] = {64, 128, f.reach};
+    for (int i = 0; i < 3; i++) {
+        const int e = ends[i];
+        if (i < 2 && !(start_pos < e && e < f.reach)) continue;
+        DecRouteFacts g = f; g.reach = e;
+        const DecRoute r = plan_decode_route(g);
+        if (S.n && S.seg[S.n - 1].route == r) S.seg[S.n - 1].end = e;
+        else { S.seg[S.n].end = e; S.seg[S.n].route = r; S.n++; }
+    }
+    return S;
 }
+
+}
diff --git a/inferflow_amd/csrc/ifa_engine.hip b/inferflow_amd/csrc/ifa_engine.hip
--- a/inferflow_amd/csrc/ifa_engine.hip
+++ b/inferflow_amd/csrc/ifa_engine.hip
@@ -103,18 +103,23 @@
     return IFA_OK;
 }
 
+void destroy_step_graphs(std::vector<ifa_model::StepGraph> &t)
+{
+    for (auto &g : t) {
+        if (g.exec) (void)hipGraphExecDestroy(g.exec);
+        if (g.graph) (void)hipGraphDestroy(g.graph);
+        if (g.exec_n) (void)hipGraphExecDestroy(g.exec_n);
+        if (g.graph_n) (void)hipGraphDestroy(g.graph_n);
+    }
+    t.clear();
+}
+
 void drop_graphs(ifa_model *m)
 {
     if (m->tp_graph_exec) { (void)hipGraphExecDestroy(m->tp_graph_exec); m->tp_graph_exec = nullptr; }
     if (m->tp_graph) { (void)hipGraphDestroy(m->tp_graph); m->tp_graph = nullptr; }
-    if (m->graph_exec) { (void)hipGraphExecDestroy(m->graph_exec); m->graph_exec = nullptr; }
-    if (m->graph) { (void)hipGraphDestroy(m->graph); m->graph = nullptr; }
-    if (m->graph_exec_n) { (void)hipGraphExecDestroy(m->graph_exec_n); m->graph_exec_n = nullptr; }
-    if (m->graph_n) { (void)hipGraphDestroy(m->graph_n); m->graph_n = nullptr; }
-    for (auto &sl : m->slots) {
-        if (sl.exec) { (void)hipGraphExecDestroy(sl.exec); sl.exec = nullptr; }
-        if (sl.graph) { (void)hipGraphDestroy(sl.graph); sl.graph = nullptr; }
-    }
+    destroy_step_graphs(m->step_graphs);
+    for (auto &sl : m->slots) destroy_step_graphs(sl.step_graphs);
     for (auto &kv : m->batch_graphs) if (kv.second) (void)hipGraphExecDestroy(kv.second);
     m->batch_graphs.clear();
     for (auto &kv : m->draft_graphs) if (kv.second) (void)hipGraphExecDestroy(kv.second);
@@ -504,12 +509,10 @@
     ifa_model::KvSlot &out = m->slots[(size_t)m->cur_slot], &in = m->slots[(size_t)slot];
     out.k.clear(); out.v.clear();
     for (Layer &L : m->layers) { out.k.push_back(std::move(L.kcache)); out.v.push_back(std::move(L.vcache)); }
-    out.graph = m->graph; out.exec = m->graph_exec;
-    if (m->graph_exec_n) { (void)hipGraphExecDestroy(m->graph_exec_n); m->graph_exec_n = nullptr; }
-    if (m->graph_n) { (void)hipGraphDestroy(m->graph_n); m->graph_n = nullptr; }
     for (size_t l = 0; l < m->layers.size(); l++) { m->layers[l].kcache = std::move(in.k[l]); m->layers[l].vcache = std::move(in.v[l]); }
-    m->graph = in.graph; m->graph_exec = in.exec;
-    in.k.clear(); in.v.clear(); in.graph = nullptr; in.exec = nullptr;
+    out.step_graphs = std::move(m->step_graphs);
+    m->step_graphs = std::move(in.step_graphs);
+    in.k.clear(); in.v.clear(); in.step_graphs.clear();
     m->cur_slot = slot;
     return IFA_OK;
 }
@@ -521,7 +524,7 @@
     struct { const char *n; int *p; } opts[] = {
         {"fused", &m->opt_fused}, {"graph", &m->opt_graph}, {"rpw_qkv", &m->opt_rpw_qkv}, {"rpw_wo", &m->opt_rpw_wo},
         {"rpw_ffn", &m->opt_rpw_ffn}, {"rpw_w2", &m->opt_rpw_w2}, {"rpw_lm", &m->opt_rpw_lm}, {"trace", &m->opt_trace},
-        {"bench_mode", &m->opt_bench_mode}, {"touch_stride", &m->opt_touch_stride}, {"attn_split_ctx", &m->opt_attn_split_ctx}, {"batch_graph", &m->opt_batch_graph}, {"gemm_rows", &m->opt_gemm_rows}, {"batch_fused", &m->opt_batch_fused}, {"rows_mo", &m->opt_rows_mo}, {"debug_mo_alloc_fail", &m->opt_debug_mo_alloc_fail}, {"rows_kparts", &m->opt_rows_kparts}, {"prefill_chunk", &m->opt_prefill_chunk}, {"prefill_big_min", &m->opt_prefill_big_min}, {"prefill_mid", &m->opt_prefill_mid}, {"prefill_mid_max", &m->opt_prefill_mid_max}, {"prefill_res_mid", &m->opt_prefill_res_mid}, {"gemm_splitk", &m->opt_gemm_splitk}, {"moe_singles", &m->opt_moe_singles}, {"moe_overlap", &m->opt_moe_overlap}, {"prefill_big", &m->opt_prefill_big}, {"moe_router_fused", &m->opt_moe_router_fused}, {"tp_fuse_add", &m->opt_tp_fuse_add}, {"attn_q8", &m->opt_attn_q8}, {"attn_kt", &m->opt_attn_kt}, {"fuse_attn", &m->opt_fuse_attn}, {"fuse_ffn", &m->opt_fuse_ffn}, {"attn_post_as_residual", &m->opt_attn_post_as_residual}, {"chain_late_w2", &m->opt_chain_late_w2}, {"exact_order", &m->opt_exact_order}, {"perf_stat", &m->opt_perf_stat}, {"attn_nsplits", &m->opt_attn_nsplits}, {"attn_unload", &m->opt_attn_unload}, {"q3h_native", &m->opt_q3h_native}, {"fuse_attn_timeout_us", &m->opt_fuse_attn_timeout_us}, {"step_tail", &m->opt_step_tail}, {"graph_steps", &m->opt_graph_steps}, {"moe_device", &m->opt_moe_device}, 
+        {"bench_mode", &m->opt_bench_mode}, {"touch_stride", &m->opt_touch_stride}, {"attn_split_ctx", &m->opt_attn_split_ctx}, {"batch_graph", &m->opt_batch_graph}, {"gemm_rows", &m->opt_gemm_rows}, {"batch_fused", &m->opt_batch_fused}, {"rows_mo", &m->opt_rows_mo}, {"debug_mo_alloc_fail", &m->opt_debug_mo_alloc_fail}, {"rows_kparts", &m->opt_rows_kparts}, {"prefill_chunk", &m->opt_prefill_chunk}, {"prefill_big_min", &m->opt_prefill_big_min}, {"prefill_mid", &m->opt_prefill_mid}, {"prefill_mid_max", &m->opt_prefill_mid_max}, {"prefill_res_mid", &m->opt_prefill_res_mid}, {"gemm_splitk", &m->opt_gemm_splitk}, {"moe_singles", &m->opt_moe_singles}, {"moe_overlap", &m->opt_moe_overlap}, {"prefill_big", &m->opt_prefill_big}, {"moe_router_fused", &m->opt_moe_router_fused}, {"tp_fuse_add", &m->opt_tp_fuse_add}, {"attn_q8", &m->opt_attn_q8}, {"attn_kt", &m->opt_attn_kt}, {"fuse_attn", &m->opt_fuse_attn}, {"fuse_ffn", &m->opt_fuse_ffn}, {"attn_post_as_residual", &m->opt_attn_post_as_residual}, {"chain_late_w2", &m->opt_chain_late_w2}, {"exact_order", &m->opt_exact_order}, {"perf_stat", &m->opt_perf_stat}, {"attn_nsplits", &m->opt_attn_nsplits}, {"attn_unload", &m->opt_attn_unload}, {"q3h_native", &m->opt_q3h_native}, {"fuse_attn_timeout_us", &m->opt_fuse_attn_timeout_us}, {"step_tail", &m->opt_step_tail}, {"graph_steps", &m->opt_graph_steps}, {"route_segments", &m->opt_route_segments}, {"moe_device", &m->opt_moe_device}, 
         
         {"debug_layers", &m->opt_debug_layers}, {"debug_layer0", &m->opt_debug_layer0}, {"debug_hidden_in", &m->opt_debug_hidden_in}};
     for (auto &o : opts)
@@ -585,6 +588,42 @@
     IFA_REQUIRE(m && out && n_out >= DEC_ROUTE_N_OUT + 3, "ifa_model_decode_route: %d outputs expected", DEC_ROUTE_N_OUT + 3);
     memcpy(out, &m->route, sizeof(m->route));
     out[DEC_ROUTE_N_OUT] = num_cus(); out[DEC_ROUTE_N_OUT + 1] = visible_cus(); out[DEC_ROUTE_N_OUT + 2] = waits_enabled() ? 1 : 0;
+    return IFA_OK;
+}
+
+static void segments_out(const DecSegments &S, int *out)
+{
+    memset(out, 0, sizeof(int) * DEC_ROUTE_N_SEG_OUT);
+    out[0] = S.n;
+    for (int i = 0; i < S.n; i++) {
+        int *o = out + 1 + i * (1 + DEC_ROUTE_N_OUT);
+        o[0] = S.seg[i].end;
+        memcpy(o + 1, &S.seg[i].route, sizeof(DecRoute));
+    }
+}
+
+int ifa_decode_segments_plan(const int *facts, int n_facts, int start_pos, int *out, int n_out)
+{
+    IFA_REQUIRE(facts && out && n_facts == DEC_ROUTE_N_FACTS && n_out >= DEC_ROUTE_N_SEG_OUT, "ifa_decode_segments_plan: %d facts, %d outputs expected", DEC_ROUTE_N_FACTS, DEC_ROUTE_N_SEG_OUT);
+    DecRouteFacts f;
+    memcpy(&f, facts, sizeof(f));
+    IFA_REQUIRE(f.head_dim >= 8 && f.max_ctx >= 1, "ifa_decode_segments_plan: head_dim %d, max_ctx %d", f.head_dim, f.max_ctx);
+    IFA_REQUIRE(start_pos >= 0 && start_pos < f.reach, "ifa_decode_segments_plan: start_pos %d, reach %d", start_pos, f.reach);
+    segments_out(plan_decode_segments(f, start_pos), out);
+    return IFA_OK;
+}
+
+int ifa_model_decode_segments(ifa_model *m, int *out, int n_out)
+{
+    IFA_REQUIRE(m && out && n_out >= DEC_ROUTE_N_SEG_OUT, "ifa_model_decode_segments: %d outputs expected", DEC_ROUTE_N_SEG_OUT);
+    segments_out(m->last_segments, out);
+    return IFA_OK;
+}
+
+int ifa_model_graph_captures(ifa_model *m, unsigned long long *n_out)
+{
+    IFA_REQUIRE(m && n_out, "ifa_model_graph_captures: null pointer");
+    *n_out = m->graph_captures;
     return IFA_OK;
 }
 
diff --git a/inferflow_amd/csrc/ifa_engine_decode.hip b/inferflow_amd/csrc/ifa_engine_decode.hip
--- a/inferflow_amd/csrc/ifa_engine_decode.hip
+++ b/inferflow_amd/csrc/ifa_engine_decode.hip
@@ -174,12 +174,18 @@
     return f;
 }
 
-int decode_route_ready(ifa_model *m, int reach, bool own_launches)
-{
-    const ifa_model_config &c = m->cfg;
-    const DecRoute route = plan_decode_route(route_facts(m, reach, own_launches));
+void select_route(ifa_model *m, const DecRoute &route, int reach)
+{
     m->route_reach = reach;
-    if (!(route == m->route)) { m->route = route; drop_graphs(m); }
+    if (route == m->route) return;
+    m->route = route;
+    if (m->tp_graph_exec) { (void)hipGraphExecDestroy(m->tp_graph_exec); m->tp_graph_exec = nullptr; }
+    if (m->tp_graph) { (void)hipGraphDestroy(m->tp_graph); m->tp_graph = nullptr; }
+}
+
+static int route_buffers_ready(ifa_model *m, const DecRoute &route)
+{
+    const ifa_model_config &c = m->cfg;
     if (route.kind == DEC_ROUTE_FUSED_TAIL && !m->qa_gran) {
         const size_t n = (size_t)c.layers * (size_t)(c.heads + 2 * c.kv_heads) * c.head_dim;
         DevBuf<unsigned long long> gran; DevBuf<unsigned> call, err;
@@ -206,6 +212,16 @@
         IFA_HIP_CHECK(hipStreamSynchronize(m->stream));
     }
     return IFA_OK;
+}
+
+int decode_route_ready(ifa_model *m, int reach, bool own_launches)
+{
+    const DecRoute route = plan_decode_route(route_facts(m, reach, own_launches));
+    if (own_launches) {
+        m->route_reach = reach;
+        if (!(route == m->route)) { m->route = route; drop_graphs(m); }
+    } else select_route(m, route, reach);
+    return route_buffers_ready(m, route);
 }
 
 void qkv_params(ifa_model *m, int l, const half_t *x, DecGemvParams &P)
@@ -646,7 +662,21 @@
     if (*graph) (void)hipGraphDestroy(*graph);
     *graph = gph;
     IFA_HIP_CHECK(hipGraphInstantiate(exec, gph, nullptr, nullptr, 0));
+    m->graph_captures++;
     return IFA_OK;
+}
+
+static size_t step_graph_of(ifa_model *m)
+{
+    for (size_t i = 0; i < m->step_graphs.size(); i++) if (m->step_graphs[i].route == m->route) return i;
+    m->step_graphs.emplace_back();
+    m->step_graphs.back().route = m->route;
+    return m->step_graphs.size() - 1;
+}
+
+static void upload_graph(ifa_model *m, hipGraphExec_t exec)
+{
+    if (hipGraphUpload(exec, m->stream) != hipSuccess) (void)hipGetLastError();
 }
 
 int decode_impl(ifa_model *m, int first_token, int start_pos, int n_steps, int *out_tokens_host, float *elapsed_ms, bool prepare_only,
@@ -682,8 +712,14 @@
     if (rc) return rc;
     if (m->opt_q3h_native && (rc = ensure_q3hn(m))) return rc;
     hipStream_t s = m->stream;
-    if ((rc = decode_route_ready(m, start_pos + n_steps))) return rc;
-    const bool waits_on = m->route.kind == DEC_ROUTE_FUSED_TAIL || m->route.chain;
+    const DecRouteFacts facts = route_facts(m, start_pos + n_steps, false);
+    DecSegments segs;
+    if (m->opt_route_segments) segs = plan_decode_segments(facts, start_pos);
+    else { segs.n = 1; segs.seg[0].end = facts.reach; segs.seg[0].route = plan_decode_route(facts); }
+    m->last_segments = segs;
+    const DecRoute &last_route = segs.seg[segs.n - 1].route;
+    if ((rc = route_buffers_ready(m, last_route))) return rc;
+    const bool waits_on = last_route.kind == DEC_ROUTE_FUSED_TAIL || last_route.chain;
     if ((rc = step_tail_ready(m))) return rc;
     m->host_pinned[0] = first_token; m->host_pinned[1] = start_pos; m->host_pinned[2] = 0;
     IFA_HIP_CHECK(hipMemcpyAsync(m->state, m->host_pinned, 3 * sizeof(int), hipMemcpyHostToDevice, s));
@@ -692,37 +728,55 @@
         m->host_pinned[6] = (int)m->qa_calls;
         IFA_HIP_CHECK(hipMemcpyAsync(m->qa_call, m->host_pinned + 6, sizeof(int), hipMemcpyHostToDevice, s));
     }
-    hipGraphExec_t samp_exec = nullptr;
-    if (sc) {
-        if ((rc = sampled_prepare(m, *sc))) return rc;
-        if (m->opt_graph && (rc = sampled_graph(m, &samp_exec))) return rc;
-        if ((rc = sampled_begin(m, *sc))) return rc;
-    }
-    if (!sc && m->opt_graph && !m->graph_exec && (rc = capture_steps(m, 1, &m->graph, &m->graph_exec))) return rc;
+    if (sc && (rc = sampled_prepare(m, *sc))) return rc;
+    hipGraphExec_t samp_exec[3] = {nullptr, nullptr, nullptr};
+    size_t entry[3] = {0, 0, 0};
     const int S = m->opt_graph_steps;
-    if (!sc && m->opt_graph && S > 1 && n_steps >= S && (!m->graph_exec_n || m->graph_n_steps != S)) {
-        if (m->graph_exec_n) { (void)hipGraphExecDestroy(m->graph_exec_n); m->graph_exec_n = nullptr; }
-        if (m->graph_n) { (void)hipGraphDestroy(m->graph_n); m->graph_n = nullptr; }
-        if ((rc = capture_steps(m, S, &m->graph_n, &m->graph_exec_n))) return rc;
-        m->graph_n_steps = S;
-    }
-    if (prepare_only) return IFA_OK;
+    for (int k = 0; m->opt_graph && k < segs.n; k++) {
+        select_route(m, segs.seg[k].route, segs.seg[k].end);
+        if (sc) {
+            if ((rc = sampled_graph(m, &samp_exec[k]))) return rc;
+            continue;
+        }
+        const int len = segs.seg[k].end - (k ? segs.seg[k - 1].end : start_pos);
+        entry[k] = step_graph_of(m);
+        ifa_model::StepGraph &G = m->step_graphs[entry[k]];
+        if (!G.exec) {
+            if ((rc = capture_steps(m, 1, &G.graph, &G.exec))) return rc;
+            if (prepare_only) upload_graph(m, G.exec);
+        }
+        if (S > 1 && len >= S && (!G.exec_n || G.n_steps != S)) {
+            if (G.exec_n) { (void)hipGraphExecDestroy(G.exec_n); G.exec_n = nullptr; }
+            if (G.graph_n) { (void)hipGraphDestroy(G.graph_n); G.graph_n = nullptr; }
+            if ((rc = capture_steps(m, S, &G.graph_n, &G.exec_n))) return rc;
+            G.n_steps = S;
+            if (prepare_only) upload_graph(m, G.exec_n);
+        }
+    }
+    select_route(m, last_route, facts.reach);
+    if (prepare_only) { IFA_HIP_CHECK(hipStreamSynchronize(s)); return IFA_OK; }
+    if (sc && (rc = sampled_begin(m, *sc))) return rc;
     th("state copies enqueued");
     hipEvent_t e0 = nullptr, e1 = nullptr;
     if (elapsed_ms) { IFA_HIP_CHECK(hipEventCreate(&e0)); IFA_HIP_CHECK(hipEventCreate(&e1)); IFA_HIP_CHECK(hipEventRecord(e0, s)); }
     th("events created, first recorded");
     if (!sc && m->st_on && (rc = launch_gather(m))) return rc;
-    for (int i = 0; i < n_steps;) {
-        if (sc) {
-            if (samp_exec) IFA_HIP_CHECK(hipGraphLaunch(samp_exec, s));
-            else if ((rc = enqueue_fused_step(m, STEP_TAIL_SAMPLED))) return rc;
+    for (int k = 0, i = 0; k < segs.n; k++) {
+        select_route(m, segs.seg[k].route, segs.seg[k].end);
+        const int seg_n = segs.seg[k].end - start_pos;
+        const ifa_model::StepGraph *G = (m->opt_graph && !sc) ? &m->step_graphs[entry[k]] : nullptr;
+        while (i < seg_n) {
+            if (sc) {
+                if (samp_exec[k]) IFA_HIP_CHECK(hipGraphLaunch(samp_exec[k], s));
+                else if ((rc = enqueue_fused_step(m, STEP_TAIL_SAMPLED))) return rc;
+                i++;
+                continue;
+            }
+            if (G && G->exec_n && G->n_steps == S && S > 1 && seg_n - i >= S) { IFA_HIP_CHECK(hipGraphLaunch(G->exec_n, s)); i += S; continue; }
+            if (G) IFA_HIP_CHECK(hipGraphLaunch(G->exec, s));
+            else if ((rc = enqueue_fused_step(m))) return rc;
             i++;
-            continue;
-        }
-        if (m->opt_graph && m->graph_exec_n && m->graph_n_steps == S && S > 1 && n_steps - i >= S) { IFA_HIP_CHECK(hipGraphLaunch(m->graph_exec_n, s)); i += S; continue; }
-        if (m->opt_graph) IFA_HIP_CHECK(hipGraphLaunch(m->graph_exec, s));
-        else if ((rc = enqueue_fused_step(m))) return rc;
-        i++;
+        }
     }
     th("steps enqueued");
     if (elapsed_ms) IFA_HIP_CHECK(hipEventRecord(e1, s));
diff --git a/inferflow_amd/csrc/ifa_engine_sampled.hip b/inferflow_amd/csrc/ifa_engine_sampled.hip
--- a/inferflow_amd/csrc/ifa_engine_sampled.hip
+++ b/inferflow_amd/csrc/ifa_engine_sampled.hip
@@ -57,7 +57,8 @@
 
 int sampled_graph(ifa_model *m, hipGraphExec_t *exec_out)
 {
-    const int key = (m->cur_slot << 10) | (m->samp_k << 1) | (m->samp_armed ? 1 : 0);
+    ifa_model::SampKey key;
+    key.key = (m->cur_slot << 10) | (m->samp_k << 1) | (m->samp_armed ? 1 : 0); key.route = m->route;
     ifa_model::SampGraph &G = m->samp_graphs[key];
     const void *now[8] = {m->samp_blk.dev.get(), m->pool_blk.dev.get(), m->pool_excl.get(), m->la_state.get(), m->la_bias.get(), m->la_params.get(),
                           m->la_adj.get(), m->logits};
@@ -75,6 +76,7 @@
         (void)hipGraphDestroy(gph);
         if (ei != hipSuccess) { G.exec = nullptr; return ifa_fail(IFA_ERR_HIP, "hipGraphInstantiate: %s", hipGetErrorString(ei)); }
         std::copy(now, now + 8, G.ptrs);
+        m->graph_captures++;
     }
     *exec_out = G.exec;
     return IFA_OK;
diff --git a/inferflow_amd/csrc/ifa_engine_state.h b/inferflow_amd/csrc/ifa_engine_state.h
--- a/inferflow_amd/csrc/ifa_engine_state.h
+++ b/inferflow_amd/csrc/ifa_engine_state.h
@@ -92,9 +92,16 @@
     PinBuf<int> host_pinned;
     int scratch_tokens = 0;
     size_t kv_row_bytes = 0;
-    hipGraph_t graph = nullptr;
-    hipGraphExec_t graph_exec = nullptr;
-    hipGraph_t graph_n = nullptr; hipGraphExec_t graph_exec_n = nullptr; int graph_n_steps = 0, opt_graph_steps = 1;
+    struct StepGraph {
+        DecRoute route;
+        hipGraph_t graph = nullptr; hipGraphExec_t exec = nullptr;
+        hipGraph_t graph_n = nullptr; hipGraphExec_t exec_n = nullptr; int n_steps = 0;
+    };
+    std::vector<StepGraph> step_graphs;
+    int opt_graph_steps = 1;
+    int opt_route_segments = 1;
+    DecSegments last_segments;
+    unsigned long long graph_captures = 0;
     struct PendingAdd { const half_t *x = nullptr, *add = nullptr, *bias = nullptr; half_t *out = nullptr; bool on = false; } pend;
     int opt_tp_fuse_add = 1;
     DevPin<void> batch_tab;
@@ -123,7 +130,7 @@
     DevBuf<unsigned long long> st_keys; DevBuf<unsigned> st_counter;
     int opt_attn_kt = 1;
     int opt_attn_split_ctx = -1, opt_batch_graph = 0, opt_gemm_rows = 1, opt_batch_fused = 1, opt_moe_router_fused = 1, opt_prefill_big = 1, opt_rows_mo = 1, opt_moe_singles = 1;
-    struct KvSlot { std::vector<DevBuf<void>> k, v; hipGraph_t graph = nullptr; hipGraphExec_t exec = nullptr; };
+    struct KvSlot { std::vector<DevBuf<void>> k, v; std::vector<StepGraph> step_graphs; };
     std::vector<KvSlot> slots;
     int cur_slot = 0;
     int opt_attn_q8 = 1;
@@ -181,7 +188,11 @@
     std::vector<DevPin<void *>> kvc_retired;
     DevBuf<float> kvs_rot;
     struct SampGraph { hipGraphExec_t exec = nullptr; const void *ptrs[8] = {}; };
-    std::map<int, SampGraph> samp_graphs;
+    struct SampKey {
+        int key = 0; DecRoute route;
+        bool operator<(const SampKey &o) const { return key != o.key ? key < o.key : std::memcmp(&route, &o.route, sizeof(route)) < 0; }
+    };
+    std::map<SampKey, SampGraph> samp_graphs;
     DevPin<int> samp_blk;
     int samp_k = 0; bool samp_armed = false;
     static constexpr int RING = 1024;
@@ -272,6 +283,7 @@
 }
 
 void drop_graphs(ifa_model *m);
+void destroy_step_graphs(std::vector<ifa_model::StepGraph> &t);
 int perf_begin(ifa_model *m, int key);
 void perf_end(ifa_model *m, int idx);
 int perf_collect(ifa_model *m);
@@ -296,6 +308,7 @@
 int sep_norm(ifa_model *m, const half_t *x, const Tensor &w, const Tensor &b, half_t *dst);
 void attn_params(ifa_model *m, int l, DecAttnParams &A);
 int decode_route_ready(ifa_model *m, int reach, bool own_launches = false);
+void select_route(ifa_model *m, const DecRoute &route, int reach);
 void qkv_params(ifa_model *m, int l, const half_t *x, DecGemvParams &P);
 int launch_qkv_attn(ifa_model *m, int l, const half_t *x, unsigned tag_add = 0);
 int launch_qkv(ifa_model *m, int l, const half_t *x);
diff --git a/inferflow_amd/worker.py b/inferflow_amd/worker.py
--- a/inferflow_amd/worker.py
+++ b/inferflow_amd/worker.py
@@ -231,6 +231,24 @@
         d = dict(zip(self.ROUTE_FIELDS, out))
         d["kind"] = self.ROUTE_KINDS[d["kind"]]
         return d
+
+    def decode_segments(self):
+        n_route = 14
+        out = (C.c_int * (1 + 3 * (1 + n_route)))()
+        check(lib().ifa_model_decode_segments(self._h, out, len(out)))
+        segs = []
+        for i in range(out[0]):
+            o = out[1 + i * (1 + n_route):1 + (i + 1) * (1 + n_route)]
+            d = dict(zip(self.ROUTE_FIELDS[:n_route], o[1:]))
+            d["kind"] = self.ROUTE_KINDS[d["kind"]]
+            d["end"] = o[0]
+            segs.append(d)
+        return segs
+
+    def graph_captures(self):
+        n = C.c_ulonglong(0)
+        check(lib().ifa_model_graph_captures(self._h, C.byref(n)))
+        return int(n.value)
 
     PROMPT_ROUTE_FIELDS = ("kind", "first_pass", "norm_fused", "res_mid") + tuple(
         p + "_" + k for p in ("qkv", "wo", "w13", "w2") for k in ("kernel", "src", "mo", "no_waits")) + ("need_mo", "need_x32")
```

Result: no change. 623.5 tokens/s, median of 3 (+0.2%).
